# qitianwu/SGFormer

Hardware: AMD Instinct MI355X
Metric: SGFormer fwd+bwd nodes/sec on ogbn-products full-graph (higher is better)
Workload: dtype bf16

## Files before the change

include/sgf.h:

```cpp
#ifndef SGF_H_
#define SGF_H_

#include <stddef.h>
#include <stdint.h>

#ifdef __cplusplus
extern "C" {
#endif

#define SGF_VERSION 662

#define SGF_F32 0
#define SGF_BF16 1
#define SGF_F32_BF16X3 2

#define SGF_OK 0
#define SGF_E_INVALID (-1)
#define SGF_E_WORKSPACE (-2)
#define SGF_E_HIP (-3)
#define SGF_E_UNSUPPORTED (-4)

int sgf_version(void);
const char* sgf_last_error(void);
int sgf_reload_env(void);

size_t sgf_csr_workspace_bytes(int64_t nnz, int64_t n);
int sgf_csr_build(const int64_t* edge_index, int64_t nnz, int64_t n, int64_t* rowptr,
                  int32_t* colind, float* val, int32_t* deg, void* workspace,
                  size_t workspace_bytes, void* stream);

int sgf_csr_transpose(const int64_t* edge_index, int64_t nnz, int64_t n, const int32_t* deg,
                      const int64_t* rowptr, const int32_t* colind, int64_t* t_rowptr,
                      int32_t* t_colind, float* t_val, int32_t* is_symmetric, void* workspace,
                      size_t workspace_bytes, void* stream);

size_t sgf_subgraph_workspace_bytes(int64_t nnz, int64_t n);
int sgf_subgraph_plan(const int64_t* edge_index, int64_t nnz, int64_t n, const int64_t* subset,
                      int64_t m, int32_t* relabel, int64_t* total, void* workspace,
                      size_t workspace_bytes, void* stream);
int sgf_subgraph_emit(const int64_t* edge_index, int64_t nnz, int64_t n, const int32_t* relabel,
                      int32_t relabel_nodes, int64_t total, int64_t* out, int64_t* out_eid,
                      void* workspace, size_t workspace_bytes, void* stream);

size_t sgf_subgraph_csr_plan_workspace_bytes(int64_t m);
size_t sgf_subgraph_csr_emit_workspace_bytes(int64_t m, int64_t total);
int sgf_subgraph_csr_plan(const int64_t* rowptr, const int32_t* colind, int64_t n, const int64_t* subset, int64_t m,
                          int32_t* local_of, int64_t* rowptr_b, int32_t* deg_b, int64_t* total, void* workspace,
                          size_t workspace_bytes, void* stream);
int sgf_subgraph_csr_emit(const int64_t* rowptr, const int32_t* colind, int64_t n, const int64_t* subset, int64_t m,
                          int32_t* local_of, const int64_t* rowptr_b, const int32_t* deg_b, int64_t total, int32_t* colind_b,
                          float* val_b, int64_t* edge_index_b, void* workspace, size_t workspace_bytes, void* stream);

size_t sgf_graph_prologue_workspace_bytes(int64_t m, int64_t n);
int sgf_graph_prologue_plan(const int64_t* edge_index, int64_t m, int64_t n, int32_t to_undirected,
                            int32_t remove_self_loops, int32_t add_self_loops, int64_t* total,
                            void* workspace, size_t workspace_bytes, void* stream);
int sgf_graph_prologue_emit(int64_t m, int64_t n, int32_t to_undirected, int32_t add_self_loops,
                            int64_t total, int64_t* out, void* workspace, size_t workspace_bytes,
                            void* stream);

int sgf_spmm(const int64_t* rowptr, const int32_t* colind, const float* val, const void* x,
             int64_t ldx, int64_t n_cols, void* y, int64_t ldy, int64_t n_rows, int32_t d,
             int32_t dtype, void* stream);

int32_t sgf_spmm_segment_len(void);
int32_t sgf_spmm_arm(int32_t d, int32_t dtype, int64_t ldx, int64_t ldy, int64_t n_cols, int32_t aligned16,
                     int32_t stream);
size_t sgf_spmm_split_workspace_bytes(int64_t long_segments, int32_t d);
int sgf_spmm_split(const int64_t* rowptr, const int32_t* colind, const float* val, const void* x,
                   int64_t ldx, int64_t n_cols, void* y, int64_t ldy, int64_t n_rows, int32_t d, int32_t dtype,
                   int64_t long_len, int64_t long_segments, void* workspace, size_t workspace_bytes,
                   void* stream);

int sgf_spmm_stream(const int64_t* rowptr, const int32_t* colind, const float* val, const void* x,
                    int64_t ldx, int64_t n_cols, void* y, int64_t ldy, int64_t n_rows, int32_t d, int32_t dtype,
                    int64_t long_len, int64_t long_segments, void* workspace, size_t workspace_bytes,
                    void* stream);

size_t sgf_reorder_workspace_bytes(int64_t nnz, int64_t n);
int sgf_reorder(const int64_t* edge_index, int64_t nnz, int64_t n, int32_t iters1, int32_t iters2,
                int32_t* perm, int32_t* inv, int32_t* community, void* workspace, size_t workspace_bytes,
                void* stream);
size_t sgf_spmm_plan_workspace_bytes(int64_t nnz, int64_t n, int32_t rows_per_block);
int sgf_spmm_plan(const int64_t* rowptr, const int32_t* colind, const float* val, int64_t n, int64_t nnz,
                  int32_t rows_per_block, int32_t lds_rows, int64_t long_len, int32_t* ecode, float* eval,
                  int32_t* nlds, int32_t* sh_ptr, int32_t* sh_cols, int64_t* stats, void* workspace,
                  size_t workspace_bytes, void* stream);
int32_t sgf_spmm_lds_rows_len(int32_t dtype);
int32_t sgf_spmm_blocked_arm(int32_t d, int32_t dtype, int64_t ldx, int64_t ldy, int64_t n_rows, int32_t rows_per_block,
                             int32_t lds_rows, int32_t aligned16);
int sgf_spmm_blocked(const int64_t* rowptr, const int32_t* ecode, const float* eval, const int32_t* nlds,
                     const int32_t* sh_ptr, const int32_t* sh_cols, const void* x, int64_t ldx, void* y,
                     int64_t ldy, int64_t n_rows, int32_t d, int32_t dtype, int32_t rows_per_block,
                     int32_t lds_rows, int64_t long_len, int64_t long_segments, void* workspace,
                     size_t workspace_bytes, void* stream);

int sgf_spmm_tile_supported(int32_t d, int32_t dtype);
int sgf_spmm_tile_blocks(const int32_t* comm_sorted, int64_t n, int32_t max_rows, int32_t* blk_row,
                         int64_t blk_cap, int64_t* nb_out, void* stream);
size_t sgf_spmm_tile_plan_workspace_bytes(int64_t nnz, int64_t n, int64_t nb);
int sgf_spmm_tile_plan(const int64_t* rowptr, const int32_t* colind, const float* val, int64_t n, int64_t nnz,
                       const int32_t* blk_row, int64_t nb, int32_t cap, int32_t min_count, int64_t long_len,
                       int32_t* ecode, float* eval, int32_t* nlds, int32_t* sh_ptr, int32_t* sh_cols,
                       int64_t* tile_ptr, int64_t* rem_rowptr, int64_t* stats, void* workspace,
                       size_t workspace_bytes, void* stream);
int sgf_spmm_tile_fill(const int64_t* rowptr, const int32_t* ecode, const float* eval, const int32_t* nlds,
                       int64_t n, int64_t nnz, const int32_t* blk_row, int64_t nb, const int64_t* tile_ptr,
                       int64_t n_frag, const int64_t* rem_rowptr, void* tiles, int32_t* rem_col, float* rem_val,
                       void* stream);
int32_t sgf_spmm_tile_sparse_len(void);
size_t sgf_spmm_tile_pack_workspace_bytes(int64_t n_frag);
int sgf_spmm_tile_pack_layout(const int32_t* blk_row, int64_t nb, const int64_t* tile_ptr, const void* tiles,
                              int64_t n_frag, int32_t* grp, int64_t* pool_units, void* workspace,
                              size_t workspace_bytes, void* stream);
int sgf_spmm_tile_pack(const int32_t* blk_row, int64_t nb, const int64_t* tile_ptr, const void* tiles, int64_t n_frag,
                       const int32_t* grp, void* pool, int64_t pool_units, void* stream);
int sgf_spmm_tile(const int32_t* blk_row, int64_t nb, int32_t block_rows, const int32_t* sh_ptr, const int32_t* sh_cols,
                  const int64_t* tile_ptr, const int32_t* grp, const void* pool, const int64_t* rem_rowptr,
                  const int32_t* rem_col, const float* rem_val, const void* x, int64_t ldx, int64_t n_cols, void* y, int64_t ldy,
                  int64_t n_rows, int32_t d, int32_t dtype, int64_t long_len, int64_t long_segments,
                  void* workspace, size_t workspace_bytes, void* stream);

size_t sgf_neighbor_sample_workspace_bytes(int64_t m, int64_t edge_cap);
int sgf_neighbor_sample_mark(int32_t* local_of, const int32_t* ids, int64_t count, int32_t base, void* stream);
int sgf_neighbor_sample_hop(const int64_t* rowptr, const int32_t* colind, const int32_t* frontier, int64_t m,
                            int32_t frontier_local0, int32_t fanout, uint64_t seed, uint64_t batch, int32_t hop,
                            int32_t* local_of, int32_t n_known, int64_t edge_cap, int32_t* edge_src_local,
                            int32_t* edge_dst_local, int32_t* src_global, int32_t* new_nodes, int64_t* counts,
                            void* workspace, size_t workspace_bytes, void* stream);

size_t sgf_neighbor_sample_batch_workspace_bytes(int64_t batch_size, const int32_t* fanouts, int32_t hops, int64_t* node_cap,
                                                  int64_t* edge_cap);
int sgf_neighbor_sample_batch(const int64_t* rowptr, const int32_t* colind, const int32_t* seeds, int64_t batch_size,
                              const int32_t* fanouts, int32_t hops, uint64_t seed, uint64_t batch, int32_t* local_of,
                              int32_t* nodes, int64_t node_cap, int32_t* edge_src_local, int32_t* edge_dst_local,
                              int64_t edge_cap, int64_t* counts, void* workspace, size_t workspace_bytes, void* stream);

int32_t sgf_sampled_csr_supported(int32_t max_fanout);
size_t sgf_sampled_csr_build_workspace_bytes(int64_t node_cap, int64_t edge_cap);
int sgf_sampled_csr_build(const int32_t* edge_src_local, const int32_t* edge_dst_local, const int64_t* counts,
                          int64_t node_cap, int64_t edge_cap, int32_t max_fanout, int64_t* rowptr_b, int32_t* colind_b,
                          float* val_b, int32_t* deg_b, void* workspace, size_t workspace_bytes, void* stream);
size_t sgf_sampled_csr_transpose_workspace_bytes(int64_t n, int64_t nnz);
int sgf_sampled_csr_transpose(const int64_t* rowptr, const int32_t* colind, const float* val, int64_t n, int64_t nnz,
                              int64_t* t_rowptr, int32_t* t_colind, float* t_val, void* workspace, size_t workspace_bytes,
                              void* stream);

int sgf_gather_rows(const void* src, int64_t lds, int32_t src_dtype, int64_t n_src, const void* idx,
                    int32_t idx_is_int64, int64_t n_out, int32_t d, void* dst, int64_t ldd,
                    int32_t dst_dtype, void* stream);
int sgf_pad_rows(const void* src, int64_t lds, int32_t src_dtype, int64_t n_src, const void* idx, int32_t idx_is_int64,
                 int64_t n_out, int32_t d, int32_t d_pad, void* dst, int64_t ldd, int32_t dst_dtype, void* stream);

int64_t sgf_attn_stats_len(int32_t heads, int32_t d);
size_t sgf_attn_workspace_bytes(int64_t n, int32_t heads, int32_t d);
// ... 16 lines not shown
                        int64_t ldo, const float* den, int64_t n, int32_t heads, int32_t d,
                        int32_t dtype, float* bstats, void* workspace, size_t workspace_bytes,
                        void* stream);

int sgf_attn_bwd_apply(const void* q, int64_t ldq, const void* k, int64_t ldk, const void* v,
                       int64_t ldv, const void* g, int64_t ldg, const void* o, int64_t ldo,
                       const float* den, int64_t n, double n_total, int32_t heads,
                       int32_t v_heads, int32_t d, int32_t dtype, const float* stats,
                       float* bstats, void* dq, int64_t lddq, void* dk, int64_t lddk,
                       void* dv, int64_t lddv, void* stream);
int sgf_attn_bwd_reduce_heads(const void* q, int64_t ldq, const void* g, int64_t ldg, const void* o, int64_t ldo,
                              const float* den, int64_t n, int32_t heads, int32_t d, int32_t dtype, float* bstats,
                              void* workspace, size_t workspace_bytes, void* stream);
int sgf_attn_bwd_apply_heads(const void* q, int64_t ldq, const void* k, int64_t ldk, const void* v, int64_t ldv, const void* g,
                             int64_t ldg, const void* o, int64_t ldo, const float* den, int64_t n, double n_total,
                             int32_t heads, int32_t v_heads, int32_t d, int32_t dtype, const float* stats, float* bstats,
                             void* dq, int64_t lddq, void* dk, int64_t lddk, void* dv, int64_t lddv, void* stream);

int64_t sgf_attn_h_bstats_len(int32_t d);
int32_t sgf_attn_h_supported(int32_t d, int32_t dtype);
int sgf_attn_h_fwd(const void* h, int64_t ldh, int64_t n, int32_t d, int32_t dtype, const float* M,
                   const float* m, const float* w, const float* beta, void* out, int64_t ldo,
                   float* den, void* stream);
int sgf_attn_h_bwd_reduce(const void* h, int64_t ldh, const void* g, int64_t ldg, const void* o,
                          int64_t ldo, const float* den, int64_t n, int32_t d, int32_t dtype,
                          float* hstats, void* workspace, size_t workspace_bytes, void* stream);
int sgf_attn_h_bwd_apply(const void* h, int64_t ldh, const void* g, int64_t ldg, const void* o,
                         int64_t ldo, const float* den, int64_t n, int32_t d, int32_t dtype,
                         const float* M, const float* w, const float* D, const float* ds, void* dh,
                         int64_t lddh, void* workspace, size_t workspace_bytes, void* stream);
size_t sgf_attn_h_bwd_apply_workspace_bytes(int64_t n, int32_t d, int32_t dtype);
int32_t sgf_attn_h_bwd_split_supported(int32_t d, int32_t dtype);
int sgf_attn_h_bwd_pre(const void* g, int64_t ldg, const void* o, int64_t ldo, const float* den, int64_t n, int32_t d,
                       int32_t dtype, const float* M, const float* w, void* workspace, size_t workspace_bytes,
                       float* rowscal, void* stream);
int sgf_attn_h_bwd_reduce_scaled(const void* h, int64_t ldh, const void* g, int64_t ldg, const float* rowscal, int64_t n,
                                 int32_t d, int32_t dtype, float* hstats, void* workspace, size_t workspace_bytes,
                                 void* stream);
int sgf_attn_h_bwd_post(const void* h, int64_t ldh, int64_t n, int32_t d, int32_t dtype, const float* D, const float* ds,
                        const void* workspace, size_t workspace_bytes, const void* addend, int64_t ldadd, void* dh,
                        int64_t lddh, void* stream);

size_t sgf_attn_h_small_saved_bytes(int32_t d_in, int32_t d_out);
size_t sgf_attn_h_small_workspace_bytes(int32_t d_in, int32_t d_out);
int sgf_attn_h_small_fwd(const float* G, int64_t ldg, const float* s, float n_rows, float n_total, const float* wq,
                         const float* bq, const float* wk, const float* bk, const float* wv, const float* bv, int64_t ldw,
                         int32_t d_in, int32_t d_out, float* M, int64_t ldm, float* m, float* w, float* beta, void* saved,
                         size_t saved_bytes, void* stream);
int sgf_attn_h_small_bwd(const float* dM, int64_t lddm, const float* dw, const float* dm, const float* dbeta, float n_total,
                         int32_t d_in, int32_t d_out, const void* saved, size_t saved_bytes, float* dG2, int64_t lddg,
                         float* ds, float* gwq, float* gbq, float* gwk, float* gbk, float* gwv, float* gbv, int64_t ldgw,
                         void* workspace, size_t workspace_bytes, void* stream);

size_t sgf_gram_workspace_bytes(int64_t n, int32_t m, int32_t k);
int sgf_gram(const void* a, int64_t lda, int32_t m, const void* b, int64_t ldb, int32_t k,
             int64_t n, int32_t dtype, float* c, int64_t ldc, float* colsum_a, void* workspace,
             size_t workspace_bytes, void* stream);
int sgf_gram2(const void* a, int64_t lda, int32_t m, const void* b1, int64_t ldb1, const void* b2, int64_t ldb2, int32_t k,
              int64_t n, int32_t dtype, float* c1, int64_t ldc1, float* c2, int64_t ldc2, float* colsum_a, void* workspace,
              size_t workspace_bytes, void* stream);

int sgf_ln_fwd(const void* x, int64_t ldx, const void* res, int64_t ldr, float a, float b,
               const float* gamma, const float* beta, int32_t relu, float eps, int64_t n,
               int32_t d, int32_t dtype, void* y, int64_t ldy, float* mean, float* rstd,
               void* stream);

size_t sgf_ln_bwd_workspace_bytes(int64_t n, int32_t d);
int sgf_ln_bwd(const void* dy, int64_t lddy, const void* y, int64_t ldy, const void* x,
               int64_t ldx, const void* res, int64_t ldr, float a, float b, const float* gamma,
               int32_t relu, const float* mean, const float* rstd, int64_t n, int32_t d,
               int32_t dtype, void* dx, int64_t lddx, void* dres, int64_t lddres, float* dgamma,
               float* dbeta, void* workspace, size_t workspace_bytes, void* stream);

size_t sgf_colstats_workspace_bytes(int64_t n, int32_t d);
int sgf_colstats(const void* x, int64_t ldx, const float* shift, int64_t n, int32_t d,
                 int32_t dtype, float* stats, void* workspace, size_t workspace_bytes,
                 void* stream);
int sgf_bn_finalize(const float* sums, const float* shift, double n_total, float eps, float momentum, float* running_mean,
                    float* running_var, int32_t d, float* mean, float* rstd, void* stream);
int sgf_bn_apply(const void* x, int64_t ldx, const float* mean, const float* rstd,
                 const float* gamma, const float* beta, const void* res, int64_t ldr,
                 int32_t relu, int64_t n, int32_t d, int32_t dtype, void* y, int64_t ldy,
                 void* stream);
int sgf_bn_bwd_stats(const void* dy, int64_t lddy, const void* x, int64_t ldx, const float* mean,
                     const float* rstd, const float* gamma, const float* beta, int32_t relu,
                     int64_t n, int32_t d, int32_t dtype, float* stats, void* workspace,
                     size_t workspace_bytes, void* stream);
int sgf_bn_bwd_stats2(const void* dy, int64_t lddy, const void* dy2, int64_t lddy2, const void* x, int64_t ldx,
                      const float* mean, const float* rstd, const float* gamma, const float* beta, int32_t relu, int64_t n,
                      int32_t d, int32_t dtype, float* stats, void* workspace, size_t workspace_bytes, void* stream);
int32_t sgf_gram_ln_bwd_supported(int32_t m, int32_t k, int32_t dtype);
int sgf_gram_ln_bwd(const void* g, int64_t ldg, const void* xin, int64_t ldx, const float* mean, const float* rstd,
                    const float* gamma, const float* beta, int32_t relu, int32_t m, const void* b, int64_t ldb, int32_t k,
                    int64_t n, int32_t dtype, float* c, int64_t ldc, float* colsum, float* dgamma, float* dbeta, void* workspace,
                    size_t workspace_bytes, void* stream);
int32_t sgf_gram_bn_bwd_supported(int32_t m, int32_t k, int32_t dtype);
int sgf_gram_bn_bwd(const void* g1, int64_t ldg1, const void* g2, int64_t ldg2, const void* z, int64_t ldz, const float* mean,
                    const float* rstd, const float* gamma, const float* beta, int32_t relu, const float* stats, float inv_n,
                    int32_t training, int32_t m, const void* b, int64_t ldb, int32_t k, int64_t n, int32_t dtype, float* c,
                    int64_t ldc, float* colsum, void* workspace, size_t workspace_bytes, void* stream);
int32_t sgf_gram2_bn_bwd_supported(int32_t m, int32_t k, int64_t n, int32_t dtype);
int sgf_gram2_bn_bwd(const void* g, int64_t ldg, const void* z, int64_t ldz, const float* mean, const float* rstd,
                     const float* gamma, const float* beta, int32_t relu, const float* stats, float inv_n, int32_t training,
                     int32_t m, const void* b1, int64_t ldb1, const void* b2, int64_t ldb2, int32_t k, int64_t n, int32_t dtype,
                     void* dz, int64_t lddz, float* c1, int64_t ldc1, float* c2, int64_t ldc2, float* colsum, void* workspace,
                     size_t workspace_bytes, void* stream);
int sgf_bn_bwd_apply(const void* dy, int64_t lddy, const void* x, int64_t ldx, const float* mean,
                     const float* rstd, const float* gamma, const float* beta, int32_t relu,
                     const float* stats, float inv_n, int32_t training, int64_t n, int32_t d,
                     int32_t dtype, void* dx, int64_t lddx, void* stream);

int32_t sgf_combine_fc_supported(int32_t d, int32_t classes, int32_t dtype);
int sgf_combine_fc_fwd(const void* x1, int64_t ld1, float a, const void* x2, int64_t ld2, float b,
                       const float* w, const float* bias, int64_t n, int32_t d, int32_t classes,
                       int32_t dtype, float* logits, int64_t ldl, void* stream);
int sgf_combine_fc_bwd(const float* dlogits, int64_t lddl, const float* w, int64_t n, int32_t d,
                       int32_t classes, float a, float b, int32_t dtype, void* dx1, int64_t ld1, void* dx2,
                       int64_t ld2, void* stream);
int sgf_combine_fc_fwd_mapped(const void* x1, int64_t ld1, float a, const void* x2, int64_t ld2, float b, const float* w,
                              const float* bias, int64_t n, int32_t d, int32_t classes, int32_t dtype, float* logits,
                              int64_t ldl, const int32_t* row_map, void* stream);
int sgf_combine_fc_bwd_mapped(const float* dlogits, int64_t lddl, const float* w, int64_t n, int32_t d, int32_t classes,
                              float a, float b, int32_t dtype, void* dx1, int64_t ld1, void* dx2, int64_t ld2,
                              const int32_t* row_map, void* stream);
int sgf_combine_fc_bwd_g(const float* dlogits, int64_t lddl, const float* w, int64_t n, int32_t d, int32_t classes, float a,
                         float b, int32_t dtype, void* dx1, int64_t ld1, void* dx2, int64_t ld2, const int32_t* row_map,
                         void* g_out, int64_t ldg, void* stream);

int32_t sgf_gcn_epilogue_supported(int32_t d_in, int32_t d_out, int32_t dtype);
size_t sgf_gcn_epilogue_workspace_bytes(int64_t n, int32_t d_out);
int sgf_gcn_epilogue_stats(const void* a, int64_t lda, const void* w, int64_t ldw, const float* bias,
                           int64_t n, int32_t d_in, int32_t d_out, int32_t dtype, void* y, int64_t ldy,
                           const float* shift, float* stats, void* workspace, size_t workspace_bytes,
                           void* stream);
int sgf_gcn_epilogue_dx2(const void* dy, int64_t lddy, const void* w1, const void* w2, int64_t ldw, int64_t n, int32_t d,
                         int32_t dtype, void* dx1, int64_t lddx1, void* dx2, int64_t lddx2, int32_t pair, void* stream);

int32_t sgf_gcn_epilogue_dx2_acc_supported(int32_t d, int32_t dtype);
int sgf_gcn_epilogue_dx2_acc(const void* dz, int64_t lddz, const void* w, int64_t ldw, int64_t n, int32_t d, int32_t dtype,
                             void* dy, int64_t lddy, const void* gadd, int64_t ldg, const void* acc_in, int64_t ldai,
                             void* acc_out, int64_t ldao, void* stream);
int sgf_gcn_epilogue_dx(const void* dy, int64_t lddy, const void* w, int64_t ldw, int64_t n, int32_t d_in,
                        int32_t d_out, int32_t dtype, void* dx, int64_t lddx, void* stream);
int sgf_gcn_epilogue_apply(const void* y, int64_t ldy, const float* mean, const float* rstd, const float* gamma,
                           const float* beta, const void* res, int64_t ldr, int32_t relu, int64_t n, int32_t d,
                           int32_t dtype, void* out, int64_t ldo, void* stream);
int32_t sgf_gcn_bn_bwd_dx_supported(int32_t d, int32_t dtype);
size_t sgf_gcn_bn_bwd_dx_workspace_bytes(int64_t n, int32_t d);
int sgf_gcn_bn_bwd_dx(const void* gy, int64_t ldg, const void* z, int64_t ldz, const float* mean, const float* rstd,
                      const float* gamma, const float* beta, int32_t relu, const float* stats, float inv_n,
                      int32_t training, const void* w, int64_t ldw, int64_t n, int32_t d, int32_t dtype, void* dz,
                      int64_t lddz, void* dy, int64_t lddy, const void* acc_in, void* acc_out, size_t acc_bytes,
                      void* dx0, int64_t lddx0, int32_t add_gy, void* workspace, size_t workspace_bytes, void* stream);
int32_t sgf_gcn_epilogue_cat_supported(int32_t d, int32_t dtype);
int sgf_gcn_epilogue_cat(const void* a1, int64_t lda1, const void* a2, int64_t lda2, const void* w, int64_t ldw,
                         const float* bias, int64_t n, int32_t d, int32_t dtype, void* y, int64_t ldy, const float* shift,
                         float* stats, void* workspace, size_t workspace_bytes, void* stream);
size_t sgf_gcn_epilogue_partial_bytes(int64_t n, int32_t d_out);
size_t sgf_gcn_epilogue_dtype_partial_bytes(int64_t n, int32_t d_out, int32_t dtype);
int sgf_gcn_epilogue_partial(const void* a, int64_t lda, const void* w, int64_t ldw, const float* bias, int64_t n,
                             int32_t d_in, int32_t d_out, int32_t dtype, void* partial, size_t partial_bytes,
                             void* stream);
int sgf_gcn_epilogue_stats_add(const void* a, int64_t lda, const void* w, int64_t ldw, const void* partial,
                               size_t partial_bytes, int64_t n, int32_t d_in, int32_t d_out, int32_t dtype,
                               void* y, int64_t ldy, const float* shift, float* stats, void* workspace,
                               size_t workspace_bytes, void* stream);
// ... 74 lines not shown
```

sgformer_amd/_lib.py:

```python
from __future__ import annotations

import ctypes
import os
from ctypes import c_char_p, c_double, c_float, c_int32, c_int64, c_size_t, c_uint64, c_void_p

_HERE = os.path.dirname(os.path.abspath(__file__))
LIB_PATH = os.path.join(_HERE, "lib", "libsgf.so")

SGF_F32 = 0
SGF_BF16 = 1
SGF_F32_BF16X3 = 2
SGF_BCE_TARGET_F32 = 0
SGF_BCE_TARGET_I64 = 1
SGF_BCE_TARGET_CLASS = 2
SGF_METRIC_TARGET_F32 = 0
SGF_METRIC_TARGET_I64 = 1

_lib = None

_P = c_void_p
SIGNATURES = {
    "sgf_version": (c_int32, []),
    "sgf_last_error": (c_char_p, []),
    "sgf_reload_env": (c_int32, []),
    "sgf_csr_workspace_bytes": (c_size_t, [c_int64, c_int64]),
    "sgf_csr_build": (c_int32, [_P, c_int64, c_int64, _P, _P, _P, _P, _P, c_size_t, _P]),
    "sgf_csr_transpose": (c_int32, [_P, c_int64, c_int64, _P, _P, _P, _P, _P, _P, _P, _P, c_size_t, _P]),
    "sgf_subgraph_workspace_bytes": (c_size_t, [c_int64, c_int64]),
    "sgf_subgraph_plan": (c_int32, [_P, c_int64, c_int64, _P, c_int64, _P, _P, _P, c_size_t, _P]),
    "sgf_subgraph_emit": (c_int32, [_P, c_int64, c_int64, _P, c_int32, c_int64, _P, _P, _P, c_size_t, _P]),
    "sgf_subgraph_csr_plan_workspace_bytes": (c_size_t, [c_int64]),
    "sgf_subgraph_csr_emit_workspace_bytes": (c_size_t, [c_int64, c_int64]),
    "sgf_subgraph_csr_plan": (c_int32, [_P, _P, c_int64, _P, c_int64, _P, _P, _P, _P, _P, c_size_t, _P]),
    "sgf_subgraph_csr_emit": (c_int32, [_P, _P, c_int64, _P, c_int64, _P, _P, _P, c_int64, _P, _P, _P, _P, c_size_t, _P]),
    "sgf_graph_prologue_workspace_bytes": (c_size_t, [c_int64, c_int64]),
    "sgf_graph_prologue_plan": (c_int32, [_P, c_int64, c_int64, c_int32, c_int32, c_int32, _P, _P, c_size_t, _P]),
    "sgf_graph_prologue_emit": (c_int32, [c_int64, c_int64, c_int32, c_int32, c_int64, _P, _P, c_size_t, _P]),
    "sgf_spmm": (c_int32, [_P, _P, _P, _P, c_int64, c_int64, _P, c_int64, c_int64, c_int32, c_int32, _P]),
    "sgf_spmm_segment_len": (c_int32, []),
    "sgf_spmm_arm": (c_int32, [c_int32, c_int32, c_int64, c_int64, c_int64, c_int32, c_int32]),
    "sgf_spmm_split_workspace_bytes": (c_size_t, [c_int64, c_int32]),
    "sgf_spmm_split": (c_int32, [_P, _P, _P, _P, c_int64, c_int64, _P, c_int64, c_int64, c_int32, c_int32, c_int64,
                                 c_int64, _P, c_size_t, _P]),
    "sgf_spmm_stream": (c_int32, [_P, _P, _P, _P, c_int64, c_int64, _P, c_int64, c_int64, c_int32, c_int32, c_int64,
                                  c_int64, _P, c_size_t, _P]),
    "sgf_reorder_workspace_bytes": (c_size_t, [c_int64, c_int64]),
    "sgf_reorder": (c_int32, [_P, c_int64, c_int64, c_int32, c_int32, _P, _P, _P, _P, c_size_t, _P]),
    "sgf_spmm_plan_workspace_bytes": (c_size_t, [c_int64, c_int64, c_int32]),
    "sgf_spmm_plan": (c_int32, [_P, _P, _P, c_int64, c_int64, c_int32, c_int32, c_int64, _P, _P, _P, _P, _P, _P,
                                _P, c_size_t, _P]),
    "sgf_spmm_lds_rows_len": (c_int32, [c_int32]),
    "sgf_spmm_blocked_arm": (c_int32, [c_int32, c_int32, c_int64, c_int64, c_int64, c_int32, c_int32, c_int32]),
    "sgf_spmm_blocked": (c_int32, [_P, _P, _P, _P, _P, _P, _P, c_int64, _P, c_int64, c_int64, c_int32, c_int32,
                                   c_int32, c_int32, c_int64, c_int64, _P, c_size_t, _P]),
    "sgf_spmm_tile_supported": (c_int32, [c_int32, c_int32]),
    "sgf_spmm_tile_blocks": (c_int32, [_P, c_int64, c_int32, _P, c_int64, _P, _P]),
    "sgf_spmm_tile_plan_workspace_bytes": (c_size_t, [c_int64, c_int64, c_int64]),
    "sgf_spmm_tile_plan": (c_int32, [_P, _P, _P, c_int64, c_int64, _P, c_int64, c_int32, c_int32, c_int64, _P, _P, _P,
                                     _P, _P, _P, _P, _P, _P, c_size_t, _P]),
    "sgf_spmm_tile_fill": (c_int32, [_P, _P, _P, _P, c_int64, c_int64, _P, c_int64, _P, c_int64, _P, _P, _P, _P, _P]),
    "sgf_spmm_tile_sparse_len": (c_int32, []),
    "sgf_spmm_tile_pack_workspace_bytes": (c_size_t, [c_int64]),
    "sgf_spmm_tile_pack_layout": (c_int32, [_P, c_int64, _P, _P, c_int64, _P, _P, _P, c_size_t, _P]),
    "sgf_spmm_tile_pack": (c_int32, [_P, c_int64, _P, _P, c_int64, _P, _P, c_int64, _P]),
    "sgf_spmm_tile": (c_int32, [_P, c_int64, c_int32, _P, _P, _P, _P, _P, _P, _P, _P, _P, c_int64, c_int64, _P, c_int64,
                                c_int64, c_int32, c_int32, c_int64, c_int64, _P, c_size_t, _P]),
    "sgf_neighbor_sample_workspace_bytes": (c_size_t, [c_int64, c_int64]),
    "sgf_neighbor_sample_mark": (c_int32, [_P, _P, c_int64, c_int32, _P]),
    "sgf_neighbor_sample_batch_workspace_bytes": (c_size_t, [c_int64, _P, c_int32, _P, _P]),
    "sgf_neighbor_sample_batch": (c_int32, [_P, _P, _P, c_int64, _P, c_int32, c_uint64, c_uint64, _P, _P, c_int64, _P, _P,
                                            c_int64, _P, _P, c_size_t, _P]),
    "sgf_neighbor_sample_hop": (c_int32, [_P, _P, _P, c_int64, c_int32, c_int32, c_uint64, c_uint64, c_int32, _P, c_int32,
                                          c_int64, _P, _P, _P, _P, _P, _P, c_size_t, _P]),
    "sgf_sampled_csr_supported": (c_int32, [c_int32]),
    "sgf_sampled_csr_build_workspace_bytes": (c_size_t, [c_int64, c_int64]),
    "sgf_sampled_csr_build": (c_int32, [_P, _P, _P, c_int64, c_int64, c_int32, _P, _P, _P, _P, _P, c_size_t, _P]),
    "sgf_sampled_csr_transpose_workspace_bytes": (c_size_t, [c_int64, c_int64]),
    "sgf_sampled_csr_transpose": (c_int32, [_P, _P, _P, c_int64, c_int64, _P, _P, _P, _P, c_size_t, _P]),
    "sgf_gather_rows": (c_int32, [_P, c_int64, c_int32, c_int64, _P, c_int32, c_int64, c_int32, _P, c_int64,
                                  c_int32, _P]),
    "sgf_pad_rows": (c_int32, [_P, c_int64, c_int32, c_int64, _P, c_int32, c_int64, c_int32, c_int32, _P, c_int64,
                               c_int32, _P]),
    "sgf_attn_stats_len": (c_int64, [c_int32, c_int32]),
    "sgf_attn_bstats_len": (c_int64, [c_int32, c_int32]),
    "sgf_attn_workspace_bytes": (c_size_t, [c_int64, c_int32, c_int32]),
    "sgf_attn_max_blocks": (c_int32, []),
    "sgf_attn_tile_rows": (c_int32, [c_int32, c_int32, c_int32]),
    "sgf_attn_fwd_reduce": (c_int32, [_P, c_int64, _P, c_int64, _P, c_int64, c_int64, c_int32, c_int32,
                                      c_int32, c_int32, _P, _P, c_size_t, _P]),
    "sgf_attn_fwd_apply": (c_int32, [_P, c_int64, _P, c_int64, c_int64, c_double, c_int32, c_int32,
                                     c_int32, c_int32, _P, _P, c_int64, _P, _P, _P]),
    "sgf_attn_bwd_reduce": (c_int32, [_P, c_int64, _P, c_int64, _P, c_int64, _P, c_int64, c_int32,
                                      c_int32, c_int32, _P, _P, c_size_t, _P]),
    "sgf_attn_bwd_apply": (c_int32, [_P, c_int64, _P, c_int64, _P, c_int64, _P, c_int64, _P, c_int64,
                                     _P, c_int64, c_double, c_int32, c_int32, c_int32, c_int32, _P, _P,
                                     _P, c_int64, _P, c_int64, _P, c_int64, _P]),
    "sgf_attn_bwd_reduce_heads": (c_int32, [_P, c_int64, _P, c_int64, _P, c_int64, _P, c_int64, c_int32,
                                            c_int32, c_int32, _P, _P, c_size_t, _P]),
    "sgf_attn_bwd_apply_heads": (c_int32, [_P, c_int64, _P, c_int64, _P, c_int64, _P, c_int64, _P, c_int64,
                                           _P, c_int64, c_double, c_int32, c_int32, c_int32, c_int32, _P, _P,
                                           _P, c_int64, _P, c_int64, _P, c_int64, _P]),
    "sgf_attn_h_bstats_len": (c_int64, [c_int32]),
    "sgf_attn_h_fwd": (c_int32, [_P, c_int64, c_int64, c_int32, c_int32, _P, _P, _P, _P, _P, c_int64, _P, _P]),
    "sgf_attn_h_bwd_reduce": (c_int32, [_P, c_int64, _P, c_int64, _P, c_int64, _P, c_int64, c_int32, c_int32,
                                        _P, _P, c_size_t, _P]),
    "sgf_attn_h_bwd_apply": (c_int32, [_P, c_int64, _P, c_int64, _P, c_int64, _P, c_int64, c_int32, c_int32,
                                       _P, _P, _P, _P, _P, c_int64, _P, c_size_t, _P]),
    "sgf_attn_h_bwd_apply_workspace_bytes": (c_size_t, [c_int64, c_int32, c_int32]),
    "sgf_attn_h_bwd_split_supported": (c_int32, [c_int32, c_int32]),
    "sgf_attn_h_supported": (c_int32, [c_int32, c_int32]),
    "sgf_attn_h_bwd_pre": (c_int32, [_P, c_int64, _P, c_int64, _P, c_int64, c_int32, c_int32, _P, _P, _P, c_size_t, _P, _P]),
    "sgf_attn_h_bwd_reduce_scaled": (c_int32, [_P, c_int64, _P, c_int64, _P, c_int64, c_int32, c_int32, _P, _P, c_size_t,
                                               _P]),
    "sgf_attn_h_bwd_post": (c_int32, [_P, c_int64, c_int64, c_int32, c_int32, _P, _P, _P, c_size_t, _P, c_int64, _P,
                                      c_int64, _P]),
    "sgf_attn_h_small_saved_bytes": (c_size_t, [c_int32, c_int32]),
    "sgf_attn_h_small_workspace_bytes": (c_size_t, [c_int32, c_int32]),
    "sgf_attn_h_small_fwd": (c_int32, [_P, c_int64, _P, c_float, c_float, _P, _P, _P, _P, _P, _P, c_int64, c_int32, c_int32,
                                       _P, c_int64, _P, _P, _P, _P, c_size_t, _P]),
    "sgf_attn_h_small_bwd": (c_int32, [_P, c_int64, _P, _P, _P, c_float, c_int32, c_int32, _P, c_size_t, _P, c_int64, _P,
                                       _P, _P, _P, _P, _P, _P, c_int64, _P, c_size_t, _P]),
    "sgf_gram_workspace_bytes": (c_size_t, [c_int64, c_int32, c_int32]),
    "sgf_gram": (c_int32, [_P, c_int64, c_int32, _P, c_int64, c_int32, c_int64, c_int32, _P, c_int64, _P,
                           _P, c_size_t, _P]),
    "sgf_gram2": (c_int32, [_P, c_int64, c_int32, _P, c_int64, _P, c_int64, c_int32, c_int64, c_int32, _P, c_int64, _P,
                            c_int64, _P, _P, c_size_t, _P]),
    "sgf_ln_fwd": (c_int32, [_P, c_int64, _P, c_int64, c_float, c_float, _P, _P, c_int32, c_float,
                             c_int64, c_int32, c_int32, _P, c_int64, _P, _P, _P]),
    "sgf_ln_bwd_workspace_bytes": (c_size_t, [c_int64, c_int32]),
    "sgf_ln_bwd": (c_int32, [_P, c_int64, _P, c_int64, _P, c_int64, _P, c_int64, c_float, c_float, _P,
                             c_int32, _P, _P, c_int64, c_int32, c_int32, _P, c_int64, _P, c_int64, _P,
                             _P, _P, c_size_t, _P]),
    "sgf_colstats_workspace_bytes": (c_size_t, [c_int64, c_int32]),
    "sgf_colstats": (c_int32, [_P, c_int64, _P, c_int64, c_int32, c_int32, _P, _P, c_size_t, _P]),
    "sgf_bn_finalize": (c_int32, [_P, _P, c_double, c_float, c_float, _P, _P, c_int32, _P, _P, _P]),
    "sgf_bn_apply": (c_int32, [_P, c_int64, _P, _P, _P, _P, _P, c_int64, c_int32, c_int64, c_int32,
                               c_int32, _P, c_int64, _P]),
    "sgf_bn_bwd_stats": (c_int32, [_P, c_int64, _P, c_int64, _P, _P, _P, _P, c_int32, c_int64, c_int32,
                                   c_int32, _P, _P, c_size_t, _P]),
    "sgf_bn_bwd_stats2": (c_int32, [_P, c_int64, _P, c_int64, _P, c_int64, _P, _P, _P, _P, c_int32, c_int64, c_int32,
                                    c_int32, _P, _P, c_size_t, _P]),
    "sgf_gram_ln_bwd_supported": (c_int32, [c_int32, c_int32, c_int32]),
    "sgf_gram_ln_bwd": (c_int32, [_P, c_int64, _P, c_int64, _P, _P, _P, _P, c_int32, c_int32, _P, c_int64, c_int32, c_int64,
                                  c_int32, _P, c_int64, _P, _P, _P, _P, c_size_t, _P]),
    "sgf_gram_bn_bwd_supported": (c_int32, [c_int32, c_int32, c_int32]),
    "sgf_gram_bn_bwd": (c_int32, [_P, c_int64, _P, c_int64, _P, c_int64, _P, _P, _P, _P, c_int32, _P, c_float, c_int32,
                                  c_int32, _P, c_int64, c_int32, c_int64, c_int32, _P, c_int64, _P, _P, c_size_t, _P]),
    "sgf_gram2_bn_bwd_supported": (c_int32, [c_int32, c_int32, c_int64, c_int32]),
    "sgf_gram2_bn_bwd": (c_int32, [_P, c_int64, _P, c_int64, _P, _P, _P, _P, c_int32, _P, c_float, c_int32, c_int32, _P, c_int64,
                                   _P, c_int64, c_int32, c_int64, c_int32, _P, c_int64, _P, c_int64, _P, c_int64, _P, _P,
                                   c_size_t, _P]),
    "sgf_bn_bwd_apply": (c_int32, [_P, c_int64, _P, c_int64, _P, _P, _P, _P, c_int32, _P, c_float,
                                   c_int32, c_int64, c_int32, c_int32, _P, c_int64, _P]),
    "sgf_dropout": (c_int32, [_P, c_int64, _P, c_int64, c_float, c_uint64, c_int64, c_int32, c_int32, _P,
                              c_int64, _P]),
    "sgf_dropout_dev": (c_int32, [_P, c_int64, _P, c_int64, c_float, _P, c_int64, c_int32, c_int32, _P,
                                  c_int64, _P]),
    "sgf_nll_workspace_bytes": (c_size_t, [c_int64]),
    "sgf_nll_fwd": (c_int32, [_P, c_int64, c_int64, c_int32, c_int32, _P, _P, c_int64, _P, _P, c_size_t, _P]),
    "sgf_nll_bwd": (c_int32, [_P, c_int64, c_int64, c_int32, c_int32, _P, _P, c_int64, _P, c_float, _P,
                              c_int64, _P]),
    "sgf_bce_workspace_bytes": (c_size_t, [c_int64, c_int32]),
    "sgf_bce_fwd": (c_int32, [_P, c_int64, c_int64, c_int32, c_int32, _P, c_int64, c_int32, _P, c_int64, c_float, _P, _P,
                              c_size_t, _P]),
    "sgf_bce_bwd": (c_int32, [_P, c_int64, c_int64, c_int32, c_int32, _P, c_int64, c_int32, _P, c_int64, _P, c_float, _P,
                              c_int64, _P]),
    "sgf_rocauc_workspace_bytes": (c_size_t, [c_int64, c_int32]),
    "sgf_rocauc_counts": (c_int32, [_P, c_int64, c_int64, c_int32, c_int32, _P, c_int64, c_int32, _P, c_int64, _P, _P,
                                    c_size_t, _P]),
    "sgf_argmax_workspace_bytes": (c_size_t, [c_int64, c_int32]),
    "sgf_argmax_count": (c_int32, [_P, c_int64, c_int64, c_int32, c_int32, _P, c_int64, c_int32, _P, c_int64, _P, _P,
                                   c_size_t, _P]),
    "sgf_sum_n": (c_int32, [_P, _P, c_int32, c_int64, c_int32, c_int32, _P, c_int64, _P]),
    "sgf_colsum_workspace_bytes": (c_size_t, [c_int64, c_int32]),
    "sgf_colsum": (c_int32, [_P, c_int64, c_int64, c_int32, c_int32, _P, _P, c_size_t, _P]),
    "sgf_combine_fc_supported": (c_int32, [c_int32, c_int32, c_int32]),
    "sgf_combine_fc_fwd": (c_int32, [_P, c_int64, c_float, _P, c_int64, c_float, _P, _P, c_int64, c_int32, c_int32,
                                     c_int32, _P, c_int64, _P]),
    "sgf_combine_fc_bwd": (c_int32, [_P, c_int64, _P, c_int64, c_int32, c_int32, c_float, c_float, c_int32, _P,
                                     c_int64, _P, c_int64, _P]),
    "sgf_combine_fc_fwd_mapped": (c_int32, [_P, c_int64, c_float, _P, c_int64, c_float, _P, _P, c_int64, c_int32, c_int32,
                                     c_int32, _P, c_int64, _P, _P]),
    "sgf_combine_fc_bwd_g": (c_int32, [_P, c_int64, _P, c_int64, c_int32, c_int32, c_float, c_float, c_int32, _P, c_int64, _P,
                                       c_int64, _P, _P, c_int64, _P]),
    "sgf_combine_fc_bwd_mapped": (c_int32, [_P, c_int64, _P, c_int64, c_int32, c_int32, c_float, c_float, c_int32, _P,
                                     c_int64, _P, c_int64, _P, _P]),
    "sgf_gcn_epilogue_supported": (c_int32, [c_int32, c_int32, c_int32]),
    "sgf_gcn_epilogue_workspace_bytes": (c_size_t, [c_int64, c_int32]),
    "sgf_gcn_epilogue_stats": (c_int32, [_P, c_int64, _P, c_int64, _P, c_int64, c_int32, c_int32, c_int32, _P, c_int64,
                                         _P, _P, _P, c_size_t, _P]),
    "sgf_gcn_epilogue_dx": (c_int32, [_P, c_int64, _P, c_int64, c_int64, c_int32, c_int32, c_int32, _P, c_int64, _P]),
    "sgf_gcn_epilogue_dx2": (c_int32, [_P, c_int64, _P, _P, c_int64, c_int64, c_int32, c_int32, _P, c_int64, _P, c_int64,
                                       c_int32, _P]),
    "sgf_gcn_epilogue_dx2_acc_supported": (c_int32, [c_int32, c_int32]),
    "sgf_gcn_epilogue_dx2_acc": (c_int32, [_P, c_int64, _P, c_int64, c_int64, c_int32, c_int32, _P, c_int64, _P, c_int64, _P,
                                           c_int64, _P, c_int64, _P]),
    "sgf_gcn_epilogue_apply": (c_int32, [_P, c_int64, _P, _P, _P, _P, _P, c_int64, c_int32, c_int64, c_int32,
                               c_int32, _P, c_int64, _P]),
    "sgf_gcn_bn_bwd_dx_supported": (c_int32, [c_int32, c_int32]),
    "sgf_gcn_bn_bwd_dx_workspace_bytes": (c_size_t, [c_int64, c_int32]),
    "sgf_gcn_bn_bwd_dx": (c_int32, [_P, c_int64, _P, c_int64, _P, _P, _P, _P, c_int32, _P, c_float, c_int32, _P, c_int64,
                                    c_int64, c_int32, c_int32, _P, c_int64, _P, c_int64, _P, _P, c_size_t, _P, c_int64,
                                    c_int32, _P, c_size_t, _P]),
    "sgf_gcn_epilogue_cat_supported": (c_int32, [c_int32, c_int32]),
    "sgf_gcn_epilogue_cat": (c_int32, [_P, c_int64, _P, c_int64, _P, c_int64, _P, c_int64, c_int32, c_int32, _P, c_int64,
                                       _P, _P, _P, c_size_t, _P]),
    "sgf_gcn_epilogue_partial_bytes": (c_size_t, [c_int64, c_int32]),
    "sgf_gcn_epilogue_dtype_partial_bytes": (c_size_t, [c_int64, c_int32, c_int32]),
    "sgf_gcn_epilogue_partial": (c_int32, [_P, c_int64, _P, c_int64, _P, c_int64, c_int32, c_int32, c_int32, _P,
                                           c_size_t, _P]),
    "sgf_gcn_epilogue_stats_add": (c_int32, [_P, c_int64, _P, c_int64, _P, c_size_t, c_int64, c_int32, c_int32,
                                             c_int32, _P, c_int64, _P, _P, _P, c_size_t, _P]),
    "sgf_stem_pair_supported": (c_int32, [c_int32, c_int32, c_int32]),
    "sgf_stem_pair": (c_int32, [_P, c_int64, c_int64, c_int32, _P, c_int64, _P, _P, c_int64, _P, c_int32, c_int32, _P,
                                c_int64, _P, c_int64, _P, _P, _P, c_size_t, _P]),
    "sgf_gemm": (c_int32, [_P, c_int64, c_int64, c_int32, _P, c_int64, c_int64, c_int32, c_int64, c_int32, c_int64, c_float,
                           _P, _P, c_float, _P, c_int64, c_int32, _P, c_int64, c_int32, _P]),
    "sgf_comm_available": (c_int32, []),
    "sgf_comm_unique_id_bytes": (c_int32, []),
    "sgf_comm_unique_id": (c_int32, [_P]),
# ... 47 lines not shown
```

sgformer_amd/csrc/fused.hip:

```cpp
#include "common.h"

namespace sgf {
namespace {

constexpr int kThreads = 256;
constexpr int kMaxD = 1024;
constexpr int kMaxStatBlocks = 2048;

__device__ __forceinline__ float4 zero4() { return make_float4(0.f, 0.f, 0.f, 0.f); }
__device__ __forceinline__ float4 ld4f(const float* p) { return *reinterpret_cast<const float4*>(p); }

inline int lanes_per_row(int d) {
  int l = 16;
  while (l * 4 < d && l < 64) l <<= 1;
  return l;
}

template <typename T, int LPR, int NC>
__global__ __launch_bounds__(kThreads) void k_ln_fwd(
    const T* __restrict__ x, int64_t ldx, const T* __restrict__ res, int64_t ldr, float a, float b,
    const float* __restrict__ gamma, const float* __restrict__ beta, int relu, float eps, int64_t n,
    int d, T* __restrict__ y, int64_t ldy, float* __restrict__ mean, float* __restrict__ rstd) {
  constexpr int RPB = kThreads / LPR;
  const int sl = threadIdx.x % LPR;
// ... 466 lines not shown
          g.z = (xh.z * ga.z + be.z) > 0.f ? g.z : 0.f;
          g.w = (xh.w * ga.w + be.w) > 0.f ? g.w : 0.f;
        }
        if (training) {
          g.x -= s0.x * inv_n + xh.x * s1.x * inv_n;
          g.y -= s0.y * inv_n + xh.y * s1.y * inv_n;
          g.z -= s0.z * inv_n + xh.z * s1.z * inv_n;
          g.w -= s0.w * inv_n + xh.w * s1.w * inv_n;
        }
        store4<T>(dx + row * lddx + col,
                  make_float4(ga.x * rs.x * g.x, ga.y * rs.y * g.y, ga.z * rs.z * g.z, ga.w * rs.w * g.w));
      }
    }
  }
}

typedef __bf16 ew_bf16v2 __attribute__((ext_vector_type(2)));
typedef float ew_f32v2 __attribute__((ext_vector_type(2)));
__device__ __forceinline__ uint32_t ew_pack(float a, float b) {
  const ew_f32v2 v = {a, b};
  return __builtin_bit_cast(uint32_t, __builtin_convertvector(v, ew_bf16v2));
}
__device__ __forceinline__ void ew_unpack(const uint4& r, float (&v)[8]) {
  v[0] = __uint_as_float(r.x << 16); v[1] = __uint_as_float(r.x & 0xffff0000u);
  v[2] = __uint_as_float(r.y << 16); v[3] = __uint_as_float(r.y & 0xffff0000u);
  v[4] = __uint_as_float(r.z << 16); v[5] = __uint_as_float(r.z & 0xffff0000u);
  v[6] = __uint_as_float(r.w << 16); v[7] = __uint_as_float(r.w & 0xffff0000u);
}
__device__ __forceinline__ uint4 ew_pack8(const float (&o)[8]) {
  return make_uint4(ew_pack(o[0], o[1]), ew_pack(o[2], o[3]), ew_pack(o[4], o[5]), ew_pack(o[6], o[7]));
}
struct BnCoeffs8 {
  float mu[8], rs[8], ga[8], be[8];
};
__device__ __forceinline__ void bn_coeffs8(const BnParams& p, int col, BnCoeffs8& c) {
#pragma unroll
  for (int e = 0; e < 8; ++e) {
    c.mu[e] = p.mean[col + e];
    c.rs[e] = p.rstd[col + e];
    c.ga[e] = p.gamma ? p.gamma[col + e] : 1.f;
    c.be[e] = p.beta ? p.beta[col + e] : 0.f;
  }
}

template <bool kRes, int U>
__global__ __launch_bounds__(kThreads) void k_bn_apply_bf16x8(const uint16_t* __restrict__ x, int64_t ldx, BnParams p,
                                                              const uint16_t* __restrict__ res, int64_t ldr, int relu,
                                                              int64_t n, int d, uint16_t* __restrict__ y, int64_t ldy) {
  const int f8 = d / 8;
  const int rpp = kThreads / f8;
  const int sr = threadIdx.x / f8;
  if (sr >= rpp) return;
  const int col = (threadIdx.x % f8) * 8;
  BnCoeffs8 c;
  bn_coeffs8(p, col, c);
  const int64_t rpb = static_cast<int64_t>(rpp) * U;
  for (int64_t row0 = static_cast<int64_t>(blockIdx.x) * rpb + sr; row0 < n; row0 += static_cast<int64_t>(gridDim.x) * rpb) {
    uint4 xv[U], rv[U];
#pragma unroll
    for (int u = 0; u < U; ++u) {
      const int64_t row = row0 + u * rpp;
      if (row < n) {
        xv[u] = *reinterpret_cast<const uint4*>(x + row * ldx + col);
        if (kRes) rv[u] = *reinterpret_cast<const uint4*>(res + row * ldr + col);
      }
    }
#pragma unroll
    for (int u = 0; u < U; ++u) {
      const int64_t row = row0 + u * rpp;
      if (row < n) {
        float v[8], r[8], o[8];
        ew_unpack(xv[u], v);
        if (kRes) ew_unpack(rv[u], r);
#pragma unroll
        for (int e = 0; e < 8; ++e) {
          o[e] = fmaf((v[e] - c.mu[e]) * c.rs[e], c.ga[e], c.be[e]);
          if (relu) o[e] = fmaxf(o[e], 0.f);
          if (kRes) o[e] += r[e];
        }
        *reinterpret_cast<uint4*>(y + row * ldy + col) = ew_pack8(o);
      }
    }
  }
}

template <int U>
__global__ __launch_bounds__(kThreads) void k_bn_bwd_apply_bf16x8(
    const uint16_t* __restrict__ dy, int64_t lddy, const uint16_t* __restrict__ x, int64_t ldx, BnParams p, int relu,
    const float* __restrict__ stats, float inv_n, int training, int64_t n, int d, uint16_t* __restrict__ dx, int64_t lddx) {
  const int f8 = d / 8;
  const int rpp = kThreads / f8;
  const int sr = threadIdx.x / f8;
  if (sr >= rpp) return;
  const int col = (threadIdx.x % f8) * 8;
  BnCoeffs8 c;
  bn_coeffs8(p, col, c);
  float s0[8], s1[8];
#pragma unroll
  for (int e = 0; e < 8; ++e) {
    s0[e] = training ? stats[col + e] : 0.f;
    s1[e] = training ? stats[d + col + e] : 0.f;
  }
  const int64_t rpb = static_cast<int64_t>(rpp) * U;
  for (int64_t row0 = static_cast<int64_t>(blockIdx.x) * rpb + sr; row0 < n; row0 += static_cast<int64_t>(gridDim.x) * rpb) {
    uint4 xv[U], gv[U];
#pragma unroll
    for (int u = 0; u < U; ++u) {
      const int64_t row = row0 + u * rpp;
      if (row < n) {
        xv[u] = *reinterpret_cast<const uint4*>(x + row * ldx + col);
        gv[u] = *reinterpret_cast<const uint4*>(dy + row * lddy + col);
      }
    }
#pragma unroll
    for (int u = 0; u < U; ++u) {
      const int64_t row = row0 + u * rpp;
      if (row < n) {
        float v[8], g[8], o[8];
        ew_unpack(xv[u], v);
        ew_unpack(gv[u], g);
#pragma unroll
        for (int e = 0; e < 8; ++e) {
          const float xh = (v[e] - c.mu[e]) * c.rs[e];
          float ge = g[e];
          if (relu) ge = fmaf(xh, c.ga[e], c.be[e]) > 0.f ? ge : 0.f;
          if (training) ge -= s0[e] * inv_n + xh * s1[e] * inv_n;
          o[e] = c.ga[e] * c.rs[e] * ge;
        }
        *reinterpret_cast<uint4*>(dx + row * lddx + col) = ew_pack8(o);
      }
    }
  }
}

template <int LPR, int R>
__global__ __launch_bounds__(kThreads) void k_ln_bwd_bf16x8(
    const uint16_t* __restrict__ dy, int64_t lddy, const uint16_t* __restrict__ y, int64_t ldy, const uint16_t* __restrict__ x,
    int64_t ldx, const uint16_t* __restrict__ res, int64_t ldr, float a, float b, const float* __restrict__ gamma, int relu,
    const float* __restrict__ mean, const float* __restrict__ rstd, int64_t n, uint16_t* __restrict__ dxo, int64_t lddx,
    uint16_t* __restrict__ dro, int64_t lddr, float* __restrict__ part) {
  constexpr int RPS = kThreads / LPR;
  constexpr int RPB = RPS * R;
  constexpr int D = 8 * LPR;
  constexpr float inv_d = 1.0f / static_cast<float>(D);
  __shared__ float red[2 * RPS * D];
  const int sl = threadIdx.x % LPR;
  const int sr = threadIdx.x / LPR;
  const int col = sl * 8;
  const bool ln = gamma != nullptr;
  float gm[8], dg[8], db[8];
#pragma unroll
  for (int e = 0; e < 8; ++e) {
    gm[e] = ln ? gamma[col + e] : 1.f;
    dg[e] = db[e] = 0.f;
  }
  for (int64_t row0 = static_cast<int64_t>(blockIdx.x) * RPB; row0 < n; row0 += static_cast<int64_t>(gridDim.x) * RPB) {
    uint4 gv[R], yv[R], xv[R], rv[R];
    float mu[R], rs[R];
#pragma unroll
    for (int q = 0; q < R; ++q) {
      const int64_t row = row0 + q * RPS + sr;
      const int64_t rr = row < n ? row : n - 1;
      gv[q] = *reinterpret_cast<const uint4*>(dy + rr * lddy + col);
      if (relu) yv[q] = *reinterpret_cast<const uint4*>(y + rr * ldy + col);
      if (ln) {
        xv[q] = *reinterpret_cast<const uint4*>(x + rr * ldx + col);
// ... 713 lines not shown
}

extern "C" int sgf_colstats(const void* x, int64_t ldx, const float* shift, int64_t n, int32_t d,
                            int32_t dtype, float* stats, void* workspace, size_t workspace_bytes,
                            void* stream) {
  int rc = check_ew("sgf_colstats", n, d, dtype);
  if (rc != SGF_OK) return rc;
  hipStream_t st = static_cast<hipStream_t>(stream);
  SGF_REQUIRE(stats, SGF_E_INVALID, "sgf_colstats: null stats");
  if (n == 0) {
    SGF_CHECK_HIP(hipMemsetAsync(stats, 0, 2 * d * sizeof(float), st));
    return SGF_OK;
  }
  SGF_REQUIRE(x && ldx % 4 == 0, SGF_E_INVALID, "sgf_colstats: bad x / ldx");
  SGF_REQUIRE(workspace && workspace_bytes >= sgf_colstats_workspace_bytes(n, d), SGF_E_WORKSPACE,
              "sgf_colstats: workspace too small");
  if (dtype == SGF_F32)
    return colreduce(ColStatsF<float>{static_cast<const float*>(x), ldx, shift}, n, d, stats,
                     workspace, st);
  return colreduce(ColStatsF<uint16_t>{static_cast<const uint16_t*>(x), ldx, shift}, n, d, stats,
                   workspace, st);
}

__global__ __launch_bounds__(256) void k_bn_finalize(const float* __restrict__ sums, const float* __restrict__ shift,
                                                     float inv_n, float unbias, float eps, float momentum,
                                                     float* __restrict__ rmean, float* __restrict__ rvar, int d,
                                                     float* __restrict__ mean, float* __restrict__ rstd) {
  const int c = blockIdx.x * 256 + threadIdx.x;
  if (c >= d) return;
  const float m1 = sums[c] * inv_n;
  const float mu = (shift ? shift[c] : 0.f) + m1;
  float var = sums[d + c] * inv_n - m1 * m1;
  var = var > 0.f ? var : 0.f;
  mean[c] = mu;
  rstd[c] = 1.0f / sqrtf(var + eps);
  if (rmean) rmean[c] = rmean[c] * (1.0f - momentum) + momentum * mu;
  if (rvar) rvar[c] = rvar[c] * (1.0f - momentum) + momentum * (var * unbias);
}

extern "C" int sgf_bn_finalize(const float* sums, const float* shift, double n_total, float eps, float momentum,
                               float* running_mean, float* running_var, int32_t d, float* mean, float* rstd, void* stream) {
  SGF_REQUIRE(d >= 1 && n_total >= 0, SGF_E_INVALID, "sgf_bn_finalize: bad sizes");
  SGF_REQUIRE(sums && mean && rstd, SGF_E_INVALID, "sgf_bn_finalize: null pointer");
  const double nn = n_total > 1.0 ? n_total : 1.0;
  const float unbias = static_cast<float>(n_total / (n_total - 1.0 > 1.0 ? n_total - 1.0 : 1.0));
  hipLaunchKernelGGL(k_bn_finalize, dim3((d + 255) / 256), dim3(256), 0, static_cast<hipStream_t>(stream), sums, shift,
                     static_cast<float>(1.0 / nn), unbias, eps, momentum, running_mean, running_var, d, mean, rstd);
  SGF_LAUNCH_CHECK();
  return SGF_OK;
}

extern "C" int sgf_bn_apply(const void* x, int64_t ldx, const float* mean, const float* rstd,
                            const float* gamma, const float* beta, const void* res, int64_t ldr,
                            int32_t relu, int64_t n, int32_t d, int32_t dtype, void* y, int64_t ldy,
                            void* stream) {
  int rc = check_ew("sgf_bn_apply", n, d, dtype);
  if (rc != SGF_OK) return rc;
  if (n == 0) return SGF_OK;
  SGF_REQUIRE(x && y && mean && rstd, SGF_E_INVALID, "sgf_bn_apply: null pointer");
  SGF_REQUIRE(ldx % 4 == 0 && ldy % 4 == 0 && (!res || ldr % 4 == 0), SGF_E_INVALID,
              "sgf_bn_apply: leading dims must be multiples of 4");
  hipStream_t st = static_cast<hipStream_t>(stream);
  const BnParams p{mean, rstd, gamma, beta};
  if (dtype == SGF_BF16 && ew8_rows(d, {{x, ldx}, {res, ldr}, {y, ldy}})) {
    const dim3 g8(rowwalk8_grid(n, d));
#define SGF_BNA(RES_, U_)                                                                                             \
  hipLaunchKernelGGL((k_bn_apply_bf16x8<RES_, U_>), g8, dim3(kThreads), 0, st, static_cast<const uint16_t*>(x), ldx, p, \
                     static_cast<const uint16_t*>(res), ldr, relu, n, d, static_cast<uint16_t*>(y), ldy)
    if (res) SGF_BNA(true, kEw8Unroll);
    else SGF_BNA(false, kEw8Unroll);
#undef SGF_BNA
    SGF_LAUNCH_CHECK();
    return SGF_OK;
  }
  const dim3 grid(rowwalk_grid(n, d));
  if (dtype == SGF_F32)
    hipLaunchKernelGGL((k_bn_apply<float>), grid, dim3(kThreads), 0, st,
                       static_cast<const float*>(x), ldx, p, static_cast<const float*>(res), ldr,
                       relu, n, d, static_cast<float*>(y), ldy);
  else
    hipLaunchKernelGGL((k_bn_apply<uint16_t>), grid, dim3(kThreads), 0, st,
                       static_cast<const uint16_t*>(x), ldx, p, static_cast<const uint16_t*>(res),
                       ldr, relu, n, d, static_cast<uint16_t*>(y), ldy);
  SGF_LAUNCH_CHECK();
  return SGF_OK;
}

extern "C" int sgf_bn_bwd_stats2(const void* dy, int64_t lddy, const void* dy2, int64_t lddy2, const void* x, int64_t ldx,
                                 const float* mean, const float* rstd, const float* gamma, const float* beta,
                                 int32_t relu, int64_t n, int32_t d, int32_t dtype, float* stats, void* workspace,
                                 size_t workspace_bytes, void* stream) {
  int rc = check_ew("sgf_bn_bwd_stats2", n, d, dtype);
  if (rc != SGF_OK) return rc;
  hipStream_t st = static_cast<hipStream_t>(stream);
  SGF_REQUIRE(stats, SGF_E_INVALID, "sgf_bn_bwd_stats2: null stats");
  if (n == 0) {
    SGF_CHECK_HIP(hipMemsetAsync(stats, 0, 2 * d * sizeof(float), st));
    return SGF_OK;
  }
  SGF_REQUIRE(dy && x && mean && rstd && lddy % 4 == 0 && ldx % 4 == 0 && (!dy2 || lddy2 % 4 == 0), SGF_E_INVALID,
              "sgf_bn_bwd_stats2: bad pointer / ld");
  SGF_REQUIRE(workspace && workspace_bytes >= sgf_colstats_workspace_bytes(n, d), SGF_E_WORKSPACE,
              "sgf_bn_bwd_stats2: workspace too small");
  const BnParams p{mean, rstd, gamma, beta};
  if (dtype == SGF_BF16 && ew8_rows(d, {{dy, lddy}, {dy2, lddy2}, {x, ldx}})) {
    const int nblk = stat_blocks(n);
    float* part = static_cast<float*>(workspace);
#define SGF_BNS(TWO_, U_)                                                                                             \
  hipLaunchKernelGGL((k_bn_bwd_stats_bf16x8<TWO_, U_>), dim3(nblk), dim3(kThreads), 0, st, static_cast<const uint16_t*>(dy), \
                     lddy, static_cast<const uint16_t*>(dy2), lddy2, static_cast<const uint16_t*>(x), ldx, p, relu, n, d, part)
    if (dy2) SGF_BNS(true, kEw8Unroll);
    else SGF_BNS(false, kEw8Unroll);
#undef SGF_BNS
    SGF_LAUNCH_CHECK();
    hipLaunchKernelGGL(k_sum_partials, dim3((2 * d + 7) / 8), dim3(256), 0, st, part, nblk, 2 * d, stats, stats + d, d);
    SGF_LAUNCH_CHECK();
    return SGF_OK;
  }
  if (dtype == SGF_F32)
    return colreduce(BnBwdStatsF<float>{static_cast<const float*>(dy), lddy, static_cast<const float*>(x), ldx, p, relu,
                                        static_cast<const float*>(dy2), lddy2},
                     n, d, stats, workspace, st);
  return colreduce(BnBwdStatsF<uint16_t>{static_cast<const uint16_t*>(dy), lddy, static_cast<const uint16_t*>(x), ldx, p,
                                         relu, static_cast<const uint16_t*>(dy2), lddy2},
                   n, d, stats, workspace, st);
}

extern "C" int sgf_bn_bwd_stats(const void* dy, int64_t lddy, const void* x, int64_t ldx,
                                const float* mean, const float* rstd, const float* gamma,
                                const float* beta, int32_t relu, int64_t n, int32_t d,
                                int32_t dtype, float* stats, void* workspace,
                                size_t workspace_bytes, void* stream) {
  return sgf_bn_bwd_stats2(dy, lddy, nullptr, 0, x, ldx, mean, rstd, gamma, beta, relu, n, d, dtype, stats, workspace,
                           workspace_bytes, stream);
}

extern "C" int sgf_bn_bwd_apply(const void* dy, int64_t lddy, const void* x, int64_t ldx,
                                const float* mean, const float* rstd, const float* gamma,
                                const float* beta, int32_t relu, const float* stats, float inv_n,
                                int32_t training, int64_t n, int32_t d, int32_t dtype, void* dx,
                                int64_t lddx, void* stream) {
  int rc = check_ew("sgf_bn_bwd_apply", n, d, dtype);
  if (rc != SGF_OK) return rc;
  if (n == 0) return SGF_OK;
  SGF_REQUIRE(dy && x && dx && mean && rstd && (!training || stats), SGF_E_INVALID,
              "sgf_bn_bwd_apply: null pointer");
  SGF_REQUIRE(lddy % 4 == 0 && ldx % 4 == 0 && lddx % 4 == 0, SGF_E_INVALID,
              "sgf_bn_bwd_apply: leading dims must be multiples of 4");
  hipStream_t st = static_cast<hipStream_t>(stream);
  const BnParams p{mean, rstd, gamma, beta};
  if (dtype == SGF_BF16 && ew8_rows(d, {{dy, lddy}, {x, ldx}, {dx, lddx}})) {
#define SGF_BNB(U_)                                                                                                   \
  hipLaunchKernelGGL((k_bn_bwd_apply_bf16x8<U_>), dim3(rowwalk8_grid(n, d)), dim3(kThreads), 0, st,                     \
                     static_cast<const uint16_t*>(dy), lddy, static_cast<const uint16_t*>(x), ldx, p, relu, stats, inv_n, \
                     training, n, d, static_cast<uint16_t*>(dx), lddx)
    SGF_BNB(kEw8Unroll);
#undef SGF_BNB
    SGF_LAUNCH_CHECK();
    return SGF_OK;
  }
  const dim3 grid(rowwalk_grid(n, d));
  if (dtype == SGF_F32)
    hipLaunchKernelGGL((k_bn_bwd_apply<float>), grid, dim3(kThreads), 0, st,
                       static_cast<const float*>(dy), lddy, static_cast<const float*>(x), ldx, p,
                       relu, stats, inv_n, training, n, d, static_cast<float*>(dx), lddx);
  else
// ... 296 lines not shown
```

sgformer_amd/csrc/spmm.hip:

```cpp
#include "common.h"
#include "spmm_shared.h"

#include <climits>
#include <cstdlib>

namespace sgf {
namespace {

constexpr int kWavesPerBlock = 4;

__device__ __forceinline__ void fma4(float4& acc, float v, const float4& x) {
  acc.x = fmaf(v, x.x, acc.x);
  acc.y = fmaf(v, x.y, acc.y);
  acc.z = fmaf(v, x.z, acc.z);
  acc.w = fmaf(v, x.w, acc.w);
}

template <typename T, int UNROLL>
__global__ __launch_bounds__(kWavesPerBlock * 64) void k_spmm_wave(
    const int64_t* __restrict__ rowptr, const int32_t* __restrict__ colind,
    const float* __restrict__ val, const T* __restrict__ x, int64_t ldx, T* __restrict__ y,
    int64_t ldy, int64_t n_rows, int32_t d, LongQueue lq) {
  const int lane = threadIdx.x & 63;
  const int wid = __builtin_amdgcn_readfirstlane(static_cast<int>(threadIdx.x >> 6));
// ... 70 lines not shown
  int32_t c[N];
  float v[N];
  typename BufRow<T>::Raw raw[N];
#pragma unroll
  for (int u = 0; u < N; ++u) {
    c[u] = colind[e + u];
    v[u] = val[e + u];
  }
#pragma unroll
  for (int u = 0; u < N; ++u) raw[u] = BufRow<T>::load(rsrc, voff, static_cast<uint32_t>(c[u]) * pitch);
#pragma unroll
  for (int u = 0; u < N; ++u) fma4(acc, v[u], BufRow<T>::widen(raw[u]));
}

template <typename T, int UNROLL>
__global__ __launch_bounds__(kWavesPerBlock * 64) void k_spmm_row(
    const int64_t* __restrict__ rowptr, const int32_t* __restrict__ colind, const float* __restrict__ val,
    const T* __restrict__ x, uint32_t pitch, uint32_t x_bytes, T* __restrict__ y, int64_t ldy, int64_t n_rows,
    int32_t d, LongQueue lq) {
  const int lane = threadIdx.x & 63;
  const int wid = __builtin_amdgcn_readfirstlane(static_cast<int>(threadIdx.x >> 6));
  const int64_t blk = xcd_remap(blockIdx.x, gridDim.x);
  const int64_t row = blk * kWavesPerBlock + wid;
  if (row >= n_rows) return;
  const int64_t e0 = rowptr[row];
  const int64_t e1 = rowptr[row + 1];
  if (e1 - e0 > lq.long_len) {
    push_long_row(lq, row, e1 - e0, lane, 64);
    return;
  }
  const __amdgpu_buffer_rsrc_t rsrc = __builtin_amdgcn_make_buffer_rsrc(const_cast<T*>(x), 0, x_bytes, 0x00020000);
  const int fc = lane * 4;
  const bool active = fc < d;
  const int voff = active ? fc * static_cast<int>(sizeof(T)) : 0;
  float4 acc = make_float4(0.f, 0.f, 0.f, 0.f);
  const int32_t* __restrict__ ci = colind + e0;
  const float* __restrict__ va = val + e0;
  const int len = static_cast<int>(e1 - e0);
  int i = 0;
  if (UNROLL <= len) {
    int32_t c0[UNROLL], c1[UNROLL];
    float v0[UNROLL], v1[UNROLL];
    typename BufRow<T>::Raw raw[UNROLL];
#pragma unroll
    for (int u = 0; u < UNROLL; ++u) {
      c0[u] = ci[u];
      v0[u] = va[u];
    }
    for (;;) {
#pragma unroll
      for (int u = 0; u < UNROLL; ++u) raw[u] = BufRow<T>::load(rsrc, voff, static_cast<uint32_t>(c0[u]) * pitch);
      i += UNROLL;
      const bool more_a = i + UNROLL <= len;
      if (more_a) {
#pragma unroll
        for (int u = 0; u < UNROLL; ++u) {
          c1[u] = ci[i + u];
          v1[u] = va[i + u];
        }
      }
#pragma unroll
      for (int u = 0; u < UNROLL; ++u) fma4(acc, v0[u], BufRow<T>::widen(raw[u]));
      if (!more_a) break;
#pragma unroll
      for (int u = 0; u < UNROLL; ++u) raw[u] = BufRow<T>::load(rsrc, voff, static_cast<uint32_t>(c1[u]) * pitch);
      i += UNROLL;
      const bool more_b = i + UNROLL <= len;
      if (more_b) {
#pragma unroll
        for (int u = 0; u < UNROLL; ++u) {
          c0[u] = ci[i + u];
          v0[u] = va[i + u];
        }
      }
#pragma unroll
      for (int u = 0; u < UNROLL; ++u) fma4(acc, v1[u], BufRow<T>::widen(raw[u]));
      if (!more_b) break;
    }
  }
  if (i + 4 <= len) { gather_batch<T, 4>(rsrc, voff, pitch, ci, va, i, acc); i += 4; }
  if (i + 2 <= len) { gather_batch<T, 2>(rsrc, voff, pitch, ci, va, i, acc); i += 2; }
  if (i < len) gather_batch<T, 1>(rsrc, voff, pitch, ci, va, i, acc);
  if (active) store4<T>(y + row * ldy + fc, acc);
}

constexpr int kSegRows = 4;

template <typename T, int G>
__global__ __launch_bounds__(kWavesPerBlock * 64) void k_spmm_seg(
    const int64_t* __restrict__ rowptr, const int32_t* __restrict__ colind, const float* __restrict__ val,
    const T* __restrict__ x, uint32_t pitch, uint32_t x_bytes, T* __restrict__ y, int64_t ldy, int64_t n_rows,
    int32_t d, int32_t chunk_blocks, LongQueue lq) {
  using Raw = typename BufRow<T>::Raw;
  const int lane = threadIdx.x & 63;
  const int wid = __builtin_amdgcn_readfirstlane(static_cast<int>(threadIdx.x >> 6));
  const int64_t blk = xcd_remap(blockIdx.x, gridDim.x, chunk_blocks);
  const int64_t r_first = (blk * kWavesPerBlock + wid) * kSegRows;
  if (r_first >= n_rows) return;
  const int nr = n_rows - r_first < kSegRows ? static_cast<int>(n_rows - r_first) : kSegRows;
  const __amdgpu_buffer_rsrc_t rsrc = __builtin_amdgcn_make_buffer_rsrc(const_cast<T*>(x), 0, x_bytes, 0x00020000);
  const int fc = lane * 4;
  const bool active = fc < d;
  const int voff = active ? fc * static_cast<int>(sizeof(T)) : 0;
  T* __restrict__ yl = y + r_first * ldy + (active ? fc : 0);

  const int64_t e_first = rowptr[r_first];
  const int64_t end_abs = rowptr[r_first + 1 + (lane < nr ? lane : nr - 1)];
  const int64_t begin_abs = __shfl_up(end_abs, 1, 64);
  const int64_t len_i = end_abs - (lane == 0 ? e_first : begin_abs);
  const bool long_i = lane < nr && len_i > lq.long_len;
  auto lane64 = [&](int64_t v, int i) -> int64_t {
    const uint32_t lo = __builtin_amdgcn_readlane(static_cast<int>(v & 0xffffffff), i);
    const uint32_t hi = __builtin_amdgcn_readlane(static_cast<int>(v >> 32), i);
    return static_cast<int64_t>((static_cast<uint64_t>(hi) << 32) | lo);
  };
  const int64_t total64 = lane64(end_abs, nr - 1) - e_first;
  const int32_t* __restrict__ ci = colind + e_first;
  const float* __restrict__ va = val + e_first;

  if (__ballot(long_i) != 0 || total64 >= (static_cast<int64_t>(1) << 31)) {
    for (int r = 0; r < nr; ++r) {
      const int64_t re = lane64(end_abs, r);
      const int64_t rb = r == 0 ? e_first : lane64(end_abs, r - 1);
      if (re - rb > lq.long_len) {
        push_long_row(lq, r_first + r, re - rb, lane, 64);
        continue;
      }
      float4 acc = make_float4(0.f, 0.f, 0.f, 0.f);
      for (int64_t e = rb; e < re; ++e)
        fma4(acc, val[e], BufRow<T>::widen(BufRow<T>::load(rsrc, voff, static_cast<uint32_t>(colind[e]) * pitch)));
      if (active) store4<T>(yl + r * ldy, acc);
    }
    return;
  }

  const int rel_v = static_cast<int>(end_abs - e_first);
  const int total = static_cast<int>(total64);
  int row = 0;
  int row_end = __builtin_amdgcn_readlane(rel_v, 0);
  float4 acc = make_float4(0.f, 0.f, 0.f, 0.f);
  auto boundary = [&](int p) {
    while (p == row_end && row < nr) {
      if (active) store4<T>(yl + row * ldy, acc);
      acc = make_float4(0.f, 0.f, 0.f, 0.f);
      ++row;
      row_end = row < nr ? __builtin_amdgcn_readlane(rel_v, row < kSegRows ? row : kSegRows - 1) : 0x7fffffff;
    }
  };

  int pos = 0;
  int32_t c0[G], c1[G];
  float v0[G], v1[G];
  Raw raw[G];
  if (G <= total) {
#pragma unroll
    for (int u = 0; u < G; ++u) {
      c0[u] = ci[u];
      v0[u] = va[u];
    }
    for (;;) {
#pragma unroll
      for (int u = 0; u < G; ++u) raw[u] = BufRow<T>::load(rsrc, voff, static_cast<uint32_t>(c0[u]) * pitch);
      const bool more_a = pos + 2 * G <= total;
      if (more_a) {
#pragma unroll
        for (int u = 0; u < G; ++u) {
// ... 741 lines not shown
  c.blk2 = elem_size == 2 && d % 8 == 0 && d <= 256 && ldx % 8 == 0 && ldy % 8 == 0 && aligned16 &&
           c.x_bytes < (static_cast<uint64_t>(1) << 32) && c.threads <= 512 && g_blk2.get() != 0;
  return c;
}
bool blk_rows_ok(int32_t rows_per_block) {
  return rows_per_block >= kBlkRowsPerWave && rows_per_block <= 128 && rows_per_block % kBlkRowsPerWave == 0;
}
bool blk_lds_rows_ok(int32_t lds_rows, int32_t dtype) { return lds_rows >= 1 && lds_rows <= sgf_spmm_lds_rows_len(dtype); }

template <typename T>
int launch_blocked(const int64_t* rowptr, const int32_t* ecode, const float* eval, const int32_t* nlds,
                   const int32_t* sh_ptr, const int32_t* sh_cols, const T* x, int64_t ldx, T* y, int64_t ldy,
                   int64_t n_rows, int32_t d, int32_t rows_per_block, int32_t lds_rows, hipStream_t st,
                   const LongQueue& lq, float* partial) {
  const BlkChoice c = choose_blocked(d, sizeof(T), ldx, ldy, n_rows, rows_per_block, lds_rows,
                                     reinterpret_cast<uintptr_t>(x) % 16 == 0 && reinterpret_cast<uintptr_t>(y) % 16 == 0);
  const int threads = c.threads;
  const size_t lds_bytes = c.lds_bytes;
  const bool lean = c.lean;
  const int64_t nb = (n_rows + rows_per_block - 1) / rows_per_block;
  int chunk = 4096 / rows_per_block;
  if (chunk < 1) chunk = 1;
#ifdef SGF_PROBES
  const int dbg = g_blk_debug.get();
#else
  const int dbg = 0;
#endif
  constexpr int DGd = sizeof(T) == 4 ? 4 : 8, DGl = sizeof(T) == 4 ? 2 : 4;
  auto deep_fn = &k_spmm_blk<T, DGd, DGd, 4>;
  auto lean_fn = &k_spmm_blk<T, DGl, DGl, 8>;
  static thread_local size_t attr_set[4] = {0, 0, 0, 0};
  const int which = (sizeof(T) == 4 ? 0 : 2) + (lean ? 1 : 0);
  if (lds_bytes > attr_set[which]) {
    SGF_CHECK_HIP(hipFuncSetAttribute(lean ? reinterpret_cast<const void*>(lean_fn) : reinterpret_cast<const void*>(deep_fn),
                                      hipFuncAttributeMaxDynamicSharedMemorySize, static_cast<int>(lds_bytes)));
    attr_set[which] = lds_bytes;
  }
  if (c.blk2) {
    const size_t lds2 = lds_bytes;
    auto fn2 = &k_spmm_blk2<8, 4>;
    static thread_local size_t attr2 = 0;
    if (lds2 > attr2) {
      SGF_CHECK_HIP(hipFuncSetAttribute(reinterpret_cast<const void*>(fn2), hipFuncAttributeMaxDynamicSharedMemorySize,
                                        static_cast<int>(lds2)));
      attr2 = lds2;
    }
    hipLaunchKernelGGL(fn2, dim3(static_cast<unsigned>(nb)), dim3(threads), lds2, st, rowptr, ecode, eval, nlds, sh_ptr,
                       sh_cols, reinterpret_cast<const uint16_t*>(x), static_cast<uint32_t>(ldx * sizeof(T)),
                       static_cast<uint32_t>(c.x_bytes), reinterpret_cast<uint16_t*>(y), ldy, n_rows, d, rows_per_block,
                       lds_rows, chunk, lq, dbg);
  } else if (lean)
    hipLaunchKernelGGL(lean_fn, dim3(static_cast<unsigned>(nb)), dim3(threads), lds_bytes, st, rowptr, ecode, eval,
                       nlds, sh_ptr, sh_cols, x, ldx, y, ldy, n_rows, d, rows_per_block, lds_rows, chunk, lq, dbg);
  else
    hipLaunchKernelGGL(deep_fn, dim3(static_cast<unsigned>(nb)), dim3(threads), lds_bytes, st, rowptr, ecode, eval,
                       nlds, sh_ptr, sh_cols, x, ldx, y, ldy, n_rows, d, rows_per_block, lds_rows, chunk, lq, dbg);
  SGF_LAUNCH_CHECK();
  return spmm_long_rows(sizeof(T) == 2 ? SGF_BF16 : SGF_F32, rowptr, ecode, eval, x, ldx, d, lq, partial, y, ldy, st);
}

enum class Arm { SegBf16x2, Seg, Row, Wave, Sub };
struct Choice { Arm arm; int lanes_per_row; };
Choice choose_kernel(int32_t d, size_t elem_size, bool fits32, bool pair_ok, bool stream, int forced) {
  const bool pairs = fits32 && elem_size == 2 && pair_ok;
  const bool narrow_stream = d > 64 && d <= 128 && pairs && forced != kForceSub;
  if (d > 128 || narrow_stream) {
    if (pairs && (stream || forced == kForceSeg2 || (narrow_stream && forced == kForceNone))) return {Arm::SegBf16x2, 0};
    if (fits32 && forced == kForceSeg) return {Arm::Seg, 0};
    if (fits32 && forced != kForceWave) return {Arm::Row, 0};
    return {Arm::Wave, 0};
  }
  return {Arm::Sub, d > 64 ? 32 : d > 32 ? 16 : d > 16 ? 8 : d > 8 ? 4 : d > 4 ? 2 : 1};
}

Choice choose_for_operands(int32_t d, size_t elem_size, int64_t ldx, int64_t ldy, int64_t n_cols, bool aligned16,
                           bool stream, uint64_t* x_bytes_out = nullptr) {
  const uint64_t x_bytes = static_cast<uint64_t>(n_cols) * static_cast<uint64_t>(ldx) * elem_size;
  if (x_bytes_out) *x_bytes_out = x_bytes;
  const bool fits32 = d <= 256 && n_cols > 0 && x_bytes < (static_cast<uint64_t>(1) << 32);
  const bool pair_ok = d % 8 == 0 && ldx % 8 == 0 && ldy % 8 == 0 && aligned16;
  return choose_kernel(d, elem_size, fits32, pair_ok, stream, g_forced.get());
}

template <typename T>
int launch(const int64_t* rowptr, const int32_t* colind, const float* val, const T* x, int64_t ldx, int64_t n_cols,
           T* y, int64_t ldy, int64_t n_rows, int32_t d, hipStream_t st, const LongQueue& lq,
           float* partial, bool stream) {
  constexpr int UNROLL = 8;
  const dim3 block(kWavesPerBlock * 64);
  uint64_t x_bytes;
  const Choice c = choose_for_operands(d, sizeof(T), ldx, ldy, n_cols,
                                       reinterpret_cast<uintptr_t>(x) % 16 == 0 && reinterpret_cast<uintptr_t>(y) % 16 == 0,
                                       stream, &x_bytes);
  const int64_t nb = (n_rows + kWavesPerBlock - 1) / kWavesPerBlock;
  const int64_t nbs = (n_rows + kWavesPerBlock * kSegRows - 1) / (kWavesPerBlock * kSegRows);
  const int chunk_rows = g_chunk_rows.get() > 0 ? g_chunk_rows.get() : 4096;
  const int chunk = chunk_rows / (kWavesPerBlock * kSegRows) > 0 ? chunk_rows / (kWavesPerBlock * kSegRows) : 1;
#define SGF_SUB(LPR_)                                                                         \
  case LPR_: {                                                                                \
    constexpr int RPB = kWavesPerBlock * (64 / LPR_);                                         \
    const int64_t nbr = (n_rows + RPB - 1) / RPB;                                             \
    hipLaunchKernelGGL((k_spmm_sub<T, LPR_, UNROLL>), dim3(static_cast<unsigned>(nbr)), block, \
                       0, st, rowptr, colind, val, x, ldx, y, ldy, n_rows, d, lq);            \
  } break;
  switch (c.arm) {
    case Arm::SegBf16x2:
      hipLaunchKernelGGL((k_spmm_seg_bf16x2<16>), dim3(static_cast<unsigned>(nbs)), block, 0, st, rowptr, colind, val,
                         reinterpret_cast<const uint16_t*>(x), static_cast<uint32_t>(ldx * sizeof(T)),
                         static_cast<uint32_t>(x_bytes), reinterpret_cast<uint16_t*>(y), ldy, n_rows, d, chunk, lq);
      break;
    case Arm::Seg:
      hipLaunchKernelGGL((k_spmm_seg<T, (sizeof(T) == 4 ? 8 : 16)>), dim3(static_cast<unsigned>(nbs)), block, 0, st,
                         rowptr, colind, val, x, static_cast<uint32_t>(ldx * sizeof(T)),
                         static_cast<uint32_t>(x_bytes), y, ldy, n_rows, d, chunk, lq);
      break;
    case Arm::Row:
      hipLaunchKernelGGL((k_spmm_row<T, UNROLL>), dim3(static_cast<unsigned>(nb)), block, 0, st, rowptr, colind,
                         val, x, static_cast<uint32_t>(ldx * sizeof(T)), static_cast<uint32_t>(x_bytes), y, ldy,
                         n_rows, d, lq);
      break;
    case Arm::Wave:
      hipLaunchKernelGGL((k_spmm_wave<T, UNROLL>), dim3(static_cast<unsigned>(nb)), block, 0, st,
                         rowptr, colind, val, x, ldx, y, ldy, n_rows, d, lq);
      break;
    case Arm::Sub:
      switch (c.lanes_per_row) {
        SGF_SUB(32)
        SGF_SUB(16)
        SGF_SUB(8)
        SGF_SUB(4)
        SGF_SUB(2)
        SGF_SUB(1)
      }
      break;
  }
#undef SGF_SUB
  SGF_LAUNCH_CHECK();
  return spmm_long_rows(sizeof(T) == 2 ? SGF_BF16 : SGF_F32, rowptr, colind, val, x, ldx, d, lq, partial, y, ldy, st);
}

}

int spmm_long_rows(int dtype, const int64_t* rowptr, const int32_t* colind, const float* val, const void* x, int64_t ldx,
                   int32_t d, const LongQueue& lq, float* partial, void* y, int64_t ldy, hipStream_t st) {
  if (lq.cap <= 0) return SGF_OK;
  constexpr int UNROLL = 8;
  const dim3 block(kWavesPerBlock * 64);
  const int nb = lq.cap < 2048 ? lq.cap : 2048;
  if (dtype == SGF_BF16) {
    hipLaunchKernelGGL((k_spmm_long_seg<uint16_t, UNROLL>), dim3(nb), block, 0, st, rowptr, colind, val,
                       static_cast<const uint16_t*>(x), ldx, d, lq, partial);
    SGF_LAUNCH_CHECK();
    hipLaunchKernelGGL((k_spmm_long_fin<uint16_t>), dim3(nb), dim3(256), 0, st, lq, partial, d,
                       static_cast<uint16_t*>(y), ldy);
  } else {
    hipLaunchKernelGGL((k_spmm_long_seg<float, UNROLL>), dim3(nb), block, 0, st, rowptr, colind, val,
                       static_cast<const float*>(x), ldx, d, lq, partial);
    SGF_LAUNCH_CHECK();
    hipLaunchKernelGGL((k_spmm_long_fin<float>), dim3(nb), dim3(256), 0, st, lq, partial, d, static_cast<float*>(y), ldy);
  }
  SGF_LAUNCH_CHECK();
  return SGF_OK;
}

}

using namespace sgf;

namespace {
int check_spmm_operands(const char* fn, const void* x, int64_t ldx, const void* y, int64_t ldy, int32_t d, int32_t dtype) {
  SGF_REQUIRE(dtype == SGF_F32 || dtype == SGF_BF16, SGF_E_INVALID, "%s: unknown dtype %d", fn, dtype);
  SGF_REQUIRE(d % 4 == 0 && ldx % 4 == 0 && ldy % 4 == 0 && ldx >= d && ldy >= d, SGF_E_INVALID,
              "%s: d, ldx, ldy must be multiples of 4 with ld >= d (d=%d ldx=%lld ldy=%lld)", fn, d,
              static_cast<long long>(ldx), static_cast<long long>(ldy));
  const size_t esz = dtype == SGF_BF16 ? 2 : 4;
  SGF_REQUIRE(reinterpret_cast<uintptr_t>(x) % (4 * esz) == 0 && reinterpret_cast<uintptr_t>(y) % (4 * esz) == 0,
              SGF_E_INVALID, "%s: x / y must be aligned to 4 elements", fn);
  return SGF_OK;
}

int spmm_common(const int64_t* rowptr, const int32_t* colind, const float* val, const void* x, int64_t ldx,
                int64_t n_cols, void* y, int64_t ldy, int64_t n_rows, int32_t d, int32_t dtype, const LongQueue& lq,
                float* partial, hipStream_t st, const char* fn, bool stream = false) {
  SGF_REQUIRE(n_rows >= 0 && d >= 0 && n_cols >= 0, SGF_E_INVALID, "%s: negative size", fn);
  if (n_rows == 0 || d == 0) return SGF_OK;
  SGF_REQUIRE(rowptr && x && y, SGF_E_INVALID, "%s: null pointer", fn);
  SGF_REQUIRE(n_rows < (static_cast<int64_t>(1) << 31) * kWavesPerBlock, SGF_E_UNSUPPORTED,
              "%s: n_rows too large for one launch", fn);
  if (const int rc = check_spmm_operands(fn, x, ldx, y, ldy, d, dtype)) return rc;
  if (dtype == SGF_F32)
    return launch<float>(rowptr, colind, val, static_cast<const float*>(x), ldx, n_cols, static_cast<float*>(y), ldy,
                         n_rows, d, st, lq, partial, stream);
  return launch<uint16_t>(rowptr, colind, val, static_cast<const uint16_t*>(x), ldx, n_cols,
                          static_cast<uint16_t*>(y), ldy, n_rows, d, st, lq, partial, stream);
}
}

extern "C" int sgf_spmm(const int64_t* rowptr, const int32_t* colind, const float* val,
                        const void* x, int64_t ldx, int64_t n_cols, void* y, int64_t ldy, int64_t n_rows,
                        int32_t d, int32_t dtype, void* stream) {
  const LongQueue none{nullptr, nullptr, 0, INT64_MAX};
  return spmm_common(rowptr, colind, val, x, ldx, n_cols, y, ldy, n_rows, d, dtype, none, nullptr,
                     static_cast<hipStream_t>(stream), "sgf_spmm");
}

extern "C" int32_t sgf_spmm_segment_len(void) { return kSegLen; }

extern "C" int32_t sgf_spmm_arm(int32_t d, int32_t dtype, int64_t ldx, int64_t ldy, int64_t n_cols, int32_t aligned16,
                                int32_t stream) {
  if (dtype != SGF_F32 && dtype != SGF_BF16) return -1;
  const Choice c = choose_for_operands(d, dtype == SGF_BF16 ? 2 : 4, ldx, ldy, n_cols, aligned16 != 0, stream != 0);
  return static_cast<int32_t>(c.arm) | (c.arm == Arm::Sub ? c.lanes_per_row << 8 : 0);
}

extern "C" size_t sgf_spmm_split_workspace_bytes(int64_t long_segments, int32_t d) {
  if (long_segments < 0 || d < 0) return 0;
  return long_partial_off(long_segments) + static_cast<size_t>(long_segments) * static_cast<size_t>(d) * sizeof(float);
}

int sgf::spmm_long_queue(const char* fn, int64_t long_len, int64_t long_segments, int32_t d, void* workspace,
                         size_t workspace_bytes, hipStream_t st, LongQueue* lq, float** partial) {
  SGF_REQUIRE(long_len >= 1 && long_segments >= 0 && long_segments < (static_cast<int64_t>(1) << 31),
              SGF_E_INVALID, "%s: bad long_len / long_segments", fn);
  *lq = LongQueue{nullptr, nullptr, 0, INT64_MAX};
  *partial = nullptr;
  if (long_segments == 0) return SGF_OK;
  SGF_REQUIRE(workspace && workspace_bytes >= sgf_spmm_split_workspace_bytes(long_segments, d),
              SGF_E_WORKSPACE, "%s: workspace too small", fn);
  char* ws = static_cast<char*>(workspace);
  lq->count = reinterpret_cast<int32_t*>(ws + kLongCountOff);
  lq->entries = reinterpret_cast<LongEntry*>(ws + kLongEntriesOff);
  lq->cap = static_cast<int32_t>(long_segments);
  lq->long_len = long_len;
  *partial = reinterpret_cast<float*>(ws + long_partial_off(long_segments));
  SGF_CHECK_HIP(hipMemsetAsync(lq->count, 0, sizeof(int32_t), st));
  return SGF_OK;
}

static int spmm_split_impl(bool stream_hint, const char* fn, const int64_t* rowptr, const int32_t* colind, const float* val,
                              const void* x, int64_t ldx, int64_t n_cols, void* y, int64_t ldy, int64_t n_rows,
                              int32_t d, int32_t dtype, int64_t long_len, int64_t long_segments,
                              void* workspace, size_t workspace_bytes, void* stream) {
  hipStream_t st = static_cast<hipStream_t>(stream);
  LongQueue lq;
  float* partial;
  if (const int rc = spmm_long_queue(fn, long_len, long_segments, d, workspace, workspace_bytes, st, &lq, &partial)) return rc;
  return spmm_common(rowptr, colind, val, x, ldx, n_cols, y, ldy, n_rows, d, dtype, lq, partial, st, fn, stream_hint);
}

extern "C" int sgf_spmm_split(const int64_t* rowptr, const int32_t* colind, const float* val, const void* x,
                              int64_t ldx, int64_t n_cols, void* y, int64_t ldy, int64_t n_rows, int32_t d,
                              int32_t dtype, int64_t long_len, int64_t long_segments, void* workspace,
                              size_t workspace_bytes, void* stream) {
  return spmm_split_impl(false, "sgf_spmm_split", rowptr, colind, val, x, ldx, n_cols, y, ldy, n_rows, d, dtype,
                         long_len, long_segments, workspace, workspace_bytes, stream);
}

extern "C" int sgf_spmm_stream(const int64_t* rowptr, const int32_t* colind, const float* val, const void* x,
                               int64_t ldx, int64_t n_cols, void* y, int64_t ldy, int64_t n_rows, int32_t d,
                               int32_t dtype, int64_t long_len, int64_t long_segments, void* workspace,
                               size_t workspace_bytes, void* stream) {
  return spmm_split_impl(true, "sgf_spmm_stream", rowptr, colind, val, x, ldx, n_cols, y, ldy, n_rows, d, dtype,
                         long_len, long_segments, workspace, workspace_bytes, stream);
}

extern "C" int32_t sgf_spmm_lds_rows_len(int32_t dtype) {
  return dtype == SGF_BF16 ? 288 : 144;
}

extern "C" int32_t sgf_spmm_blocked_arm(int32_t d, int32_t dtype, int64_t ldx, int64_t ldy, int64_t n_rows,
                                        int32_t rows_per_block, int32_t lds_rows, int32_t aligned16) {
  if (dtype != SGF_F32 && dtype != SGF_BF16) return -1;
  if (!blk_rows_ok(rows_per_block) || !blk_lds_rows_ok(lds_rows, dtype)) return -1;
  const BlkChoice c = choose_blocked(d, dtype == SGF_BF16 ? 2 : 4, ldx, ldy, n_rows, rows_per_block, lds_rows, aligned16 != 0);
  return c.blk2 ? 0 : c.lean ? 1 : 2;
}

extern "C" int sgf_spmm_blocked(const int64_t* rowptr, const int32_t* ecode, const float* eval,
                                const int32_t* nlds, const int32_t* sh_ptr, const int32_t* sh_cols,
                                const void* x, int64_t ldx, void* y, int64_t ldy, int64_t n_rows, int32_t d,
                                int32_t dtype, int32_t rows_per_block, int32_t lds_rows, int64_t long_len,
                                int64_t long_segments, void* workspace, size_t workspace_bytes, void* stream) {
  const char* fn = "sgf_spmm_blocked";
  SGF_REQUIRE(n_rows >= 0 && d >= 0, SGF_E_INVALID, "%s: negative size", fn);
  if (n_rows == 0 || d == 0) return SGF_OK;
  SGF_REQUIRE(rowptr && ecode && eval && nlds && sh_ptr && sh_cols && x && y, SGF_E_INVALID, "%s: null pointer", fn);
  SGF_REQUIRE(d <= 256, SGF_E_UNSUPPORTED, "%s: d = %d > 256 (one wave per row)", fn, d);
  SGF_REQUIRE(blk_rows_ok(rows_per_block), SGF_E_INVALID, "%s: rows_per_block must be a multiple of %d in [%d, 128]", fn, kBlkRowsPerWave,
              kBlkRowsPerWave);
  SGF_REQUIRE(blk_lds_rows_ok(lds_rows, dtype), SGF_E_INVALID,
              "%s: lds_rows %d outside [1, %d]", fn, lds_rows, sgf_spmm_lds_rows_len(dtype));
  if (const int rc = check_spmm_operands(fn, x, ldx, y, ldy, d, dtype)) return rc;
  hipStream_t st = static_cast<hipStream_t>(stream);
  LongQueue lq;
  float* partial;
  if (const int rc = spmm_long_queue(fn, long_len, long_segments, d, workspace, workspace_bytes, st, &lq, &partial)) return rc;
  if (dtype == SGF_F32)
    return launch_blocked<float>(rowptr, ecode, eval, nlds, sh_ptr, sh_cols, static_cast<const float*>(x), ldx,
                                 static_cast<float*>(y), ldy, n_rows, d, rows_per_block, lds_rows, st, lq, partial);
  return launch_blocked<uint16_t>(rowptr, ecode, eval, nlds, sh_ptr, sh_cols, static_cast<const uint16_t*>(x), ldx,
                                  static_cast<uint16_t*>(y), ldy, n_rows, d, rows_per_block, lds_rows, st, lq, partial);
}
```

sgformer_amd/graph.py:

```python
from __future__ import annotations

import ctypes
from collections import OrderedDict
from typing import Optional

import torch

from . import _lib
from .kernels import (HipKernels, LONG_ROW, _SEGMENT, _code, _ld, _one_pass_cat, _pair_gram, _ptr, _rows,
                      _rows16, _stream, _workspace, _workspaces)

_F32 = torch.float32
_BF16 = torch.bfloat16


K = HipKernels()



SMALL_GRAPH_NNZ = 1 << 23


def long_row_segments(rowptr: torch.Tensor, nnz: Optional[int] = None, max_row_len: Optional[int] = None) -> int:
    if rowptr.numel() <= 1:
# ... 268 lines not shown
    def __init__(self, capacity: int = 4):
        self.capacity = capacity
        self._d: "OrderedDict[tuple, CSRGraph]" = OrderedDict()

    def get(self, edge_index: torch.Tensor, num_nodes: int, factory=None, tag=None):
        key = (edge_index.data_ptr(), edge_index._version, tuple(edge_index.shape),
               tuple(edge_index.stride()), str(edge_index.device), int(num_nodes), tag)
        g = self._d.get(key)
        if g is not None:
            self._d.move_to_end(key)
            return g
        g = (factory or CSRGraph)(edge_index, num_nodes)
        g.edge_index_ref = edge_index
        self._d[key] = g
        while len(self._d) > self.capacity:
            self._d.popitem(last=False)
        return g

    def clear(self):
        self._d.clear()


graph_cache = _GraphCache()


def _sharded_spmm(graph, x, shard, transposed: bool):
    rowptr, colind, val = graph.transposed() if transposed else (graph.rowptr, graph.colind, graph.val)
    long_segments = graph.t_long_segments if transposed else graph.long_segments
    n_local = graph.n_local
    plan = graph.halo(shard, transposed) if hasattr(graph, "halo") else None
    if plan is not None and plan.enabled:
        if plan.n_halo == 0:
            return _own_block_spmm(graph, plan, (rowptr, plan.colind, val, long_segments), x, n_local, transposed)
        if getattr(shard, "overlap", False):
            shard.overlapped_exchanges = getattr(shard, "overlapped_exchanges", 0) + 1
            own, (rp_h, ci_h, va_h, seg_h) = plan.split(rowptr, val, n_local)
            recv, work, keep = shard.halo_exchange_start(x, plan)
            y = _own_block_spmm(graph, plan, own, x, n_local, transposed)
            work.wait()
            y.add_(K.spmm(rp_h, ci_h, va_h, recv, n_local, long_segments=seg_h))
            del keep
            return y
        return K.spmm(rowptr, plan.colind, val, shard.halo_exchange(x, plan), n_local, long_segments=long_segments)
    d = x.shape[1]
    chunks = shard.gather_chunks(d)
    if chunks <= 1:
        return K.spmm(rowptr, colind, val, shard.all_gather_rows(x), n_local, long_segments=long_segments)
    w = d // chunks
    pending = [shard.all_gather_rows(x[:, c * w:(c + 1) * w].contiguous(), async_op=True) for c in range(chunks)]
    y = torch.empty((n_local, d), dtype=x.dtype, device=x.device)
    for c, (buf, work) in enumerate(pending):
        work.wait()
        K.spmm(rowptr, colind, val, buf, n_local, out=y[:, c * w:(c + 1) * w], long_segments=long_segments)
    return y


def _own_block_spmm(graph, plan, own, x, n_local: int, transposed: bool):
    rp, ci, va, segs = own
    if getattr(graph, "locality", False):
        import os
        if (hasattr(K, "tile_supported") and K.tile_supported(x.shape[1], x.dtype) and getattr(graph, "comm_local", None) is not None
                and os.environ.get("SGF_SPMM_TILED", "1") == "1" and n_local >= 256
                and x.shape[0] * max(x.stride(0), x.shape[1]) * 2 < 2 ** 32 - 2048):
            plans = plan.__dict__.setdefault("_own_tile_plans", {})
            tp = plans.get("plan")
            if tp is None:
                try:
                    _, _, max_rows = _tile_params()
                    blk_row = K.tile_blocks(graph.comm_local, n_local, max_rows, x.device)
                    tp = TilePlan(rp, ci, va, n_local, blk_row)
                    if tp.tile_fraction < REORDER_MIN_LDS_FRACTION:
                        tp = False
                except (ValueError, _lib.SgfError):
                    tp = False
                plans["plan"] = tp
            if tp:
                return K.spmm_tile(tp, x, n_local)
        return K.spmm(rp, ci, va, x, n_local, long_segments=segs, stream_hint=True)
    return K.spmm(rp, ci, va, x, n_local, long_segments=segs)


class _SpMM(torch.autograd.Function):
    @staticmethod
    def forward(ctx, x, graph, shard):
        K.check(x)
        ctx.graph, ctx.shard = graph, shard
        if shard is not None:
            return _sharded_spmm(graph, x, shard, False)
        return spmm_on(graph, x, False)

    @staticmethod
    def backward(ctx, gy):
        graph, shard = ctx.graph, ctx.shard
        if shard is not None:
            return _sharded_spmm(graph, gy.contiguous(), shard, True), None, None
        return spmm_on(graph, gy.contiguous(), True), None, None


def spmm_on(graph, x: torch.Tensor, transposed: bool, out=None) -> torch.Tensor:
    rp, ci, va = graph.transposed() if transposed else (graph.rowptr, graph.colind, graph.val)
    segs = graph.t_long_segments if transposed else graph.long_segments
    plan = graph.plan(x.dtype, transposed) if (getattr(graph, "blocked", False) and x.shape[1] <= 256) else None
    if plan is not None:
        return K.spmm_blocked(rp, plan, x, graph.n, out=out, long_segments=segs)
    if getattr(graph, "tiled", False):
        if (K.tile_supported(x.shape[1], x.dtype)
                and x.shape[0] * max(x.stride(0), x.shape[1]) * 2 < 2 ** 32 - 2048
                and (out is None or (out.stride(0) % 8 == 0 and out.data_ptr() % 16 == 0))):
            return K.spmm_tile(graph.tile_plan(transposed), x, graph.n, out=out)
        if not K.tile_supported(x.shape[1], x.dtype) and getattr(graph, "_tile_plans", None):
            graph._tile_plans.clear()
    if getattr(graph, "locality", False):
        return K.spmm(rp, ci, va, x, graph.n, out=out, long_segments=segs, stream_hint=True)
    return K.spmm(rp, ci, va, x, graph.n, out=out, long_segments=segs)


def spmm(graph, x: torch.Tensor, shard=None) -> torch.Tensor:
    return _SpMM.apply(x, graph, shard)
```

sgformer_amd/kernels.py:

```python
from __future__ import annotations

import ctypes
from typing import Optional

import torch

from . import _lib

_F32 = torch.float32
_BF16 = torch.bfloat16

LONG_ROW = 1024
_SEGMENT = 1024


def _ptr(t: Optional[torch.Tensor]):
    return None if t is None else ctypes.c_void_p(t.data_ptr())


def _stream(device) -> ctypes.c_void_p:
    return ctypes.c_void_p(torch.cuda.current_stream(device).cuda_stream)


def _code(t: torch.Tensor) -> int:
    if t.dtype == _F32:
        return _lib.SGF_F32
    if t.dtype == _BF16:
        return _lib.SGF_BF16
    raise TypeError(f"sgformer_amd kernels take float32 or bfloat16 storage, got {t.dtype}")


_X3_PRECISIONS = ("high", "medium")


def f32_matmul_code() -> int:
    return _lib.SGF_F32_BF16X3 if torch.get_float32_matmul_precision() in _X3_PRECISIONS else _lib.SGF_F32


_x3_cache: "dict[tuple, bool]" = {}


def _mm_code(t: torch.Tensor, query: Optional[str] = None, *shape) -> int:
    code = _code(t)
    if code != _lib.SGF_F32 or f32_matmul_code() != _lib.SGF_F32_BF16X3:
        return code
    if query is None:
        return _lib.SGF_F32_BF16X3
    key = (query,) + tuple(int(v) for v in shape)
    ok = _x3_cache.get(key)
    if ok is None:
        ok = _x3_cache[key] = bool(getattr(_lib.load(), query)(*key[1:], _lib.SGF_F32_BF16X3))
    return _lib.SGF_F32_BF16X3 if ok else _lib.SGF_F32


def _ld(t: Optional[torch.Tensor]) -> int:
    return 0 if t is None else t.stride(0)


def _rows(t: Optional[torch.Tensor]) -> Optional[torch.Tensor]:
    if t is None:
        return None
    if t.stride(-1) != 1 or t.stride(0) % 4 != 0 or t.data_ptr() % (4 * t.element_size()) != 0:
        t = t.contiguous()
        if t.shape[0] > 1 and t.stride(0) % 4 != 0:
            raise ValueError(f"feature dimension {t.shape[-1]} must be a multiple of 4")
    return t


_workspaces: "dict[tuple, torch.Tensor]" = {}


_capture_scope = None


def begin_capture_scope() -> dict:
    global _capture_scope
    _capture_scope = {}
    return _capture_scope


def end_capture_scope():
    global _capture_scope
    _capture_scope = None


class SeedBank:

    def __init__(self, device, capacity: int = 64):
        self.seeds = torch.zeros(int(capacity), dtype=torch.int64, device=device)
        self.used = 0

    def take(self) -> int:
        if self.used >= self.seeds.numel():
            raise RuntimeError(f"sgformer_amd: more than {self.seeds.numel()} dropout calls in one captured step")
        self.used += 1
        return self.used - 1
# ... 126 lines not shown
                t = 0 if bad else int(t)
                colind_b = torch.empty(t, dtype=torch.int32, device=dev)
                val_b = torch.empty(t, dtype=_F32, device=dev)
                ei_b = torch.empty((2, t), dtype=torch.int64, device=dev) if want_edges else None
                ws2 = _workspace(dev, "subgraph_csr_emit", lib.sgf_subgraph_csr_emit_workspace_bytes(m, t))
            except BaseException:
                local_of.fill_(-1)
                raise
            _lib.call("sgf_subgraph_csr_emit", _ptr(rowptr), _ptr(colind), n, _ptr(subset), m, _ptr(local_of), _ptr(rowptr_b),
                      _ptr(deg_b), t, _ptr(colind_b), _ptr(val_b), _ptr(ei_b), _ptr(ws2), ws2.numel(), _stream(dev))
        if bad:
            return None
        return rowptr_b, colind_b, val_b, deg_b[:m], ei_b, int(longest)

    @staticmethod
    def sampled_csr_supported(max_fanout: int) -> bool:
        return bool(_lib.load().sgf_sampled_csr_supported(int(max_fanout)))

    @staticmethod
    def sampled_csr_build(e_src: torch.Tensor, e_dst: torch.Tensor, counts: torch.Tensor, node_cap: int, edge_cap: int,
                          max_fanout: int):
        dev = e_src.device
        rowptr_b = torch.empty(node_cap + 1, dtype=torch.int64, device=dev)
        colind_b = torch.empty(max(edge_cap, 1), dtype=torch.int32, device=dev)
        val_b = torch.empty(max(edge_cap, 1), dtype=_F32, device=dev)
        deg_b = torch.empty(node_cap + 1, dtype=torch.int32, device=dev)
        ws = _workspace(dev, "sampled_csr_build", _lib.load().sgf_sampled_csr_build_workspace_bytes(node_cap, edge_cap))
        with torch.cuda.device(dev):
            _lib.call("sgf_sampled_csr_build", _ptr(e_src), _ptr(e_dst), _ptr(counts), node_cap, edge_cap, int(max_fanout),
                      _ptr(rowptr_b), _ptr(colind_b), _ptr(val_b), _ptr(deg_b), _ptr(ws), ws.numel(), _stream(dev))
        return rowptr_b, colind_b, val_b, deg_b

    @staticmethod
    def sampled_csr_transpose(rowptr, colind, val, n: int):
        dev, nnz = rowptr.device, int(colind.numel())
        t_rowptr = torch.empty(n + 1, dtype=torch.int64, device=dev)
        t_colind = torch.empty(nnz, dtype=torch.int32, device=dev)
        t_val = torch.empty(nnz, dtype=_F32, device=dev)
        ws = _workspace(dev, "sampled_csr_transpose", _lib.load().sgf_sampled_csr_transpose_workspace_bytes(n, nnz))
        with torch.cuda.device(dev):
            _lib.call("sgf_sampled_csr_transpose", _ptr(rowptr), _ptr(colind), _ptr(val), n, nnz, _ptr(t_rowptr), _ptr(t_colind),
                      _ptr(t_val), _ptr(ws), ws.numel(), _stream(dev))
        return t_rowptr, t_colind, t_val

    @staticmethod
    def graph_prologue(ei: torch.Tensor, n: int, undirected: bool, remove_loops: bool, add_loops: bool):
        dev, m = ei.device, int(ei.shape[1])
        lib = _lib.load()
        total = torch.zeros(1, dtype=torch.int64, device=dev)
        ws = torch.empty(max(lib.sgf_graph_prologue_workspace_bytes(m, n), 256), dtype=torch.uint8, device=dev)
        with torch.cuda.device(dev):
            _lib.call("sgf_graph_prologue_plan", _ptr(ei), m, n, int(undirected), int(remove_loops), int(add_loops),
                      _ptr(total), _ptr(ws), ws.numel(), _stream(dev))
            k = int(total.item())
            out = torch.empty((2, k), dtype=torch.int64, device=dev)
            _lib.call("sgf_graph_prologue_emit", m, n, int(undirected), int(add_loops), k, _ptr(out), _ptr(ws),
                      ws.numel(), _stream(dev))
        return out

    @staticmethod
    def spmm(rowptr, colind, val, x: torch.Tensor, n_rows: int, out: Optional[torch.Tensor] = None,
             long_segments: int = 0, stream_hint: bool = False) -> torch.Tensor:
        x = _rows(x)
        d = x.shape[1]
        y = torch.empty((n_rows, d), dtype=x.dtype, device=x.device) if out is None else out
        if out is not None and (out.shape != (n_rows, d) or out.dtype != x.dtype or out.stride(1) != 1
                                or out.stride(0) % 4 != 0 or out.data_ptr() % (4 * out.element_size()) != 0):
            raise ValueError("spmm: `out` must be [n_rows, d], same dtype, row-contiguous and 4-element aligned")
        if n_rows == 0 or d == 0:
            return y
        with torch.cuda.device(x.device):
            if long_segments > 0 or stream_hint:
                ws = (_workspace(x.device, "spmm_long", _lib.load().sgf_spmm_split_workspace_bytes(long_segments, d))
                      if long_segments > 0 else None)
                _lib.call("sgf_spmm_stream" if stream_hint else "sgf_spmm_split", _ptr(rowptr), _ptr(colind), _ptr(val), _ptr(x), x.stride(0), x.shape[0],
                          _ptr(y), y.stride(0), n_rows, d, _code(x), LONG_ROW, long_segments, _ptr(ws),
                          0 if ws is None else ws.numel(), _stream(x.device))
            else:
                _lib.call("sgf_spmm", _ptr(rowptr), _ptr(colind), _ptr(val), _ptr(x), x.stride(0), x.shape[0],
                          _ptr(y), y.stride(0), n_rows, d, _code(x), _stream(x.device))
        return y

    @staticmethod
    def reorder(ei: torch.Tensor, n: int, iters1: int, iters2: int):
        dev, nnz = ei.device, int(ei.shape[1])
        perm = torch.empty(n, dtype=torch.int32, device=dev)
        inv = torch.empty(n, dtype=torch.int32, device=dev)
        comm = torch.empty(n, dtype=torch.int32, device=dev)
        nbytes = _lib.load().sgf_reorder_workspace_bytes(nnz, n)
        ws = torch.empty(max(nbytes, 256), dtype=torch.uint8, device=dev)
        with torch.cuda.device(dev):
            _lib.call("sgf_reorder", _ptr(ei), nnz, n, int(iters1), int(iters2), _ptr(perm), _ptr(inv),
                      _ptr(comm), _ptr(ws), ws.numel(), _stream(dev))
        return perm, inv, comm

    @staticmethod
    def spmm_plan(rowptr, colind, val, n: int, rows_per_block: int, lds_rows: int, long_len: int):
        dev, nnz = rowptr.device, int(colind.numel())
        nb = (n + rows_per_block - 1) // rows_per_block
        ecode = torch.empty(nnz, dtype=torch.int32, device=dev)
        ev = torch.empty(nnz, dtype=_F32, device=dev)
        nlds = torch.empty(max(n, 1), dtype=torch.int32, device=dev)
        sh_ptr = torch.empty(nb + 1, dtype=torch.int32, device=dev)
        sh_cols = torch.empty(max(nb * lds_rows, 1), dtype=torch.int32, device=dev)
        stats = torch.zeros(4, dtype=torch.int64, device=dev)
        nbytes = _lib.load().sgf_spmm_plan_workspace_bytes(nnz, n, rows_per_block)
        ws = torch.empty(max(nbytes, 256), dtype=torch.uint8, device=dev)
        with torch.cuda.device(dev):
            _lib.call("sgf_spmm_plan", _ptr(rowptr), _ptr(colind), _ptr(val), n, nnz, int(rows_per_block),
                      int(lds_rows), int(long_len), _ptr(ecode), _ptr(ev), _ptr(nlds), _ptr(sh_ptr),
                      _ptr(sh_cols), _ptr(stats), _ptr(ws), ws.numel(), _stream(dev))
        st = [int(v) for v in stats.tolist()]
        return ecode, ev, nlds, sh_ptr, sh_cols[: max(st[1], 1)].clone(), st

    @staticmethod
    def spmm_blocked(rowptr, plan, x: torch.Tensor, n_rows: int, out: Optional[torch.Tensor] = None,
                     long_segments: int = 0) -> torch.Tensor:
        x = _rows(x)
        d = x.shape[1]
        y = torch.empty((n_rows, d), dtype=x.dtype, device=x.device) if out is None else out
        if n_rows == 0 or d == 0:
            return y
        with torch.cuda.device(x.device):
            ws = None
            if long_segments > 0:
                ws = _workspace(x.device, "spmm_long", _lib.load().sgf_spmm_split_workspace_bytes(long_segments, d))
            _lib.call("sgf_spmm_blocked", _ptr(rowptr), _ptr(plan.ecode), _ptr(plan.eval), _ptr(plan.nlds),
                      _ptr(plan.sh_ptr), _ptr(plan.sh_cols), _ptr(x), x.stride(0), _ptr(y), y.stride(0), n_rows, d,
                      _code(x), plan.rows_per_block, plan.lds_rows, LONG_ROW, long_segments, _ptr(ws),
                      0 if ws is None else ws.numel(), _stream(x.device))
        return y

    @staticmethod
    def tile_supported(d: int, dtype) -> bool:
        return bool(_lib.load().sgf_spmm_tile_supported(int(d), _lib.SGF_BF16 if dtype == _BF16 else _lib.SGF_F32))

    @staticmethod
    def tile_blocks(comm_sorted: Optional[torch.Tensor], n: int, max_rows: int, device) -> torch.Tensor:
        cap = 4 * n // int(max_rows) + 4
        blk = torch.empty(cap + 1, dtype=torch.int32, device=device)
        nb = ctypes.c_int64(0)
        with torch.cuda.device(device):
            _lib.call("sgf_spmm_tile_blocks", _ptr(comm_sorted), n, int(max_rows), _ptr(blk), cap, ctypes.byref(nb),
                      _stream(device))
        return blk[: nb.value + 1].clone()

    @staticmethod
    def tile_plan(rowptr, colind, val, n: int, blk_row: torch.Tensor, cap: int, min_count: int, long_len: int):
        dev, nnz, nb = rowptr.device, int(colind.numel()), int(blk_row.numel()) - 1
        ecode = torch.empty(max(nnz, 1), dtype=torch.int32, device=dev)
        ev = torch.empty(max(nnz, 1), dtype=_F32, device=dev)
        nlds = torch.empty(max(n, 1), dtype=torch.int32, device=dev)
        sh_ptr = torch.empty(nb + 1, dtype=torch.int32, device=dev)
        sh_cols = torch.empty(max(nb * cap, 1), dtype=torch.int32, device=dev)
        tile_ptr = torch.empty(nb + 1, dtype=torch.int64, device=dev)
        rem_rowptr = torch.empty(n + 1, dtype=torch.int64, device=dev)
        stats = torch.zeros(8, dtype=torch.int64, device=dev)
        nbytes = _lib.load().sgf_spmm_tile_plan_workspace_bytes(nnz, n, nb)
        ws = torch.empty(max(nbytes, 256), dtype=torch.uint8, device=dev)
        with torch.cuda.device(dev):
            _lib.call("sgf_spmm_tile_plan", _ptr(rowptr), _ptr(colind), _ptr(val), n, nnz, _ptr(blk_row), nb, int(cap),
                      int(min_count), int(long_len), _ptr(ecode), _ptr(ev), _ptr(nlds), _ptr(sh_ptr), _ptr(sh_cols),
                      _ptr(tile_ptr), _ptr(rem_rowptr), _ptr(stats), _ptr(ws), ws.numel(), _stream(dev))
            st = [int(v) for v in stats.tolist()]
            del ws
            if st[7]:
# ... 254 lines not shown
        dev = a.device
        if out is None:
            out = torch.empty((m, k), dtype=_F32, device=dev)
        cs = torch.empty(m, dtype=_F32, device=dev) if want_colsum else None
        ws = _workspace(dev, "attn", _lib.load().sgf_gram_workspace_bytes(n, m, k))
        with torch.cuda.device(dev):
            _lib.call("sgf_gram", _ptr(a), _ld(a), m, _ptr(b), _ld(b), k, n, _mm_code(a), _ptr(out),
                      out.stride(0), _ptr(cs), _ptr(ws), ws.numel(), _stream(dev))
        return out, cs

    @staticmethod
    def gram2(a, b1, b2, out1, out2, want_colsum=True):
        n, m = a.shape
        k = b1.shape[1]
        dev = a.device
        cs = torch.empty(m, dtype=_F32, device=dev) if want_colsum else None
        ws = _workspace(dev, "attn", _lib.load().sgf_gram_workspace_bytes(n, m, k))
        with torch.cuda.device(dev):
            _lib.call("sgf_gram2", _ptr(a), _ld(a), m, _ptr(b1), _ld(b1), _ptr(b2), _ld(b2), k, n, _mm_code(a), _ptr(out1),
                      out1.stride(0), _ptr(out2), out2.stride(0), _ptr(cs), _ptr(ws), ws.numel(), _stream(dev))
        return cs

    @staticmethod
    def ln_fwd(x, res, a: float, b: float, gamma, beta, relu: bool, eps: float):
        n, d = x.shape
        dev = x.device
        y = torch.empty((n, d), dtype=x.dtype, device=dev)
        mean = torch.empty(n, dtype=_F32, device=dev) if gamma is not None else None
        rstd = torch.empty(n, dtype=_F32, device=dev) if gamma is not None else None
        with torch.cuda.device(dev):
            _lib.call("sgf_ln_fwd", _ptr(x), _ld(x), _ptr(res), _ld(res), float(a), float(b),
                      _ptr(gamma), _ptr(beta), int(relu), float(eps), n, d, _code(x), _ptr(y),
                      y.stride(0), _ptr(mean), _ptr(rstd), _stream(dev))
        return y, mean, rstd

    @staticmethod
    def ln_bwd(gy, y, x, res, a: float, b: float, gamma, relu: bool, mean, rstd):
        n, d = x.shape
        dev = x.device
        dx = torch.empty_like(x)
        shared = res is not None and float(a) == float(b)
        dres = torch.empty_like(res) if (res is not None and not shared) else None
        dgamma = torch.empty(d, dtype=_F32, device=dev) if gamma is not None else None
        dbeta = torch.empty(d, dtype=_F32, device=dev) if gamma is not None else None
        ws = _workspace(dev, "ln", _lib.load().sgf_ln_bwd_workspace_bytes(n, d))
        with torch.cuda.device(dev):
            _lib.call("sgf_ln_bwd", _ptr(gy), _ld(gy), _ptr(y), _ld(y), _ptr(x), _ld(x), _ptr(res),
                      _ld(res), float(a), float(b), _ptr(gamma), int(relu), _ptr(mean), _ptr(rstd), n,
                      d, _code(x), _ptr(dx), _ld(dx), _ptr(dres), _ld(dres), _ptr(dgamma), _ptr(dbeta),
                      _ptr(ws), ws.numel(), _stream(dev))
        return dx, (dx if shared else dres), dgamma, dbeta

    @staticmethod
    def colstats(x, shift) -> torch.Tensor:
        n, d = x.shape
        dev = x.device
        stats = torch.empty(2 * d, dtype=_F32, device=dev)
        ws = _workspace(dev, "col", _lib.load().sgf_colstats_workspace_bytes(n, d))
        with torch.cuda.device(dev):
            _lib.call("sgf_colstats", _ptr(x), _ld(x), _ptr(shift), n, d, _code(x), _ptr(stats),
                      _ptr(ws), ws.numel(), _stream(dev))
        return stats

    @staticmethod
    def bn_finalize(sums, shift, n_total: float, eps: float, momentum: float, running_mean, running_var):
        d = sums.numel() // 2
        mean = torch.empty(d, dtype=_F32, device=sums.device)
        rstd = torch.empty(d, dtype=_F32, device=sums.device)
        with torch.cuda.device(sums.device):
            _lib.call("sgf_bn_finalize", _ptr(sums), _ptr(shift), float(n_total), float(eps), float(momentum),
                      _ptr(running_mean), _ptr(running_var), d, _ptr(mean), _ptr(rstd), _stream(sums.device))
        return mean, rstd

    @staticmethod
    def bn_apply(x, mean, rstd, gamma, beta, res, relu: bool) -> torch.Tensor:
        n, d = x.shape
        dev = x.device
        y = torch.empty((n, d), dtype=x.dtype, device=dev)
        with torch.cuda.device(dev):
            _lib.call("sgf_bn_apply", _ptr(x), _ld(x), _ptr(mean), _ptr(rstd), _ptr(gamma), _ptr(beta),
                      _ptr(res), _ld(res), int(relu), n, d, _code(x), _ptr(y), y.stride(0),
                      _stream(dev))
        return y

    @staticmethod
    def bn_bwd_stats(gy, x, mean, rstd, gamma, beta, relu: bool) -> torch.Tensor:
        n, d = x.shape
        dev = x.device
        stats = torch.empty(2 * d, dtype=_F32, device=dev)
        ws = _workspace(dev, "col", _lib.load().sgf_colstats_workspace_bytes(n, d))
        with torch.cuda.device(dev):
            _lib.call("sgf_bn_bwd_stats", _ptr(gy), _ld(gy), _ptr(x), _ld(x), _ptr(mean), _ptr(rstd),
                      _ptr(gamma), _ptr(beta), int(relu), n, d, _code(x), _ptr(stats), _ptr(ws),
                      ws.numel(), _stream(dev))
        return stats

    @staticmethod
    def bn_bwd_stats2(gy, gy2, x, mean, rstd, gamma, beta, relu: bool) -> torch.Tensor:
        n, d = x.shape
        dev = x.device
        stats = torch.empty(2 * d, dtype=_F32, device=dev)
        ws = _workspace(dev, "col", _lib.load().sgf_colstats_workspace_bytes(n, d))
        with torch.cuda.device(dev):
            _lib.call("sgf_bn_bwd_stats2", _ptr(gy), _ld(gy), _ptr(gy2), _ld(gy2), _ptr(x), _ld(x), _ptr(mean), _ptr(rstd),
                      _ptr(gamma), _ptr(beta), int(relu), n, d, _code(x), _ptr(stats), _ptr(ws), ws.numel(), _stream(dev))
        return stats

    @staticmethod
    def gram_ln_bwd_supported(m: int, k: int, dtype) -> bool:
        return dtype == _BF16 and bool(_lib.load().sgf_gram_ln_bwd_supported(int(m), int(k), _lib.SGF_BF16))

    @staticmethod
    def gram_ln_bwd(g, xin, mean, rstd, gamma, beta, relu: bool, b):
        n, m = xin.shape
        k = b.shape[1]
        dev = xin.device
        out = torch.empty((m, k), dtype=_F32, device=dev)
        cs = torch.empty(m, dtype=_F32, device=dev)
        dg = torch.empty(m, dtype=_F32, device=dev)
        db = torch.empty(m, dtype=_F32, device=dev)
        ws = _workspace(dev, "attn", _lib.load().sgf_gram_workspace_bytes(n, m, k))
        with torch.cuda.device(dev):
            _lib.call("sgf_gram_ln_bwd", _ptr(g), _ld(g), _ptr(xin), _ld(xin), _ptr(mean), _ptr(rstd), _ptr(gamma), _ptr(beta),
                      int(relu), m, _ptr(b), _ld(b), k, n, _code(xin), _ptr(out), out.stride(0), _ptr(cs), _ptr(dg), _ptr(db),
                      _ptr(ws), ws.numel(), _stream(dev))
        return out, cs, dg, db

    @staticmethod
    def gram_bn_bwd_supported(m: int, k: int, dtype) -> bool:
        return dtype == _BF16 and bool(_lib.load().sgf_gram_bn_bwd_supported(int(m), int(k), _lib.SGF_BF16))

    @staticmethod
    def gram_bn_bwd(gy, gy2, z, mean, rstd, gamma, beta, relu: bool, stats, inv_n: float, training: bool, b):
        n, m = z.shape
        k = b.shape[1]
        dev = z.device
        out = torch.empty((m, k), dtype=_F32, device=dev)
        cs = torch.empty(m, dtype=_F32, device=dev)
        ws = _workspace(dev, "attn", _lib.load().sgf_gram_workspace_bytes(n, m, k))
        with torch.cuda.device(dev):
            _lib.call("sgf_gram_bn_bwd", _ptr(gy), _ld(gy), _ptr(gy2), _ld(gy2), _ptr(z), _ld(z), _ptr(mean), _ptr(rstd),
                      _ptr(gamma), _ptr(beta), int(relu), _ptr(stats), float(inv_n), int(training), m, _ptr(b), _ld(b), k, n,
                      _code(z), _ptr(out), out.stride(0), _ptr(cs), _ptr(ws), ws.numel(), _stream(dev))
        return out, cs

    @staticmethod
    def gram2_bn_bwd_supported(g, z, b1, b2) -> bool:
        n, m = z.shape
        ok = all(t.dtype == _BF16 and t.dim() == 2 and t.stride(1) == 1 and t.stride(0) % 8 == 0 and t.data_ptr() % 16 == 0
                 for t in (g, z, b1, b2))
        return (ok and b1.shape == b2.shape and g.shape == z.shape
                and bool(_lib.load().sgf_gram2_bn_bwd_supported(int(m), int(b1.shape[1]), int(n), _lib.SGF_BF16)))

    @staticmethod
    def gram2_bn_bwd(g, z, mean, rstd, gamma, beta, relu: bool, stats, inv_n: float, training: bool, b1, b2, out1, out2):
        n, m = z.shape
        k = b1.shape[1]
        dev = z.device
        dz = torch.empty((n, m), dtype=z.dtype, device=dev)
        cs = torch.empty(m, dtype=_F32, device=dev)
        ws = _workspace(dev, "attn", _lib.load().sgf_gram_workspace_bytes(n, m, k))
        with torch.cuda.device(dev):
            _lib.call("sgf_gram2_bn_bwd", _ptr(g), _ld(g), _ptr(z), _ld(z), _ptr(mean), _ptr(rstd), _ptr(gamma), _ptr(beta),
                      int(relu), _ptr(stats), float(inv_n), int(training), m, _ptr(b1), _ld(b1), _ptr(b2), _ld(b2), k, n,
                      _code(z), _ptr(dz), dz.stride(0), _ptr(out1), out1.stride(0), _ptr(out2), out2.stride(0), _ptr(cs),
                      _ptr(ws), ws.numel(), _stream(dev))
# ... 419 lines not shown
```

sgformer_amd/linear.py:

```python
from __future__ import annotations

import ctypes
from collections import OrderedDict
from typing import Optional

import torch

from . import _lib
from .kernels import (HipKernels, LONG_ROW, _SEGMENT, _code, _ld, _one_pass_cat, _pair_gram, _ptr, _rows,
                      _rows16, _stream, _workspace, _workspaces)

_F32 = torch.float32
_BF16 = torch.bfloat16

from .graph import K


_BN_SAMPLE_ROWS = 1024


def batch_stats(x: torch.Tensor, shard=None):
    K.check(x)
    x = _rows(x.detach())
    n, d = x.shape
# ... 64 lines not shown
        return (dw, db, None, *dxs)


def _linear_param_grads(g, xs, widths, need_w, need_b, wdtype, bdtype):
    dw = db = None
    if need_w or need_b:
        m = g.shape[1]
        gp = _rows(g if m % 4 == 0 else torch.nn.functional.pad(g, (0, 4 - m % 4)))
        dw = torch.empty((gp.shape[1], sum(widths)), dtype=_F32, device=g.device)
        off = 0
        if (len(xs) == 2 and widths[0] == widths[1] and widths[0] % 4 == 0 and hasattr(K, "gram2") and gp.dtype == _BF16
                and xs[0].dtype == _BF16 and xs[1].dtype == _BF16 and _pair_gram()):
            k = widths[0]
            db = K.gram2(gp, _rows(xs[0]), _rows(xs[1]), dw[:, :k], dw[:, k:], want_colsum=need_b)
            xs, widths = [], []
        for i, (x, k) in enumerate(zip(xs, widths)):
            if k % 4 == 0 and off % 4 == 0:
                _, cs = K.gram(gp, _rows(x), out=dw[:, off:off + k], want_colsum=(i == 0 and need_b))
            elif k % 4 == 0:
                blk, cs = K.gram(gp, _rows(x), want_colsum=(i == 0 and need_b))
                dw[:, off:off + k] = blk
            else:
                xp = _rows(torch.nn.functional.pad(x, (0, 4 - k % 4)))
                blk, cs = K.gram(gp, xp, want_colsum=(i == 0 and need_b))
                dw[:, off:off + k] = blk[:, :k]
            if i == 0:
                db = cs
            off += k
        dw = dw[:m].to(wdtype) if need_w else None
        db = db[:m].to(bdtype) if need_b else None
    return dw, db


class _StemPair(torch.autograd.Function):

    @staticmethod
    def forward(ctx, x, w0, b0, w1, b1, stats_req):
        K.check(x)
        dt = x.dtype
        w0c, w1c = w0.to(dt), w1.to(dt)
        f32 = [None if b is None else b.detach().float().contiguous() for b in (b0, b1)]
        d = w0.shape[0]
        shift = None
        if stats_req is not None:
            shard = stats_req.get("shard")
            n = x.shape[0]
            ns = min(n, _BN_SAMPLE_ROWS)
            _, _, st_s = K.stem_pair(x[:ns], w0c, f32[0], None, None, None, want_stats0=True)
            samp = torch.cat([st_s[:d], torch.full((1,), float(ns), dtype=_F32, device=x.device)])
            n_tot = float(n)
            if shard is not None:
                shard.all_reduce(samp)
                n_tot = float(shard.n_global)
            shift = (samp[:d] / samp[d].clamp_min(1.0)).contiguous()
        y0, y1, st = K.stem_pair(x, w0c, f32[0], w1c, f32[1], shift, want_stats0=stats_req is not None)
        if stats_req is not None:
            if shard is not None:
                shard.all_reduce(st)
            m1 = st[:d] / max(n_tot, 1.0)
            stats_req["out"] = (shift + m1, (st[d:] / max(n_tot, 1.0) - m1 * m1).clamp_min_(0.0), n_tot)
        ctx.save_for_backward(x, w0c, w1c)
        ctx.meta = (w0.dtype, None if b0 is None else b0.dtype, w1.dtype, None if b1 is None else b1.dtype)
        return y0, y1

    @staticmethod
    def backward(ctx, g0, g1):
        x, w0c, w1c = ctx.saved_tensors
        wd0, bd0, wd1, bd1 = ctx.meta
        k = [x.shape[1]]
        dw0, db0 = _linear_param_grads(g0.contiguous(), [x], k, ctx.needs_input_grad[1],
                                       ctx.needs_input_grad[2] and bd0 is not None, wd0, bd0)
        dw1, db1 = _linear_param_grads(g1.contiguous(), [x], k, ctx.needs_input_grad[3],
                                       ctx.needs_input_grad[4] and bd1 is not None, wd1, bd1)
        dx = None
        if ctx.needs_input_grad[0]:
            dx = K.gemm(g0.contiguous(), w0c)
            K.gemm(g1.contiguous(), w1c, out=dx, beta=1.0, addend=dx)
        return dx, dw0, db0, dw1, db1, None


class _StemPairBN(torch.autograd.Function):

    @staticmethod
    def forward(ctx, x, w0, b0, w1, b1, gamma, beta, bn_hook, shard, ln_gamma=None, ln_beta=None, ln_cfg=None):
        K.check(x)
        dt = x.dtype
        w0c, w1c = w0.to(dt), w1.to(dt)
        f32 = [None if b is None else b.detach().float().contiguous() for b in (b0, b1)]
        d = w0.shape[0]
        n = x.shape[0]
        want = bn_hook(None)
        shift = None
        if want:
            ns = min(n, _BN_SAMPLE_ROWS)
            _, _, st_s = K.stem_pair(x[:ns], w0c, f32[0], None, None, None, want_stats0=True)
            n_tot = float(n)
            if shard is None:
                shift = st_s[:d] * (1.0 / float(max(ns, 1)))
            else:
                samp = torch.cat([st_s[:d], torch.full((1,), float(ns), dtype=_F32, device=x.device)])
                shard.all_reduce(samp)
                n_tot = float(shard.n_global)
                shift = (samp[:d] / samp[d].clamp_min(1.0)).contiguous()
        y0, y1, st = K.stem_pair(x, w0c, f32[0], w1c, f32[1], shift, want_stats0=want)
        if want:
            if shard is not None:
                shard.all_reduce(st)
            if hasattr(K, "bn_finalize"):
                mean, rstd, n_tot, training = bn_hook(("raw", st, shift, n_tot))
            else:
                m1 = st[:d] / max(n_tot, 1.0)
                mean, rstd, n_tot, training = bn_hook((shift + m1, (st[d:] / max(n_tot, 1.0) - m1 * m1).clamp_min_(0.0), n_tot))
        else:
            mean, rstd, n_tot, training = bn_hook(False)
        g32 = gamma.detach().float().contiguous() if gamma is not None else None
        be32 = beta.detach().float().contiguous() if beta is not None else None
        mean = mean.detach().float().contiguous()
        rstd = rstd.detach().float().contiguous()
        x0 = K.bn_apply(y0, mean, rstd, g32, be32, None, True)
        out1, ln_saved = y1, (None, None, None, None, None)
        if ln_cfg is not None:
            eps, ln_relu, affine = ln_cfg
            lg32 = ln_gamma.detach().float().contiguous() if affine else None
            lb32 = ln_beta.detach().float().contiguous() if affine else None
            out1, lmean, lrstd = K.ln_fwd(_rows(y1), None, 1.0, 0.0, lg32, lb32, bool(ln_relu), float(eps))
            ln_saved = (y1, lmean, lrstd, lg32, lb32)
        ctx.save_for_backward(x, w0c, w1c, y0, g32, be32, mean, rstd, *ln_saved)
        ctx.meta = (w0.dtype, None if b0 is None else b0.dtype, w1.dtype, None if b1 is None else b1.dtype,
                    None if gamma is None else gamma.dtype, bool(training), float(n_tot), shard,
                    None if ln_cfg is None else (bool(ln_cfg[1]), None if ln_gamma is None else ln_gamma.dtype))
        return x0, x0.view_as(x0), out1

    @staticmethod
    def backward(ctx, ga, gb, g1):
        x, w0c, w1c, y0, g32, be32, mean, rstd, y1, lmean, lrstd, lg32, lb32 = ctx.saved_tensors
        wd0, bd0, wd1, bd1, gdt, training, n_tot, shard, ln_meta = ctx.meta
        d = y0.shape[1]
        if ga is None:
            ga, gb = gb, None
        if ga is None:
            ga = torch.zeros_like(y0)
        ga = _rows(ga.contiguous())
        gb = None if gb is None else _rows(gb.contiguous())
        stats = K.bn_bwd_stats2(ga, gb, y0, mean, rstd, g32, be32, True)
        if shard is not None:
            shard.all_reduce(stats)
        inv_n = 1.0 / max(n_tot, 1.0)
        dw0, db0 = K.gram_bn_bwd(ga, gb, y0, mean, rstd, g32, be32, True, stats, inv_n, training, _rows(x))
        dw0 = dw0.to(wd0) if ctx.needs_input_grad[1] else None
        db0 = db0.to(bd0) if (ctx.needs_input_grad[2] and bd0 is not None) else None
        dlg = dlb = None
        if ln_meta is not None:
            ln_relu, lgdt = ln_meta
            dw1, db1, dlg, dlb = K.gram_ln_bwd(_rows(g1.contiguous()), y1, lmean, lrstd, lg32, lb32, ln_relu, _rows(x))
            dw1 = dw1.to(wd1) if ctx.needs_input_grad[3] else None
            db1 = db1.to(bd1) if (ctx.needs_input_grad[4] and bd1 is not None) else None
            dlg, dlb = (dlg.to(lgdt), dlb.to(lgdt)) if lg32 is not None else (None, None)
        else:
            dw1, db1 = _linear_param_grads(g1.contiguous(), [x], [x.shape[1]], ctx.needs_input_grad[3],
                                           ctx.needs_input_grad[4] and bd1 is not None, wd1, bd1)
        dgamma = stats[d:].to(gdt) if g32 is not None else None
        dbeta = stats[:d].to(gdt) if be32 is not None else None
        if shard is not None and g32 is not None:
            dgamma, dbeta = shard.unsum(dgamma), shard.unsum(dbeta)
        dx = None
        if ctx.needs_input_grad[0]:
            g = ga if gb is None else ga + gb
            dz = K.bn_bwd_apply(g, y0, mean, rstd, g32, be32, True, stats, inv_n, training)
            gl = g1
            if ln_meta is not None:
                gl = K.ln_bwd(_rows(g1.contiguous()), None, y1, None, 1.0, 0.0, lg32, False, lmean, lrstd)[0] \
                    if not ln_meta[0] else None
                if gl is None:
                    raise NotImplementedError("features that require a gradient behind the fused LayerNorm stem: set "
                                              "SGF_STEM_LN_FUSED=0")
            dx = K.gemm(dz, w0c)
            K.gemm(gl.contiguous(), w1c, out=dx, beta=1.0, addend=dx)
        return dx, dw0, db0, dw1, db1, dgamma, dbeta, None, None, dlg, dlb, None


def stem_pair_bn_supported(x, w0, w1) -> bool:
    return (stem_pair_supported(x, w0, w1) and hasattr(K, "gram_bn_bwd_supported")
            and K.gram_bn_bwd_supported(w0.shape[0], x.shape[1], x.dtype))


def stem_pair_bn(x, w0, b0, w1, b1, gamma, beta, bn_hook, shard=None, ln=None):
    if ln is None:
        return _StemPairBN.apply(x, w0, b0, w1, b1, gamma, beta, bn_hook, shard)
    lg, lb, eps, relu = ln
    return _StemPairBN.apply(x, w0, b0, w1, b1, gamma, beta, bn_hook, shard, lg, lb, (eps, relu, lg is not None))


def stem_ln_supported(x, w1) -> bool:
    import os
    return (hasattr(K, "gram_ln_bwd_supported") and K.gram_ln_bwd_supported(w1.shape[0], x.shape[1], x.dtype)
            and not x.requires_grad and os.environ.get("SGF_STEM_LN_FUSED", "1") != "0")


def stem_pair_supported(x, w0, w1) -> bool:
    return (x.dim() == 2 and x.shape[0] > 0 and w0.shape == w1.shape and x.stride(-1) == 1
            and (x.stride(0) * x.element_size()) % 8 == 0 and x.data_ptr() % 8 == 0
            and K.stem_pair_supported(x.shape[1], w0.shape[0], x.dtype))


def stem_pair(x, w0, b0, w1, b1, want_stats0=False, shard=None):
    req = {"shard": shard, "out": None} if want_stats0 else None
    y0, y1 = _StemPair.apply(x, w0, b0, w1, b1, req)
    return (y0, y1), (req["out"] if req is not None else None)


def _streaming_linear_ok(x: torch.Tensor, wc: torch.Tensor, dx: bool = False) -> bool:
    return (x.dim() == 2 and x.shape[0] > 0 and wc.stride(-1) == 1 and (wc.stride(0) * wc.element_size()) % 16 == 0
            and wc.data_ptr() % 16 == 0 and x.shape[1] == (wc.shape[0] if dx else wc.shape[1])
            and K.gcn_epilogue_supported(wc.shape[1], wc.shape[0], x.dtype))


def _streaming_linear(xr, wc, b32, shift=None, want_stats=False, rows=None):
    xs = xr if rows is None else [x[:rows] for x in xr]
    if len(xs) == 1:
        return K.gcn_epilogue_stats(xs[0], wc, b32, shift, want_stats=want_stats)
    return K.gcn_epilogue_cat(xs[0], xs[1], wc, b32, shift, want_stats=want_stats)


def _linear_with_stats(xr, wc, b32, stats_req):
    shard = stats_req.get("shard")
    n, d = xr[0].shape[0], wc.shape[0]
    ns = min(n, _BN_SAMPLE_ROWS)
    _, st_s = _streaming_linear(xr, wc, b32, None, want_stats=True, rows=ns)
    n_tot = float(n)
    if shard is None:
        shift = st_s[:d] * (1.0 / float(max(ns, 1)))
    else:
        samp = torch.cat([st_s[:d], torch.full((1,), float(ns), dtype=_F32, device=xr[0].device)])
        shard.all_reduce(samp)
        n_tot = float(shard.n_global)
        shift = (samp[:d] / samp[d].clamp_min(1.0)).contiguous()
    y, st = _streaming_linear(xr, wc, b32, shift, want_stats=True)
    if shard is not None:
        shard.all_reduce(st)
    if stats_req.get("raw"):
        stats_req["out"] = ("raw", st, shift, n_tot)
        return y
    m1 = st[:d] / max(n_tot, 1.0)
    stats_req["out"] = (shift + m1, (st[d:] / max(n_tot, 1.0) - m1 * m1).clamp_min_(0.0), n_tot)
    return y


class GradChain:

    def __init__(self):
        self.acc = None
        self.parts = []


def _fused_bwd() -> bool:
    import os
    return os.environ.get("SGF_GCN_BWD_FUSED", "0") == "1"


def _acc_in_place(d: int, dtype) -> bool:
    import os
    return (hasattr(K, "gcn_epilogue_dx2_acc_supported") and K.gcn_epilogue_dx2_acc_supported(d, dtype)
            and os.environ.get("SGF_GCN_DX_ACC", "1") != "0")


def gcn_layer_fused_ok(x0: torch.Tensor, w: torch.Tensor) -> bool:
    import os
    d = x0.shape[1] if x0.dim() == 2 else 0
    return (x0.dim() == 2 and x0.shape[0] > 0 and x0.dtype == _BF16 and tuple(w.shape) == (d, 2 * d)
            and hasattr(K, "gcn_bn_bwd_dx_supported") and K.gcn_bn_bwd_dx_supported(d, x0.dtype)
            and os.environ.get("SGF_GCN_FUSED", "1") != "0")


class _LinearBNActRes(torch.autograd.Function):

    @staticmethod
    def forward(ctx, y, x0, w, b, gamma, beta, bn_hook, relu: bool, use_res: bool, shard, chain, first: bool):
        K.check(y, x0)
        dt = x0.dtype
        wc = w.detach().to(dt).contiguous()
        b32 = None if b is None else b.detach().float().contiguous()
        yr, xr = _rows16(y), _rows16(x0)
        want = bn_hook(None)
        if want:
            req = {"shard": shard, "out": None, "raw": hasattr(K, "bn_finalize")}
            z = _linear_with_stats([yr, xr], wc, b32, req)
            mean, rstd, n_tot, training = bn_hook(req["out"])
        else:
            z, _ = _streaming_linear([yr, xr], wc, b32)
            mean, rstd, n_tot, training = bn_hook(False)
        g32 = gamma.detach().float().contiguous() if gamma is not None else None
        be32 = beta.detach().float().contiguous() if beta is not None else None
        mean = mean.detach().float().contiguous()
        rstd = rstd.detach().float().contiguous()
        out = K.bn_apply(z, mean, rstd, g32, be32, xr if use_res else None, relu)
        ctx.save_for_backward(yr, xr, z, wc, g32, be32, mean, rstd)
        ctx.meta = (bool(relu), bool(use_res), bool(training), float(n_tot), shard, chain, bool(first), w.dtype,
                    None if b is None else b.dtype, None if gamma is None else gamma.dtype)
        return out

    @staticmethod
    def backward(ctx, gout):
        yr, xr, z, wc, g32, be32, mean, rstd = ctx.saved_tensors
        relu, use_res, training, n_tot, shard, chain, first, wdt, bdt, gdt = ctx.meta
        d = z.shape[1]
        gout = _rows16(gout.contiguous())
        stats = K.bn_bwd_stats(gout, z, mean, rstd, g32, be32, relu)
        if shard is not None:
            shard.all_reduce(stats)
        inv_n = 1.0 / max(n_tot, 1.0)
        if _fused_bwd():
            dz, dy, acc = K.gcn_bn_bwd_dx(gout, z, mean, rstd, g32, be32, relu, stats, inv_n, training, wc, chain.acc,
                                          last=first, add_gy=use_res)
            chain.acc = None if first else acc
            dx0 = acc if first else None
        else:
            fused_dw = None
            if (ctx.needs_input_grad[2] and hasattr(K, "gram2_bn_bwd_supported") and _pair_gram()
                    and K.gram2_bn_bwd_supported(gout, z, yr, xr)):
                dwf = torch.empty((d, 2 * d), dtype=_F32, device=z.device)
                dz, dbf = K.gram2_bn_bwd(gout, z, mean, rstd, g32, be32, relu, stats, inv_n, training, yr, xr, dwf[:, :d], dwf[:, d:])
                fused_dw = (dwf.to(wdt), dbf.to(bdt) if (ctx.needs_input_grad[3] and bdt is not None) else None)
            else:
                dz = K.bn_bwd_apply(gout, z, mean, rstd, g32, be32, relu, stats, inv_n, training)
            if _acc_in_place(d, dz.dtype) and not chain.parts:
                dy, chain.acc = K.gcn_epilogue_dx2_acc(dz, wc, _rows16(gout) if use_res else None, chain.acc)
                dx0 = None
                if first:
                    dx0, chain.acc = chain.acc, None
            else:
                dy, dxi = K.gcn_epilogue_dx2(dz, wc[:, :d], wc[:, d:], True)
                chain.parts.append(dxi)
                if use_res:
                    chain.parts.append(gout)
                dx0 = None
                if first:
                    parts, chain.parts = chain.parts, []
                    if chain.acc is not None:
                        parts.append(chain.acc)
                        chain.acc = None
                    dx0 = parts[0] if len(parts) == 1 else (K.sum_n(parts) if len(parts) <= 8 else sum(parts[1:], parts[0]))
        if not _fused_bwd() and fused_dw is not None:
            dw, db = fused_dw
        else:
            dw, db = _linear_param_grads(dz, [yr, xr], [d, d], ctx.needs_input_grad[2],
                                         ctx.needs_input_grad[3] and bdt is not None, wdt, bdt)
        dgamma = stats[d:].to(gdt) if g32 is not None else None
        dbeta = stats[:d].to(gdt) if be32 is not None else None
        if shard is not None and g32 is not None:
            dgamma, dbeta = shard.unsum(dgamma), shard.unsum(dbeta)
        return dy, dx0, dw, db, dgamma, dbeta, None, None, None, None, None, None


def linear_bn_act_res(y, x0, w, b, gamma, beta, bn_hook, relu, use_res, shard, chain, first):
    return _LinearBNActRes.apply(y, x0, w, b, gamma, beta, bn_hook, relu, use_res, shard, chain, first)


def linear(x, w, b):
    return _Linear.apply(w, b, None, x)


def linear_bn_stats(xs, w, b, shard=None):
    req = {"shard": shard, "out": None}
    xs = xs if isinstance(xs, (tuple, list)) else (xs,)
    y = _Linear.apply(w, b, req, *xs)
    return y, req["out"]


def linear_cat(xs, w, b):
    return _Linear.apply(w, b, None, *xs)


def out_linear_cat(xs, w, b):
    m = w.shape[0]
    if (xs[0].dtype == _F32 and xs[0].is_cuda and m % 4 != 0
            and all(K.gcn_epilogue_supported(x.shape[1], (m + 3) // 4 * 4, _F32) for x in xs)):
        pad = (m + 3) // 4 * 4 - m
        wp = torch.nn.functional.pad(w, (0, 0, 0, pad))
        bp = None if b is None else torch.nn.functional.pad(b, (0, pad))
        return _Linear.apply(wp, bp, None, *xs)[:, :m]
    return _Linear.apply(w, b, None, *xs)


def out_linear(x, w, b):
    m = w.shape[0]
    if (x.dtype == _F32 and x.is_cuda and x.dim() == 2 and m % 4 != 0
            and K.gcn_epilogue_supported(w.shape[1], (m + 3) // 4 * 4, _F32)):
        pad = (m + 3) // 4 * 4 - m
        wp = torch.nn.functional.pad(w, (0, 0, 0, pad))
        bp = None if b is None else torch.nn.functional.pad(b, (0, pad))
        return _Linear.apply(wp, bp, None, x)[:, :m]
    if x.dtype == _BF16 and x.dim() == 2 and m % 8 != 0 and not K.gcn_epilogue_supported(w.shape[1], m, _BF16):
        pad = (m + 7) // 8 * 8 - m
        wp = torch.nn.functional.pad(w, (0, 0, 0, pad))
        bp = None if b is None else torch.nn.functional.pad(b, (0, pad))
        return _Linear.apply(wp, bp, None, x)[:, :m]
    return _Linear.apply(w, b, None, x)
```

sgformer_amd/ours.py:

```python
from __future__ import annotations

import torch
import torch.nn as nn
import torch.nn.functional as F

from . import ops

__all__ = ["GraphConvLayer", "GraphConv", "TransConvLayer", "TransConv", "SGFormer",
           "full_attention_conv"]

_NO_SHARD = None

DEFAULT_COMPUTE_DTYPE = None

import os as _os
OVERLAP_BRANCHES = _os.environ.get("SGF_OVERLAP", "1") == "1"
OVERLAP_MIN_NODES = 65536
_side_streams = {}


def _side_stream(device):
    s = _side_streams.get(device.index)
    if s is None:
        s = _side_streams[device.index] = torch.cuda.Stream(device=device)
    return s


class _Holder:
    _x_cache = None


import weakref as _weakref
_entry_cache = _weakref.WeakKeyDictionary()


def _stem_w(lin: nn.Linear, x):
    f = lin.weight.shape[1]
    pad = x.shape[1] - f
    if pad != 0 and x.shape[1] not in ((f + 3) // 4 * 4, (f + 7) // 8 * 8):
        raise RuntimeError(f"input has {x.shape[1]} features, the layer expects {f}")
    return lin.weight if pad == 0 else F.pad(lin.weight, (0, pad))


def _entry_width(f: int, cdt) -> int:
    q = 8 if cdt == torch.bfloat16 else 4
    return (f + q - 1) // q * q


def _lin(x, lin: nn.Linear):
    return ops.linear(x, _stem_w(lin, x), lin.bias)


def _drop(x, p, training, res=None):
    if training and p is not None and p > 0.0:
        if x.dim() == 2 and x.shape[1] % 4 == 0:
            return ops.dropout_res(x, res, float(p))
        x = F.dropout(x, p=p, training=True)
        return x if res is None else x + res
    if p is None:
        raise TypeError("dropout probability is None (pass --trans_dropout / --gnn_dropout)")
    return x if res is None else x + res


def full_attention_conv(qs, ks, vs, output_attn=False, shard=None):
    n, h, d = qs.shape
    qk = torch.cat([qs.reshape(n, h * d), ks.reshape(n, h * d)], dim=1)
    if vs.shape[1] == h:
        qkv = torch.cat([qk, vs.reshape(n, h * d)], dim=1)
        out = ops.attention(qkv, None, h, d, shard, per_head=h > 1)
    else:
        out = ops.attention(qk, vs.reshape(n, d), h, d, shard, per_head=h > 1)
    out = out.reshape(n, h, d)
    if output_attn:
        return out, _attention_matrix(qs, ks)
    return out


def _attention_matrix(qs, ks):
    n = qs.shape[0]
    qn = qs / torch.norm(qs, p=2)
    kn = ks / torch.norm(ks, p=2)
    attention = torch.einsum("nhm,lhm->nlh", qn, kn).mean(dim=-1)
    normalizer = (torch.einsum("nhm,hm->nh", qn, kn.sum(dim=0)) + n).mean(dim=-1, keepdim=True)
    return attention / normalizer


def _uses_batch_stats(module: nn.Module, bn: nn.BatchNorm1d) -> bool:
    return module.training or not bn.track_running_stats or bn.running_mean is None


class GraphConvLayer(nn.Module):

    def __init__(self, in_channels, out_channels, use_weight=True, use_init=False):
        super().__init__()
        self.use_init = use_init
        self.use_weight = use_weight
        in_channels_ = 2 * in_channels if use_init else in_channels
        self.W = nn.Linear(in_channels_, out_channels)
        self._shard = _NO_SHARD

    def reset_parameters(self):
        self.W.reset_parameters()

    def propagate(self, x, edge_index):
        shard = self._shard
        if isinstance(edge_index, ops.CSRGraph):
            graph = edge_index
        elif shard is not None and not shard.local_graph:
            graph = shard.graph_for(edge_index)
        else:
            graph = ops.graph_cache.get(edge_index, x.shape[0])
        return ops.spmm(graph, x, None if (shard is not None and shard.local_graph) else shard)

    def forward(self, x, edge_index, x0, bn_stats=False):
        shard = self._shard
        y = self.propagate(x, edge_index)
        if self.use_init:
            if bn_stats:
                return ops.linear_bn_stats((y, x0), self.W.weight, self.W.bias, shard)
            y = ops.linear_cat((y, x0), self.W.weight, self.W.bias)
        elif self.use_weight:
            if bn_stats:
                return ops.linear_bn_stats(y, self.W.weight, self.W.bias, shard)
            y = _lin(y, self.W)
        return (y, None) if bn_stats else y


class GraphConv(nn.Module):

    def __init__(self, in_channels, hidden_channels, num_layers=2, dropout=0.5, use_bn=True,
                 use_residual=True, use_weight=True, use_init=False, use_act=True):
        super().__init__()
        self.convs = nn.ModuleList()
        self.fcs = nn.ModuleList()
        self.fcs.append(nn.Linear(in_channels, hidden_channels))
        self.bns = nn.ModuleList()
        self.bns.append(nn.BatchNorm1d(hidden_channels))
        for _ in range(num_layers):
            self.convs.append(GraphConvLayer(hidden_channels, hidden_channels, use_weight, use_init))
            self.bns.append(nn.BatchNorm1d(hidden_channels))
        self.dropout = dropout
        self.activation = F.relu
        self.use_bn = use_bn
        self.use_residual = use_residual
        self.use_act = use_act
        self._shard = _NO_SHARD

    def reset_parameters(self):
        for conv in self.convs:
            conv.reset_parameters()
        for bn in self.bns:
            bn.reset_parameters()
        for fc in self.fcs:
            fc.reset_parameters()

    def _bn_act_res(self, bn: nn.BatchNorm1d, x, res, relu, stats=None):
        shard = self._shard
        use_batch = _uses_batch_stats(self, bn)
        if use_batch:
            mean, var, n_tot = stats if stats is not None else ops.batch_stats(x, shard)
            if n_tot <= 1 and self.training:
                raise ValueError("Expected more than 1 value per channel when training")
            if self.training and bn.track_running_stats and bn.running_mean is not None:
                with torch.no_grad():
                    bn.num_batches_tracked += 1
                    m = bn.momentum if bn.momentum is not None else 1.0 / float(bn.num_batches_tracked)
                    bn.running_mean.mul_(1.0 - m).add_(mean.to(bn.running_mean.dtype), alpha=m)
                    unbiased = var * (n_tot / max(n_tot - 1.0, 1.0))
                    bn.running_var.mul_(1.0 - m).add_(unbiased.to(bn.running_var.dtype), alpha=m)
        else:
            mean, var, n_tot = bn.running_mean.float(), bn.running_var.float(), float(x.shape[0])
        rstd = torch.rsqrt(var + bn.eps)
        return ops.bn_act_res(x, res, bn.weight, bn.bias, mean, rstd, relu, use_batch, n_tot, shard)

    def _bn_hook(self, bn: nn.BatchNorm1d):
        def hook(stats):
            use_batch = _uses_batch_stats(self, bn)
            if stats is None:
                return use_batch
            if use_batch and stats[0] == "raw":
                _, sums, shift, n_tot = stats
                if n_tot <= 1 and self.training:
                    raise ValueError("Expected more than 1 value per channel when training")
                track = self.training and bn.track_running_stats and bn.running_mean is not None
                if track and bn.momentum is not None and bn.running_mean.dtype == torch.float32:
                    with torch.no_grad():
                        bn.num_batches_tracked += 1
                        mean, rstd = ops.K.bn_finalize(sums, shift, n_tot, bn.eps, float(bn.momentum), bn.running_mean,
                                                       bn.running_var)
                    return mean, rstd, n_tot, True
                if not track:
                    mean, rstd = ops.K.bn_finalize(sums, shift, n_tot, bn.eps, 0.0, None, None)
                    return mean, rstd, n_tot, True
                d = sums.numel() // 2
                m1 = sums[:d] / max(n_tot, 1.0)
                stats = ((shift + m1) if shift is not None else m1, (sums[d:] / max(n_tot, 1.0) - m1 * m1).clamp_min_(0.0),
                         n_tot)
            if use_batch:
                mean, var, n_tot = stats
                if n_tot <= 1 and self.training:
                    raise ValueError("Expected more than 1 value per channel when training")
                if self.training and bn.track_running_stats and bn.running_mean is not None:
                    with torch.no_grad():
                        bn.num_batches_tracked += 1
                        m = bn.momentum if bn.momentum is not None else 1.0 / float(bn.num_batches_tracked)
                        bn.running_mean.mul_(1.0 - m).add_(mean.to(bn.running_mean.dtype), alpha=m)
                        unbiased = var * (n_tot / max(n_tot - 1.0, 1.0))
                        bn.running_var.mul_(1.0 - m).add_(unbiased.to(bn.running_var.dtype), alpha=m)
            else:
                mean, var, n_tot = bn.running_mean.float(), bn.running_var.float(), 0.0
            return mean, torch.rsqrt(var + bn.eps), n_tot, use_batch
        return hook

    def fused_stem_ok(self, x) -> bool:
        import os
        d = self.fcs[0].out_features
        drop_on = self.training and self.dropout is not None and self.dropout > 0.0
        return (self.use_bn and not drop_on and len(self.convs) > 0 and all(c.use_init for c in self.convs)
                and x.dim() == 2 and x.dtype == torch.bfloat16
                and all(tuple(c.W.weight.shape) == (d, 2 * d) for c in self.convs)
                and hasattr(ops.K, "gcn_bn_bwd_dx_supported") and ops.K.gcn_bn_bwd_dx_supported(d, x.dtype)
                and os.environ.get("SGF_GCN_FUSED", "1") != "0" and os.environ.get("SGF_STEM_FUSED", "1") != "0")

    def _fused_layers(self, x0):
        drop_on = self.training and self.dropout is not None and self.dropout > 0.0
        return (self.use_bn and not drop_on and len(self.convs) > 0 and all(c.use_init for c in self.convs)
                and all(ops.gcn_layer_fused_ok(x0, c.W.weight) for c in self.convs))

    def _stage(self, bn, x, res, relu, stats=None):
        drop_on = self.training and self.dropout is not None and self.dropout > 0.0
        fuse_res = res is not None and not drop_on
        if self.use_bn:
            x = self._bn_act_res(bn, x, res if fuse_res else None, relu, stats)
        else:
            if relu:
                x = torch.relu(x)
            if fuse_res:
                x = x + res
        return _drop(x, self.dropout, self.training, res if (res is not None and not fuse_res) else None)

    def forward(self, x, edge_index, stem=None):
        ops._require_cuda(x, None if isinstance(edge_index, ops.CSRGraph) else edge_index)
        x_first = None
        if stem is not None and len(stem) == 3:
            _, x, x_first = stem
        else:
            if stem is not None:
                x, stats0 = stem
            else:
                x, stats0 = _lin(x, self.fcs[0]), None
            x = self._stage(self.bns[0], x, None, True, stats0)
        if self._fused_layers(x):
            x0, chain = x, ops.GradChain()
            if x_first is not None:
                x = x_first
            for i, conv in enumerate(self.convs):
                bn = self.bns[i + 1]
                y = conv.propagate(x, edge_index)
                x = ops.linear_bn_act_res(y, x0, conv.W.weight, conv.W.bias, bn.weight, bn.bias, self._bn_hook(bn),
                                          self.use_act, self.use_residual, self._shard, chain, i == 0)
            return x
        uses_init = [c.use_init for c in self.convs]
        k = 1 + sum(uses_init) + (len(self.convs) if self.use_residual else 0)
        hub = list(ops.fan_out(x, k)) if k <= 8 else [x] * k
        x = hub.pop()
        for i, conv in enumerate(self.convs):
            want = self.use_bn and _uses_batch_stats(self, self.bns[i + 1])
            x0 = hub.pop() if uses_init[i] else None
            if want:
                x, stats = conv(x, edge_index, x0, bn_stats=True)
            else:
                x, stats = conv(x, edge_index, x0), None
            x = self._stage(self.bns[i + 1], x, hub.pop() if self.use_residual else None, self.use_act, stats)
        return x


class TransConvLayer(nn.Module):

    def __init__(self, in_channels, out_channels, num_heads, use_weight=True):
        super().__init__()
        self.Wk = nn.Linear(in_channels, out_channels * num_heads)
        self.Wq = nn.Linear(in_channels, out_channels * num_heads)
        if use_weight:
            self.Wv = nn.Linear(in_channels, out_channels * num_heads)
        self.out_channels = out_channels
        self.num_heads = num_heads
        self.use_weight = use_weight
        self._shard = _NO_SHARD

    def reset_parameters(self):
        self.Wk.reset_parameters()
        self.Wq.reset_parameters()
        if self.use_weight:
            self.Wv.reset_parameters()

    def _project(self, query_input, source_input):
        ws = [self.Wq.weight, self.Wk.weight] + ([self.Wv.weight] if self.use_weight else [])
        bs = [self.Wq.bias, self.Wk.bias] + ([self.Wv.bias] if self.use_weight else [])
        if query_input is source_input:
            return ops.linear(query_input, torch.cat(ws, 0), torch.cat(bs, 0))
        q = ops.linear(query_input, ws[0], bs[0])
        kv = ops.linear(source_input, torch.cat(ws[1:], 0), torch.cat(bs[1:], 0))
        return torch.cat([q, kv], 1)

    def forward(self, query_input, source_input, output_attn=False, grad_tap=None):
        ops._require_cuda(query_input, source_input)
        h, d = self.num_heads, self.out_channels
        if (h == 1 and query_input is source_input and not output_attn and query_input.shape[1] == d
                and d % 4 == 0 and d <= 256):
            wv, bv = (self.Wv.weight, self.Wv.bias) if self.use_weight else (None, None)
            return ops.attention_from_input(query_input, self.Wq.weight, self.Wq.bias, self.Wk.weight,
                                            self.Wk.bias, wv, bv, self._shard, tap=grad_tap)
        qkv = self._project(query_input, source_input)
        v_ext = None
        if not self.use_weight:
            if source_input.shape[1] != d:
                raise RuntimeError(f"use_weight=False needs in_channels == out_channels ({d})")
            v_ext = source_input
        final_output = ops.attention(qkv, v_ext, h, d, self._shard)
        if output_attn:
            n = qkv.shape[0]
            qs = qkv[:, :h * d].reshape(n, h, d)
            ks = qkv[:, h * d:2 * h * d].reshape(n, h, d)
            return final_output, _attention_matrix(qs, ks)
        return final_output


class TransConv(nn.Module):

    def __init__(self, in_channels, hidden_channels, num_layers=2, num_heads=1, dropout=0.5,
                 use_bn=True, use_residual=True, use_weight=True, use_act=True, alpha=None,
                 layer_cls=None):
        super().__init__()
        layer_cls = layer_cls or TransConvLayer
        self.convs = nn.ModuleList()
        self.fcs = nn.ModuleList()
        self.fcs.append(nn.Linear(in_channels, hidden_channels))
        self.bns = nn.ModuleList()
        self.bns.append(nn.LayerNorm(hidden_channels))
        for _ in range(num_layers):
            self.convs.append(layer_cls(hidden_channels, hidden_channels, num_heads=num_heads,
                                        use_weight=use_weight))
            self.bns.append(nn.LayerNorm(hidden_channels))
# ... 93 lines not shown
            self.fc = nn.Linear(2 * hidden_channels, out_channels)
        else:
            raise ValueError(f'Invalid aggregate type:{aggregate}')
        self.params1 = list(self.trans_conv.parameters())
        self.params2 = list(self.graph_conv.parameters()) if self.graph_conv is not None else []
        self.params2.extend(list(self.fc.parameters()))

    def _forward_on_gpu_from_host(self, x, edge_index):
        if not torch.cuda.is_available():
            ops._require_cuda(x)
        if torch.is_grad_enabled():
            raise RuntimeError("sgformer_amd: CPU tensors with autograd enabled — there is no CPU fallback "
                               "and training runs on MI355X only; move the model and inputs to the GPU")
        dev = torch.device("cuda", torch.cuda.current_device())
        state = {k: v.to(dev) for k, v in list(self.named_parameters()) + list(self.named_buffers())}
        out = torch.func.functional_call(self, state, (x.to(dev), edge_index.to(dev)))
        for k, v in self.named_buffers():
            v.copy_(state[k])
        return out.to(x.device)

    def forward(self, x, edge_index):
        if not x.is_cuda and ops.K.name == "hip" and not next(self.parameters()).is_cuda:
            return self._forward_on_gpu_from_host(x, edge_index)
        ops._require_cuda(x, edge_index)
        out_dtype = x.dtype if getattr(self, 'logits_dtype', None) is None else self.logits_dtype
        cdt = self.compute_dtype if self.compute_dtype is not None else x.dtype
        if getattr(edge_index, "_sgf_csr", None) is not None:
            from . import graphed
            out = graphed.maybe_step(self, x, edge_index, cdt, out_dtype)
            if out is not None:
                return out
        view = None
        if self.use_graph and self.graph_conv._shard is None and ops.K.name == "hip":
            view = ops.graph_cache.get(edge_index, x.shape[0]).view()
            edge_index = view.graph
        repart = None
        shard = self.graph_conv._shard if self.use_graph else None
        if shard is not None and not shard.local_edges and not shard.local_graph:
            repart = shard.repartition_for(edge_index)
            if repart is not None:
                x, edge_index = repart.to_new(x), repart.edge_index
        perm = view.perm if view is not None else None
        f = x.shape[1]
        fp = _entry_width(f, cdt)
        pad = fp != f and not x.requires_grad and hasattr(ops.K, "pad_rows")
        if x.requires_grad:
            if perm is not None:
                x = ops.permute_rows(x, view.perm, view.inv, cdt)
            elif x.dtype != cdt:
                x = x.to(cdt)
        elif perm is not None or pad or x.dtype != cdt:
            holder = view if view is not None else _entry_cache.setdefault(self, _Holder())
            key = (x.data_ptr(), x._version, tuple(x.shape), x.dtype, cdt, bool(pad), perm is not None)
            hit = getattr(holder, "_x_cache", None)
            if hit is None or hit[0] != key:
                if pad:
                    xe = ops.K.pad_rows(x, perm, fp, cdt)
                elif perm is not None:
                    xe = ops.permute_rows(x, view.perm, view.inv, cdt)
                else:
                    xe = x.to(cdt)
                hit = (key, xe, x)
                holder._x_cache = hit
            x = hit[1]
        return self._core(x, edge_index, view, repart, out_dtype)

    def _entry_copy_uncached(self, x, cdt):
        f = x.shape[1]
        fp = _entry_width(f, cdt)
        if fp != f and hasattr(ops.K, "pad_rows"):
            return ops.K.pad_rows(x, None, fp, cdt)
        return x if x.dtype == cdt else x.to(cdt)

    def _core(self, x, edge_index, view, repart, out_dtype):
        stem_t = stem_g = None
        gc, tc = (self.graph_conv if self.use_graph else None), self.trans_conv
        both = gc is not None and hasattr(tc, "fcs") and hasattr(gc, "fcs") and hasattr(gc, "bns")
        wg, wt = (_stem_w(gc.fcs[0], x), _stem_w(tc.fcs[0], x)) if both else (None, None)
        if both and gc.fused_stem_ok(x) and ops.stem_pair_bn_supported(x, wg, wt):
            bn0 = gc.bns[0]
            ln = None
            if getattr(tc, "use_bn", False) and hasattr(tc, "bns") and ops.stem_ln_supported(x, wt):
                ln = (tc.bns[0].weight, tc.bns[0].bias, tc.bns[0].eps, True)
            x0a, x0b, yt = ops.stem_pair_bn(x, wg, gc.fcs[0].bias, wt, tc.fcs[0].bias,
                                            bn0.weight, bn0.bias, gc._bn_hook(bn0), gc._shard, ln)
            stem_t, stem_g = (("ln", yt) if ln is not None else yt), ("bn", x0a, x0b)
        elif both and ops.stem_pair_supported(x, wg, wt):
            want = gc.use_bn and _uses_batch_stats(gc, gc.bns[0])
            (yg, yt), st = ops.stem_pair(x, wg, gc.fcs[0].bias, wt, tc.fcs[0].bias,
                                         want_stats0=want, shard=gc._shard)
            stem_t, stem_g = yt, (yg, st)
        if (self.use_graph and self.overlap_branches and ops.K.name == "hip" and self.graph_conv._shard is None
                and x.shape[0] >= OVERLAP_MIN_NODES and not torch.cuda.is_current_stream_capturing() and not ops._fused_bwd()):
            cur = torch.cuda.current_stream(x.device)
            side = _side_stream(x.device)
            side.wait_stream(cur)
            with torch.cuda.stream(side):
                x1 = self.trans_conv(x) if stem_t is None else self.trans_conv(x, stem=stem_t)
            x.record_stream(side)
            for t in (stem_t if isinstance(stem_t, (tuple, list)) else (stem_t,)):
                if torch.is_tensor(t):
                    t.record_stream(side)
            x2 = self.graph_conv(x, edge_index) if stem_g is None else self.graph_conv(x, edge_index, stem=stem_g)
            cur.wait_stream(side)
            x1.record_stream(cur)
        else:
            x1 = self.trans_conv(x) if stem_t is None else self.trans_conv(x, stem=stem_t)
            if self.use_graph:
                x2 = self.graph_conv(x, edge_index) if stem_g is None else self.graph_conv(x, edge_index, stem=stem_g)
            else:
                x2 = None
        if self.use_graph and self.aggregate == 'add' and ops.combine_fc_supported(x1, self.fc.out_features):
            gw = float(self.graph_weight)
            if (view is not None and view.perm is not None and repart is None
                    and ops.combine_fc_mapped_supported(x1, self.fc.out_features)):
                out = ops.combine_fc(x2, x1, self.fc.weight, self.fc.bias, gw, 1.0 - gw, view.perm).to(out_dtype)
                view = None
            else:
                out = ops.combine_fc(x2, x1, self.fc.weight, self.fc.bias, gw, 1.0 - gw).to(out_dtype)
        else:
            if self.use_graph and self.aggregate != 'add':
                out = ops.out_linear_cat((x1, x2), self.fc.weight, self.fc.bias).to(out_dtype)
            else:
                if self.use_graph:
                    gw = float(self.graph_weight)
                    x = ops.axpby(x2, x1, gw, 1.0 - gw)
                else:
                    x = x1
                out = ops.out_linear(x, self.fc.weight, self.fc.bias).to(out_dtype)
        if view is not None and view.perm is not None:
            out = ops.permute_rows(out, view.inv, view.perm)
        if repart is not None:
            out = repart.to_old(out)
        return out

    def get_attentions(self, x):
        return self.trans_conv.get_attentions(x)

    def reset_parameters(self):
        self.trans_conv.reset_parameters()
        if self.use_graph:
            self.graph_conv.reset_parameters()
```

Measured before the change: 29.16 million.

## Gather SpMM rows from sparsity-packed ReLU output written by BN apply

The BN-apply kernel now also writes a compressed copy of each bf16 row of width 256: a per-row nonzero bitmask followed by the packed nonzero values in a fixed-size slot, and it counts rows whose nonzeros do not fit. A new SpMM kernel gathers neighbor rows from these packed slots, rebuilding values with popcount prefix sums, DPP and byte permutes. Rows that overflow fall back to the dense source. The goal is to cut SpMM gather bandwidth after ReLU, where many entries are zero, at the cost of an extra write in BN apply, more ALU work per gathered element, and a dependent second load per neighbor. It is enabled only for the first layer by default (slot 384).

```diff
diff --git a/include/sgf.h b/include/sgf.h
--- a/include/sgf.h
+++ b/include/sgf.h
@@ -8,7 +8,7 @@
 extern "C" {
 #endif
 
-#define SGF_VERSION 662
+#define SGF_VERSION 663
 
 #define SGF_F32 0
 #define SGF_BF16 1
@@ -71,6 +71,14 @@
                    int64_t ldx, int64_t n_cols, void* y, int64_t ldy, int64_t n_rows, int32_t d, int32_t dtype,
                    int64_t long_len, int64_t long_segments, void* workspace, size_t workspace_bytes,
                    void* stream);
+
+size_t sgf_spmm_packed_bytes(int64_t n, int32_t slot_bytes);
+int32_t sgf_spmm_packed_supported(int32_t d, int32_t dtype, int64_t ldx, int64_t ldy, int64_t n_cols, int32_t aligned16,
+                                  int32_t slot_bytes);
+int sgf_spmm_packed(const int64_t* rowptr, const int32_t* colind, const float* val, const void* x, int64_t ldx,
+                    int64_t n_cols, const void* packed, int32_t slot_bytes, const int32_t* overflow, void* y, int64_t ldy,
+                    int64_t n_rows, int32_t d, int32_t dtype, int64_t long_len, int64_t long_segments, void* workspace,
+                    size_t workspace_bytes, void* stream);
 
 int sgf_spmm_stream(const int64_t* rowptr, const int32_t* colind, const float* val, const void* x,
                     int64_t ldx, int64_t n_cols, void* y, int64_t ldy, int64_t n_rows, int32_t d, int32_t dtype,
@@ -253,6 +261,9 @@
                  const float* gamma, const float* beta, const void* res, int64_t ldr,
                  int32_t relu, int64_t n, int32_t d, int32_t dtype, void* y, int64_t ldy,
                  void* stream);
+int sgf_bn_apply_packed(const void* x, int64_t ldx, const float* mean, const float* rstd, const float* gamma,
+                        const float* beta, const void* res, int64_t ldr, int32_t relu, int64_t n, int32_t d, int32_t dtype,
+                        void* y, int64_t ldy, void* packed, int32_t slot_bytes, int32_t* overflow, void* stream);
 int sgf_bn_bwd_stats(const void* dy, int64_t lddy, const void* x, int64_t ldx, const float* mean,
                      const float* rstd, const float* gamma, const float* beta, int32_t relu,
                      int64_t n, int32_t d, int32_t dtype, float* stats, void* workspace,
diff --git a/sgformer_amd/_lib.py b/sgformer_amd/_lib.py
--- a/sgformer_amd/_lib.py
+++ b/sgformer_amd/_lib.py
@@ -42,6 +42,10 @@
     "sgf_spmm_split_workspace_bytes": (c_size_t, [c_int64, c_int32]),
     "sgf_spmm_split": (c_int32, [_P, _P, _P, _P, c_int64, c_int64, _P, c_int64, c_int64, c_int32, c_int32, c_int64,
                                  c_int64, _P, c_size_t, _P]),
+    "sgf_spmm_packed_bytes": (c_size_t, [c_int64, c_int32]),
+    "sgf_spmm_packed_supported": (c_int32, [c_int32, c_int32, c_int64, c_int64, c_int64, c_int32, c_int32]),
+    "sgf_spmm_packed": (c_int32, [_P, _P, _P, _P, c_int64, c_int64, _P, c_int32, _P, _P, c_int64, c_int64, c_int32, c_int32,
+                                  c_int64, c_int64, _P, c_size_t, _P]),
     "sgf_spmm_stream": (c_int32, [_P, _P, _P, _P, c_int64, c_int64, _P, c_int64, c_int64, c_int32, c_int32, c_int64,
                                   c_int64, _P, c_size_t, _P]),
     "sgf_reorder_workspace_bytes": (c_size_t, [c_int64, c_int64]),
@@ -136,6 +140,8 @@
     "sgf_bn_finalize": (c_int32, [_P, _P, c_double, c_float, c_float, _P, _P, c_int32, _P, _P, _P]),
     "sgf_bn_apply": (c_int32, [_P, c_int64, _P, _P, _P, _P, _P, c_int64, c_int32, c_int64, c_int32,
                                c_int32, _P, c_int64, _P]),
+    "sgf_bn_apply_packed": (c_int32, [_P, c_int64, _P, _P, _P, _P, _P, c_int64, c_int32, c_int64, c_int32, c_int32, _P,
+                                      c_int64, _P, c_int32, _P, _P]),
     "sgf_bn_bwd_stats": (c_int32, [_P, c_int64, _P, c_int64, _P, _P, _P, _P, c_int32, c_int64, c_int32,
                                    c_int32, _P, _P, c_size_t, _P]),
     "sgf_bn_bwd_stats2": (c_int32, [_P, c_int64, _P, c_int64, _P, c_int64, _P, _P, _P, _P, c_int32, c_int64, c_int32,
diff --git a/sgformer_amd/csrc/fused.hip b/sgformer_amd/csrc/fused.hip
--- a/sgformer_amd/csrc/fused.hip
+++ b/sgformer_amd/csrc/fused.hip
@@ -572,6 +572,95 @@
       }
     }
   }
+}
+
+typedef uint16_t __attribute__((may_alias)) ew_u16a;
+typedef uint4 __attribute__((may_alias)) ew_uint4a;
+
+template <bool kRes, int U, int S>
+__global__ __launch_bounds__(kThreads) void k_bn_apply_bf16x8_packed(const uint16_t* __restrict__ x, int64_t ldx, BnParams p,
+                                                                     const uint16_t* __restrict__ res, int64_t ldr, int relu,
+                                                                     int64_t n, uint16_t* __restrict__ y, int64_t ldy,
+                                                                     uint4* __restrict__ packed, int32_t* __restrict__ overflow) {
+  constexpr int kCap = (S - 32) / 2;
+  constexpr int kQ = S / 16;
+  constexpr int rpp = kThreads / 32;
+  __shared__ __align__(16) unsigned char stage[rpp][S];
+  const int q = threadIdx.x & 31;
+  const int sr = threadIdx.x >> 5;
+  const int col = q * 8;
+  BnCoeffs8 c;
+  bn_coeffs8(p, col, c);
+  unsigned char* const slot = stage[sr];
+  int over = 0;
+  const int64_t rpb = static_cast<int64_t>(rpp) * U;
+  for (int64_t row0 = static_cast<int64_t>(blockIdx.x) * rpb + sr; row0 < n; row0 += static_cast<int64_t>(gridDim.x) * rpb) {
+    uint4 xv[U], rv[U];
+#pragma unroll
+    for (int u = 0; u < U; ++u) {
+      const int64_t row = row0 + u * rpp;
+      if (row < n) {
+        xv[u] = *reinterpret_cast<const uint4*>(x + row * ldx + col);
+        if (kRes) rv[u] = *reinterpret_cast<const uint4*>(res + row * ldr + col);
+      }
+    }
+#pragma unroll
+    for (int u = 0; u < U; ++u) {
+      const int64_t row = row0 + u * rpp;
+      const bool live = row < n;
+      uint4 ov = make_uint4(0u, 0u, 0u, 0u);
+      if (live) {
+        float v[8], r[8], o[8];
+        ew_unpack(xv[u], v);
+        if (kRes) ew_unpack(rv[u], r);
+#pragma unroll
+        for (int e = 0; e < 8; ++e) {
+          o[e] = fmaf((v[e] - c.mu[e]) * c.rs[e], c.ga[e], c.be[e]);
+          if (relu) o[e] = fmaxf(o[e], 0.f);
+          if (kRes) o[e] += r[e];
+        }
+        ov = ew_pack8(o);
+        *reinterpret_cast<uint4*>(y + row * ldy + col) = ov;
+      }
+      const uint32_t w[4] = {ov.x, ov.y, ov.z, ov.w};
+      uint32_t m8 = 0;
+#pragma unroll
+      for (int e = 0; e < 8; ++e)
+        if (((w[e >> 1] >> (16 * (e & 1))) & 0xffffu) != 0) m8 |= 1u << e;
+      const int cnt = __popc(m8);
+      int incl = cnt;
+#pragma unroll
+      for (int off = 1; off < 32; off <<= 1) {
+        const int t = __shfl_up(incl, off, 32);
+        if (q >= off) incl += t;
+      }
+      const int total = __shfl(incl, 31, 32);
+      if (live && q == 0 && total > kCap) ++over;
+      if (q < kQ) reinterpret_cast<ew_uint4a*>(slot)[q] = make_uint4(0u, 0u, 0u, 0u);
+      __builtin_amdgcn_fence(__ATOMIC_RELEASE, "wavefront");
+      __builtin_amdgcn_wave_barrier();
+      __builtin_amdgcn_fence(__ATOMIC_ACQUIRE, "wavefront");
+      slot[q] = static_cast<unsigned char>(m8);
+      int pos = incl - cnt;
+#pragma unroll
+      for (int e = 0; e < 8; ++e) {
+        if (m8 & (1u << e)) {
+          if (pos < kCap) *reinterpret_cast<ew_u16a*>(slot + 32 + 2 * pos) = static_cast<uint16_t>(w[e >> 1] >> (16 * (e & 1)));
+          ++pos;
+        }
+      }
+      __builtin_amdgcn_fence(__ATOMIC_RELEASE, "wavefront");
+      __builtin_amdgcn_wave_barrier();
+      __builtin_amdgcn_fence(__ATOMIC_ACQUIRE, "wavefront");
+      if (live && q < kQ) packed[row * kQ + q] = reinterpret_cast<const ew_uint4a*>(slot)[q];
+      __builtin_amdgcn_fence(__ATOMIC_RELEASE, "wavefront");
+      __builtin_amdgcn_wave_barrier();
+      __builtin_amdgcn_fence(__ATOMIC_ACQUIRE, "wavefront");
+    }
+  }
+#pragma unroll
+  for (int off = 32; off > 0; off >>= 1) over += __shfl_xor(over, off, 64);
+  if ((threadIdx.x & 63) == 0 && over > 0) atomicAdd(overflow, over);
 }
 
 template <int U>
@@ -1451,6 +1540,41 @@
     hipLaunchKernelGGL((k_bn_apply<uint16_t>), grid, dim3(kThreads), 0, st,
                        static_cast<const uint16_t*>(x), ldx, p, static_cast<const uint16_t*>(res),
                        ldr, relu, n, d, static_cast<uint16_t*>(y), ldy);
+  SGF_LAUNCH_CHECK();
+  return SGF_OK;
+}
+
+extern "C" int sgf_bn_apply_packed(const void* x, int64_t ldx, const float* mean, const float* rstd, const float* gamma,
+                                   const float* beta, const void* res, int64_t ldr, int32_t relu, int64_t n, int32_t d,
+                                   int32_t dtype, void* y, int64_t ldy, void* packed, int32_t slot_bytes, int32_t* overflow,
+                                   void* stream) {
+  const char* fn = "sgf_bn_apply_packed";
+  SGF_REQUIRE(x && y && mean && rstd && packed && overflow, SGF_E_INVALID, "%s: null pointer", fn);
+  int rc = check_ew(fn, n, d, dtype);
+  if (rc != SGF_OK) return rc;
+  SGF_REQUIRE(dtype == SGF_BF16 && d == 256, SGF_E_UNSUPPORTED, "%s: packed rows are bf16 rows of 256 columns", fn);
+  SGF_REQUIRE(slot_bytes == 384 || slot_bytes == 448, SGF_E_UNSUPPORTED, "%s: slot_bytes must be 384 or 448", fn);
+  SGF_REQUIRE(ldx % 8 == 0 && ldy % 8 == 0 && (!res || ldr % 8 == 0) && reinterpret_cast<uintptr_t>(x) % 16 == 0 &&
+                  reinterpret_cast<uintptr_t>(y) % 16 == 0 && (!res || reinterpret_cast<uintptr_t>(res) % 16 == 0) &&
+                  reinterpret_cast<uintptr_t>(packed) % 128 == 0,
+              SGF_E_INVALID, "%s: rows must be 16-byte aligned, the packed buffer 128-byte aligned", fn);
+  hipStream_t st = static_cast<hipStream_t>(stream);
+  SGF_CHECK_HIP(hipMemsetAsync(overflow, 0, sizeof(int32_t), st));
+  if (n == 0) return SGF_OK;
+  const BnParams p{mean, rstd, gamma, beta};
+  const dim3 g8(rowwalk8_grid(n, d));
+#define SGF_BNP(RES_, S_)                                                                                                 \
+  hipLaunchKernelGGL((k_bn_apply_bf16x8_packed<RES_, kEw8Unroll, S_>), g8, dim3(kThreads), 0, st,                         \
+                     static_cast<const uint16_t*>(x), ldx, p, static_cast<const uint16_t*>(res), ldr, relu, n,            \
+                     static_cast<uint16_t*>(y), ldy, static_cast<uint4*>(packed), overflow)
+  if (res) {
+    if (slot_bytes == 384) SGF_BNP(true, 384);
+    else SGF_BNP(true, 448);
+  } else {
+    if (slot_bytes == 384) SGF_BNP(false, 384);
+    else SGF_BNP(false, 448);
+  }
+#undef SGF_BNP
   SGF_LAUNCH_CHECK();
   return SGF_OK;
 }
diff --git a/sgformer_amd/csrc/spmm.hip b/sgformer_amd/csrc/spmm.hip
--- a/sgformer_amd/csrc/spmm.hip
+++ b/sgformer_amd/csrc/spmm.hip
@@ -176,6 +176,191 @@
   if (i + 2 <= len) { gather_batch<T, 2>(rsrc, voff, pitch, ci, va, i, acc); i += 2; }
   if (i < len) gather_batch<T, 1>(rsrc, voff, pitch, ci, va, i, acc);
   if (active) store4<T>(y + row * ldy + fc, acc);
+}
+
+typedef uint32_t u32x3 __attribute__((ext_vector_type(3)));
+constexpr int kPackedMaskBytes = 32;
+constexpr int kPackedTail = 128;
+
+struct DenseRowLoader {
+  static constexpr bool kAhead = false;
+  __amdgpu_buffer_rsrc_t rsrc;
+  int voff;
+  uint32_t pitch;
+  template <int N> struct Batch { u32x2 raw[N]; };
+  template <int N> __device__ __forceinline__ void request(Batch<N>& b, const int32_t (&c)[N]) const {
+#pragma unroll
+    for (int u = 0; u < N; ++u) b.raw[u] = BufRow<uint16_t>::load(rsrc, voff, static_cast<uint32_t>(c[u]) * pitch);
+  }
+  template <int N> __device__ __forceinline__ void follow(Batch<N>&) const {}
+  template <int N> __device__ __forceinline__ void apply(const Batch<N>& b, const float (&v)[N], float4& acc) const {
+#pragma unroll
+    for (int u = 0; u < N; ++u) fma4(acc, v[u], BufRow<uint16_t>::widen(b.raw[u]));
+  }
+};
+
+template <int S>
+struct PackedRowLoader {
+  static constexpr bool kAhead = true;
+  __amdgpu_buffer_rsrc_t rsrc;
+  int mask_voff;
+  int shift;
+  uint32_t below;
+  const uint4* lut;
+  template <int N> struct Batch {
+    uint32_t slot[N], mw[N], pre[N];
+    u32x3 raw[N];
+  };
+  template <int N> __device__ __forceinline__ void request(Batch<N>& b, const int32_t (&c)[N]) const {
+#pragma unroll
+    for (int u = 0; u < N; ++u) {
+      b.slot[u] = static_cast<uint32_t>(c[u]) * static_cast<uint32_t>(S);
+      b.mw[u] = __builtin_amdgcn_raw_buffer_load_b32(rsrc, mask_voff, static_cast<int>(b.slot[u]), 0);
+    }
+  }
+  template <int N> __device__ __forceinline__ void follow(Batch<N>& b) const {
+#pragma unroll
+    for (int u = 0; u < N; ++u) {
+      const int t = __popc(b.mw[u]);
+      int s = t + __builtin_amdgcn_update_dpp(0, t, 0x118, 0xf, 0xf, true);
+      s += __builtin_amdgcn_update_dpp(0, s, 0x142, 0xa, 0xf, false);
+      s += __builtin_amdgcn_update_dpp(0, s, 0x143, 0xc, 0xf, false);
+      b.pre[u] = static_cast<uint32_t>(s - t) + __popc(b.mw[u] & below);
+      const uint32_t off = ((b.pre[u] & ~1u) << 1) + (b.slot[u] + kPackedMaskBytes);
+      b.raw[u] = __builtin_amdgcn_raw_buffer_load_b96(rsrc, static_cast<int>(off), 0, 0);
+    }
+  }
+  template <int N> __device__ __forceinline__ void apply(const Batch<N>& b, const float (&v)[N], float4& acc) const {
+#pragma unroll
+    for (int u = 0; u < N; ++u) {
+      const uint4 sel = lut[(b.mw[u] >> shift) & 15u];
+      const uint32_t sh = b.pre[u] << 4;
+      const uint32_t lo = __builtin_amdgcn_alignbit(b.raw[u].y, b.raw[u].x, sh);
+      const uint32_t hi = __builtin_amdgcn_alignbit(b.raw[u].z, b.raw[u].y, sh);
+      float4 f;
+      f.x = __uint_as_float(__builtin_amdgcn_perm(hi, lo, sel.x));
+      f.y = __uint_as_float(__builtin_amdgcn_perm(hi, lo, sel.y));
+      f.z = __uint_as_float(__builtin_amdgcn_perm(hi, lo, sel.z));
+      f.w = __uint_as_float(__builtin_amdgcn_perm(hi, lo, sel.w));
+      fma4(acc, v[u], f);
+    }
+  }
+};
+
+template <int N, typename L>
+__device__ __forceinline__ void gather_batch_with(const L& ld, const int32_t* __restrict__ colind,
+                                                  const float* __restrict__ val, int e, float4& acc) {
+  int32_t c[N];
+  float v[N];
+  typename L::template Batch<N> b;
+#pragma unroll
+  for (int u = 0; u < N; ++u) {
+    c[u] = colind[e + u];
+    v[u] = val[e + u];
+  }
+  ld.request(b, c);
+  ld.follow(b);
+  ld.apply(b, v, acc);
+}
+
+template <int UNROLL, typename L>
+__device__ __forceinline__ float4 walk_row(const L& ld, const int32_t* __restrict__ ci, const float* __restrict__ va, int len) {
+  float4 acc = make_float4(0.f, 0.f, 0.f, 0.f);
+  int i = 0;
+  if (UNROLL <= len) {
+    int32_t c0[UNROLL], c1[UNROLL];
+    float v0[UNROLL], v1[UNROLL];
+    typename L::template Batch<UNROLL> ba, bb;
+#pragma unroll
+    for (int u = 0; u < UNROLL; ++u) {
+      c0[u] = ci[u];
+      v0[u] = va[u];
+    }
+    ld.request(ba, c0);
+    for (;;) {
+      i += UNROLL;
+      const bool more_a = i + UNROLL <= len;
+      if (more_a) {
+#pragma unroll
+        for (int u = 0; u < UNROLL; ++u) {
+          c1[u] = ci[i + u];
+          v1[u] = va[i + u];
+        }
+      }
+      ld.follow(ba);
+      if (L::kAhead && more_a) ld.request(bb, c1);
+      ld.apply(ba, v0, acc);
+      if (!more_a) break;
+      if (!L::kAhead) ld.request(bb, c1);
+      i += UNROLL;
+      const bool more_b = i + UNROLL <= len;
+      if (more_b) {
+#pragma unroll
+        for (int u = 0; u < UNROLL; ++u) {
+          c0[u] = ci[i + u];
+          v0[u] = va[i + u];
+        }
+      }
+      ld.follow(bb);
+      if (L::kAhead && more_b) ld.request(ba, c0);
+      ld.apply(bb, v1, acc);
+      if (!more_b) break;
+      if (!L::kAhead) ld.request(ba, c0);
+    }
+  }
+  if (i + 4 <= len) { gather_batch_with<4>(ld, ci, va, i, acc); i += 4; }
+  if (i + 2 <= len) { gather_batch_with<2>(ld, ci, va, i, acc); i += 2; }
+  if (i < len) gather_batch_with<1>(ld, ci, va, i, acc);
+  return acc;
+}
+
+template <int S, int UNROLL>
+__global__ __launch_bounds__(kWavesPerBlock * 64) void k_spmm_row_packed(
+    const int64_t* __restrict__ rowptr, const int32_t* __restrict__ colind, const float* __restrict__ val,
+    const uint16_t* __restrict__ x, uint32_t pitch, uint32_t x_bytes, const void* __restrict__ packed, uint32_t packed_bytes,
+    const int32_t* __restrict__ overflow, uint16_t* __restrict__ y, int64_t ldy, int64_t n_rows, LongQueue lq) {
+  __shared__ uint4 lut[16];
+  if (threadIdx.x < 16) {
+    uint32_t s[4];
+#pragma unroll
+    for (int k = 0; k < 4; ++k) {
+      const uint32_t i = __popc(threadIdx.x & ((1u << k) - 1u));
+      s[k] = (threadIdx.x >> k) & 1u ? ((2u * i + 1u) << 24) | ((2u * i) << 16) | 0x0c0cu : 0x0c0c0c0cu;
+    }
+    lut[threadIdx.x] = make_uint4(s[0], s[1], s[2], s[3]);
+  }
+  __syncthreads();
+  const int lane = threadIdx.x & 63;
+  const int wid = __builtin_amdgcn_readfirstlane(static_cast<int>(threadIdx.x >> 6));
+  const int64_t blk = xcd_remap(blockIdx.x, gridDim.x);
+  const int64_t row = blk * kWavesPerBlock + wid;
+  if (row >= n_rows) return;
+  const int64_t e0 = rowptr[row];
+  const int64_t e1 = rowptr[row + 1];
+  if (e1 - e0 > lq.long_len) {
+    push_long_row(lq, row, e1 - e0, lane, 64);
+    return;
+  }
+  const int32_t* __restrict__ ci = colind + e0;
+  const float* __restrict__ va = val + e0;
+  const int len = static_cast<int>(e1 - e0);
+  float4 acc;
+  if (*overflow == 0) {
+    PackedRowLoader<S> ld;
+    ld.rsrc = __builtin_amdgcn_make_buffer_rsrc(const_cast<void*>(packed), 0, packed_bytes, 0x00020000);
+    ld.mask_voff = (lane >> 3) * 4;
+    ld.shift = (lane & 7) * 4;
+    ld.below = (1u << ld.shift) - 1u;
+    ld.lut = lut;
+    acc = walk_row<UNROLL>(ld, ci, va, len);
+  } else {
+    DenseRowLoader ld;
+    ld.rsrc = __builtin_amdgcn_make_buffer_rsrc(const_cast<uint16_t*>(x), 0, x_bytes, 0x00020000);
+    ld.voff = lane * 8;
+    ld.pitch = pitch;
+    acc = walk_row<UNROLL>(ld, ci, va, len);
+  }
+  store4<uint16_t>(y + row * ldy + lane * 4, acc);
 }
 
 constexpr int kSegRows = 4;
@@ -1083,10 +1268,22 @@
   return choose_kernel(d, elem_size, fits32, pair_ok, stream, g_forced.get());
 }
 
+EnvInt g_packed{"SGF_SPMM_PACKED", 1};
+struct PackedOperand {
+  const void* slots;
+  int32_t slot_bytes;
+  const int32_t* overflow;
+};
+bool packed_rule(const Choice& c, int32_t d, size_t elem_size, int64_t n_cols, int32_t slot_bytes) {
+  return g_packed.get() != 0 && c.arm == Arm::Row && elem_size == 2 && d == 256 &&
+         (slot_bytes == 384 || slot_bytes == 448) &&
+         static_cast<uint64_t>(n_cols) * static_cast<uint64_t>(slot_bytes) + kPackedTail < (static_cast<uint64_t>(1) << 32);
+}
+
 template <typename T>
 int launch(const int64_t* rowptr, const int32_t* colind, const float* val, const T* x, int64_t ldx, int64_t n_cols,
            T* y, int64_t ldy, int64_t n_rows, int32_t d, hipStream_t st, const LongQueue& lq,
-           float* partial, bool stream) {
+           float* partial, bool stream, const PackedOperand* pk = nullptr) {
   constexpr int UNROLL = 8;
   const dim3 block(kWavesPerBlock * 64);
   uint64_t x_bytes;
@@ -1116,6 +1313,18 @@
                          static_cast<uint32_t>(x_bytes), y, ldy, n_rows, d, chunk, lq);
       break;
     case Arm::Row:
+      if (pk && packed_rule(c, d, sizeof(T), n_cols, pk->slot_bytes)) {
+        const uint32_t pk_bytes = static_cast<uint32_t>(n_cols * pk->slot_bytes + 16);
+#define SGF_ROWP(S_)                                                                                                  \
+  hipLaunchKernelGGL((k_spmm_row_packed<S_, UNROLL>), dim3(static_cast<unsigned>(nb)), block, 0, st, rowptr, colind, \
+                     val, reinterpret_cast<const uint16_t*>(x), static_cast<uint32_t>(ldx * sizeof(T)),               \
+                     static_cast<uint32_t>(x_bytes), pk->slots, pk_bytes, pk->overflow, reinterpret_cast<uint16_t*>(y), \
+                     ldy, n_rows, lq)
+        if (pk->slot_bytes == 384) SGF_ROWP(384);
+        else SGF_ROWP(448);
+#undef SGF_ROWP
+        break;
+      }
       hipLaunchKernelGGL((k_spmm_row<T, UNROLL>), dim3(static_cast<unsigned>(nb)), block, 0, st, rowptr, colind,
                          val, x, static_cast<uint32_t>(ldx * sizeof(T)), static_cast<uint32_t>(x_bytes), y, ldy,
                          n_rows, d, lq);
@@ -1182,7 +1391,7 @@
 
 int spmm_common(const int64_t* rowptr, const int32_t* colind, const float* val, const void* x, int64_t ldx,
                 int64_t n_cols, void* y, int64_t ldy, int64_t n_rows, int32_t d, int32_t dtype, const LongQueue& lq,
-                float* partial, hipStream_t st, const char* fn, bool stream = false) {
+                float* partial, hipStream_t st, const char* fn, bool stream = false, const PackedOperand* pk = nullptr) {
   SGF_REQUIRE(n_rows >= 0 && d >= 0 && n_cols >= 0, SGF_E_INVALID, "%s: negative size", fn);
   if (n_rows == 0 || d == 0) return SGF_OK;
   SGF_REQUIRE(rowptr && x && y, SGF_E_INVALID, "%s: null pointer", fn);
@@ -1193,7 +1402,7 @@
     return launch<float>(rowptr, colind, val, static_cast<const float*>(x), ldx, n_cols, static_cast<float*>(y), ldy,
                          n_rows, d, st, lq, partial, stream);
   return launch<uint16_t>(rowptr, colind, val, static_cast<const uint16_t*>(x), ldx, n_cols,
-                          static_cast<uint16_t*>(y), ldy, n_rows, d, st, lq, partial, stream);
+                          static_cast<uint16_t*>(y), ldy, n_rows, d, st, lq, partial, stream, pk);
 }
 }
 
@@ -1255,6 +1464,35 @@
                               size_t workspace_bytes, void* stream) {
   return spmm_split_impl(false, "sgf_spmm_split", rowptr, colind, val, x, ldx, n_cols, y, ldy, n_rows, d, dtype,
                          long_len, long_segments, workspace, workspace_bytes, stream);
+}
+
+extern "C" size_t sgf_spmm_packed_bytes(int64_t n, int32_t slot_bytes) {
+  if (n < 0 || slot_bytes <= 0) return 0;
+  return static_cast<size_t>(n) * static_cast<size_t>(slot_bytes) + kPackedTail;
+}
+
+extern "C" int32_t sgf_spmm_packed_supported(int32_t d, int32_t dtype, int64_t ldx, int64_t ldy, int64_t n_cols,
+                                             int32_t aligned16, int32_t slot_bytes) {
+  if (dtype != SGF_F32 && dtype != SGF_BF16) return 0;
+  const size_t esz = dtype == SGF_BF16 ? 2 : 4;
+  const Choice c = choose_for_operands(d, esz, ldx, ldy, n_cols, aligned16 != 0, false);
+  return packed_rule(c, d, esz, n_cols, slot_bytes) ? 1 : 0;
+}
+
+extern "C" int sgf_spmm_packed(const int64_t* rowptr, const int32_t* colind, const float* val, const void* x, int64_t ldx,
+                               int64_t n_cols, const void* packed, int32_t slot_bytes, const int32_t* overflow, void* y,
+                               int64_t ldy, int64_t n_rows, int32_t d, int32_t dtype, int64_t long_len, int64_t long_segments,
+                               void* workspace, size_t workspace_bytes, void* stream) {
+  const char* fn = "sgf_spmm_packed";
+  SGF_REQUIRE(packed && overflow, SGF_E_INVALID, "%s: null pointer", fn);
+  SGF_REQUIRE(slot_bytes == 384 || slot_bytes == 448, SGF_E_UNSUPPORTED, "%s: slot_bytes must be 384 or 448", fn);
+  SGF_REQUIRE(reinterpret_cast<uintptr_t>(packed) % 128 == 0, SGF_E_INVALID, "%s: the packed buffer must be 128-byte aligned", fn);
+  hipStream_t st = static_cast<hipStream_t>(stream);
+  LongQueue lq;
+  float* partial;
+  if (const int rc = spmm_long_queue(fn, long_len, long_segments, d, workspace, workspace_bytes, st, &lq, &partial)) return rc;
+  const PackedOperand pk{packed, slot_bytes, overflow};
+  return spmm_common(rowptr, colind, val, x, ldx, n_cols, y, ldy, n_rows, d, dtype, lq, partial, st, fn, false, &pk);
 }
 
 extern "C" int sgf_spmm_stream(const int64_t* rowptr, const int32_t* colind, const float* val, const void* x,
diff --git a/sgformer_amd/graph.py b/sgformer_amd/graph.py
--- a/sgformer_amd/graph.py
+++ b/sgformer_amd/graph.py
@@ -374,22 +374,32 @@
 
 class _SpMM(torch.autograd.Function):
     @staticmethod
-    def forward(ctx, x, graph, shard):
+    def forward(ctx, x, graph, shard, packed=None):
         K.check(x)
         ctx.graph, ctx.shard = graph, shard
         if shard is not None:
             return _sharded_spmm(graph, x, shard, False)
-        return spmm_on(graph, x, False)
+        return spmm_on(graph, x, False, packed=packed)
 
     @staticmethod
     def backward(ctx, gy):
         graph, shard = ctx.graph, ctx.shard
         if shard is not None:
-            return _sharded_spmm(graph, gy.contiguous(), shard, True), None, None
-        return spmm_on(graph, gy.contiguous(), True), None, None
-
-
-def spmm_on(graph, x: torch.Tensor, transposed: bool, out=None) -> torch.Tensor:
+            return _sharded_spmm(graph, gy.contiguous(), shard, True), None, None, None
+        return spmm_on(graph, gy.contiguous(), True), None, None, None
+
+
+def _row_kernel_graph(graph) -> bool:
+    return not (getattr(graph, "blocked", False) or getattr(graph, "tiled", False) or getattr(graph, "locality", False))
+
+
+def spmm_packed_slot(graph, x_shape, dtype, slot_bytes: int) -> int:
+    if not slot_bytes or not hasattr(K, "spmm_packed_supported") or not _row_kernel_graph(graph):
+        return 0
+    return slot_bytes if K.spmm_packed_supported(x_shape, dtype, slot_bytes) else 0
+
+
+def spmm_on(graph, x: torch.Tensor, transposed: bool, out=None, packed=None) -> torch.Tensor:
     rp, ci, va = graph.transposed() if transposed else (graph.rowptr, graph.colind, graph.val)
     segs = graph.t_long_segments if transposed else graph.long_segments
     plan = graph.plan(x.dtype, transposed) if (getattr(graph, "blocked", False) and x.shape[1] <= 256) else None
@@ -404,8 +414,12 @@
             graph._tile_plans.clear()
     if getattr(graph, "locality", False):
         return K.spmm(rp, ci, va, x, graph.n, out=out, long_segments=segs, stream_hint=True)
+    if packed is not None and not transposed and out is None:
+        return K.spmm_packed(rp, ci, va, x, packed, graph.n, long_segments=segs)
     return K.spmm(rp, ci, va, x, graph.n, out=out, long_segments=segs)
 
 
-def spmm(graph, x: torch.Tensor, shard=None) -> torch.Tensor:
-    return _SpMM.apply(x, graph, shard)
+def spmm(graph, x: torch.Tensor, shard=None, packed=None) -> torch.Tensor:
+    if packed is None:
+        return _SpMM.apply(x, graph, shard)
+    return _SpMM.apply(x, graph, shard, packed)
diff --git a/sgformer_amd/kernels.py b/sgformer_amd/kernels.py
--- a/sgformer_amd/kernels.py
+++ b/sgformer_amd/kernels.py
@@ -12,6 +12,15 @@
 
 LONG_ROW = 1024
 _SEGMENT = 1024
+
+counters = {"spmm_packed": 0}
+
+
+class PackedRows:
+    __slots__ = ("slots", "slot_bytes", "n", "overflow")
+
+    def __init__(self, slots, slot_bytes, n, overflow):
+        self.slots, self.slot_bytes, self.n, self.overflow = slots, slot_bytes, n, overflow
 
 
 def _ptr(t: Optional[torch.Tensor]):
@@ -304,6 +313,31 @@
         return y
 
     @staticmethod
+    def spmm_packed_supported(x_shape, dtype, slot_bytes: int) -> bool:
+        n, d = int(x_shape[0]), int(x_shape[1])
+        if dtype != torch.bfloat16 or n == 0:
+            return False
+        return bool(_lib.load().sgf_spmm_packed_supported(d, _lib.SGF_BF16, d, d, n, 1, int(slot_bytes)))
+
+    @staticmethod
+    def spmm_packed(rowptr, colind, val, x: torch.Tensor, packed: "PackedRows", n_rows: int, long_segments: int = 0) -> torch.Tensor:
+        x = _rows(x)
+        d = x.shape[1]
+        if packed.n != x.shape[0]:
+            raise ValueError("spmm_packed: the packed copy has another number of rows than x")
+        y = torch.empty((n_rows, d), dtype=x.dtype, device=x.device)
+        if n_rows == 0 or d == 0:
+            return y
+        with torch.cuda.device(x.device):
+            ws = (_workspace(x.device, "spmm_long", _lib.load().sgf_spmm_split_workspace_bytes(long_segments, d))
+                  if long_segments > 0 else None)
+            _lib.call("sgf_spmm_packed", _ptr(rowptr), _ptr(colind), _ptr(val), _ptr(x), x.stride(0), x.shape[0],
+                      _ptr(packed.slots), packed.slot_bytes, _ptr(packed.overflow), _ptr(y), y.stride(0), n_rows, d, _code(x),
+                      LONG_ROW, long_segments, _ptr(ws), 0 if ws is None else ws.numel(), _stream(x.device))
+        counters["spmm_packed"] += 1
+        return y
+
+    @staticmethod
     def reorder(ei: torch.Tensor, n: int, iters1: int, iters2: int):
         dev, nnz = ei.device, int(ei.shape[1])
         perm = torch.empty(n, dtype=torch.int32, device=dev)
@@ -724,6 +758,20 @@
                       _ptr(res), _ld(res), int(relu), n, d, _code(x), _ptr(y), y.stride(0),
                       _stream(dev))
         return y
+
+    @staticmethod
+    def bn_apply_packed(x, mean, rstd, gamma, beta, res, relu: bool, slot_bytes: int):
+        n, d = x.shape
+        dev = x.device
+        y = torch.empty((n, d), dtype=x.dtype, device=dev)
+        nbytes = _lib.load().sgf_spmm_packed_bytes(n, int(slot_bytes))
+        packed = PackedRows(torch.empty(nbytes, dtype=torch.uint8, device=dev), int(slot_bytes), n,
+                            torch.empty(1, dtype=torch.int32, device=dev))
+        with torch.cuda.device(dev):
+            _lib.call("sgf_bn_apply_packed", _ptr(x), _ld(x), _ptr(mean), _ptr(rstd), _ptr(gamma), _ptr(beta),
+                      _ptr(res), _ld(res), int(relu), n, d, _code(x), _ptr(y), y.stride(0), _ptr(packed.slots),
+                      packed.slot_bytes, _ptr(packed.overflow), _stream(dev))
+        return y, packed
 
     @staticmethod
     def bn_bwd_stats(gy, x, mean, rstd, gamma, beta, relu: bool) -> torch.Tensor:
diff --git a/sgformer_amd/linear.py b/sgformer_amd/linear.py
--- a/sgformer_amd/linear.py
+++ b/sgformer_amd/linear.py
@@ -170,7 +170,7 @@
 class _StemPairBN(torch.autograd.Function):
 
     @staticmethod
-    def forward(ctx, x, w0, b0, w1, b1, gamma, beta, bn_hook, shard, ln_gamma=None, ln_beta=None, ln_cfg=None):
+    def forward(ctx, x, w0, b0, w1, b1, gamma, beta, bn_hook, shard, ln_gamma=None, ln_beta=None, ln_cfg=None, pack=None):
         K.check(x)
         dt = x.dtype
         w0c, w1c = w0.to(dt), w1.to(dt)
@@ -205,7 +205,10 @@
         be32 = beta.detach().float().contiguous() if beta is not None else None
         mean = mean.detach().float().contiguous()
         rstd = rstd.detach().float().contiguous()
-        x0 = K.bn_apply(y0, mean, rstd, g32, be32, None, True)
+        if pack is not None:
+            x0, pack["out"] = K.bn_apply_packed(y0, mean, rstd, g32, be32, None, True, pack["slot_bytes"])
+        else:
+            x0 = K.bn_apply(y0, mean, rstd, g32, be32, None, True)
         out1, ln_saved = y1, (None, None, None, None, None)
         if ln_cfg is not None:
             eps, ln_relu, affine = ln_cfg
@@ -264,7 +267,7 @@
                                               "SGF_STEM_LN_FUSED=0")
             dx = K.gemm(dz, w0c)
             K.gemm(gl.contiguous(), w1c, out=dx, beta=1.0, addend=dx)
-        return dx, dw0, db0, dw1, db1, dgamma, dbeta, None, None, dlg, dlb, None
+        return dx, dw0, db0, dw1, db1, dgamma, dbeta, None, None, dlg, dlb, None, None
 
 
 def stem_pair_bn_supported(x, w0, w1) -> bool:
@@ -272,11 +275,11 @@
             and K.gram_bn_bwd_supported(w0.shape[0], x.shape[1], x.dtype))
 
 
-def stem_pair_bn(x, w0, b0, w1, b1, gamma, beta, bn_hook, shard=None, ln=None):
+def stem_pair_bn(x, w0, b0, w1, b1, gamma, beta, bn_hook, shard=None, ln=None, pack=None):
     if ln is None:
-        return _StemPairBN.apply(x, w0, b0, w1, b1, gamma, beta, bn_hook, shard)
+        return _StemPairBN.apply(x, w0, b0, w1, b1, gamma, beta, bn_hook, shard, None, None, None, pack)
     lg, lb, eps, relu = ln
-    return _StemPairBN.apply(x, w0, b0, w1, b1, gamma, beta, bn_hook, shard, lg, lb, (eps, relu, lg is not None))
+    return _StemPairBN.apply(x, w0, b0, w1, b1, gamma, beta, bn_hook, shard, lg, lb, (eps, relu, lg is not None), pack)
 
 
 def stem_ln_supported(x, w1) -> bool:
@@ -363,7 +366,7 @@
 class _LinearBNActRes(torch.autograd.Function):
 
     @staticmethod
-    def forward(ctx, y, x0, w, b, gamma, beta, bn_hook, relu: bool, use_res: bool, shard, chain, first: bool):
+    def forward(ctx, y, x0, w, b, gamma, beta, bn_hook, relu: bool, use_res: bool, shard, chain, first: bool, pack=None):
         K.check(y, x0)
         dt = x0.dtype
         wc = w.detach().to(dt).contiguous()
@@ -381,7 +384,10 @@
         be32 = beta.detach().float().contiguous() if beta is not None else None
         mean = mean.detach().float().contiguous()
         rstd = rstd.detach().float().contiguous()
-        out = K.bn_apply(z, mean, rstd, g32, be32, xr if use_res else None, relu)
+        if pack is not None:
+            out, pack["out"] = K.bn_apply_packed(z, mean, rstd, g32, be32, xr if use_res else None, relu, pack["slot_bytes"])
+        else:
+            out = K.bn_apply(z, mean, rstd, g32, be32, xr if use_res else None, relu)
         ctx.save_for_backward(yr, xr, z, wc, g32, be32, mean, rstd)
         ctx.meta = (bool(relu), bool(use_res), bool(training), float(n_tot), shard, chain, bool(first), w.dtype,
                     None if b is None else b.dtype, None if gamma is None else gamma.dtype)
@@ -437,11 +443,11 @@
         dbeta = stats[:d].to(gdt) if be32 is not None else None
         if shard is not None and g32 is not None:
             dgamma, dbeta = shard.unsum(dgamma), shard.unsum(dbeta)
-        return dy, dx0, dw, db, dgamma, dbeta, None, None, None, None, None, None
-
-
-def linear_bn_act_res(y, x0, w, b, gamma, beta, bn_hook, relu, use_res, shard, chain, first):
-    return _LinearBNActRes.apply(y, x0, w, b, gamma, beta, bn_hook, relu, use_res, shard, chain, first)
+        return dy, dx0, dw, db, dgamma, dbeta, None, None, None, None, None, None, None
+
+
+def linear_bn_act_res(y, x0, w, b, gamma, beta, bn_hook, relu, use_res, shard, chain, first, pack=None):
+    return _LinearBNActRes.apply(y, x0, w, b, gamma, beta, bn_hook, relu, use_res, shard, chain, first, pack)
 
 
 def linear(x, w, b):
diff --git a/sgformer_amd/ours.py b/sgformer_amd/ours.py
--- a/sgformer_amd/ours.py
+++ b/sgformer_amd/ours.py
@@ -16,6 +16,8 @@
 import os as _os
 OVERLAP_BRANCHES = _os.environ.get("SGF_OVERLAP", "1") == "1"
 OVERLAP_MIN_NODES = 65536
+
+PACKED_SLOT_BYTES = (384, 0, 0)
 _side_streams = {}
 
 
@@ -102,7 +104,7 @@
     def reset_parameters(self):
         self.W.reset_parameters()
 
-    def propagate(self, x, edge_index):
+    def propagate(self, x, edge_index, packed=None):
         shard = self._shard
         if isinstance(edge_index, ops.CSRGraph):
             graph = edge_index
@@ -110,7 +112,8 @@
             graph = shard.graph_for(edge_index)
         else:
             graph = ops.graph_cache.get(edge_index, x.shape[0])
-        return ops.spmm(graph, x, None if (shard is not None and shard.local_graph) else shard)
+        shard = None if (shard is not None and shard.local_graph) else shard
+        return ops.spmm(graph, x, shard, packed if shard is None else None)
 
     def forward(self, x, edge_index, x0, bn_stats=False):
         shard = self._shard
@@ -212,6 +215,22 @@
             return mean, torch.rsqrt(var + bn.eps), n_tot, use_batch
         return hook
 
+    def pack_request(self, layer: int, n: int, dtype, edge_index):
+        slot = PACKED_SLOT_BYTES[layer] if layer < len(PACKED_SLOT_BYTES) else 0
+        drop_on = self.training and self.dropout is not None and self.dropout > 0.0
+        if (not slot or drop_on or self._shard is not None or ops.K.name != "hip" or layer >= len(self.convs)
+                or self.convs[layer]._shard is not None or torch.cuda.is_current_stream_capturing()):
+            return None
+        if isinstance(edge_index, ops.CSRGraph):
+            graph = edge_index
+        elif torch.is_tensor(edge_index):
+            graph = ops.graph_cache.get(edge_index, n)
+        else:
+            return None
+        d = self.fcs[0].out_features
+        slot = ops.spmm_packed_slot(graph, (n, d), dtype, slot)
+        return {"slot_bytes": slot, "out": None} if slot else None
+
     def fused_stem_ok(self, x) -> bool:
         import os
         d = self.fcs[0].out_features
@@ -241,9 +260,10 @@
 
     def forward(self, x, edge_index, stem=None):
         ops._require_cuda(x, None if isinstance(edge_index, ops.CSRGraph) else edge_index)
-        x_first = None
-        if stem is not None and len(stem) == 3:
-            _, x, x_first = stem
+        x_first = packed = None
+        if stem is not None and len(stem) >= 3:
+            x, x_first = stem[1], stem[2]
+            packed = stem[3].pop("out", None) if len(stem) > 3 and stem[3] is not None else None
         else:
             if stem is not None:
                 x, stats0 = stem
@@ -256,9 +276,12 @@
                 x = x_first
             for i, conv in enumerate(self.convs):
                 bn = self.bns[i + 1]
-                y = conv.propagate(x, edge_index)
+                y = conv.propagate(x, edge_index, packed)
+                packed = None
+                req = self.pack_request(i + 1, x0.shape[0], x0.dtype, edge_index) if self.use_act else None
                 x = ops.linear_bn_act_res(y, x0, conv.W.weight, conv.W.bias, bn.weight, bn.bias, self._bn_hook(bn),
-                                          self.use_act, self.use_residual, self._shard, chain, i == 0)
+                                          self.use_act, self.use_residual, self._shard, chain, i == 0, req)
+                packed = req.pop("out", None) if req is not None else None
             return x
         uses_init = [c.use_init for c in self.convs]
         k = 1 + sum(uses_init) + (len(self.convs) if self.use_residual else 0)
@@ -518,9 +541,10 @@
             ln = None
             if getattr(tc, "use_bn", False) and hasattr(tc, "bns") and ops.stem_ln_supported(x, wt):
                 ln = (tc.bns[0].weight, tc.bns[0].bias, tc.bns[0].eps, True)
+            req = gc.pack_request(0, x.shape[0], x.dtype, edge_index)
             x0a, x0b, yt = ops.stem_pair_bn(x, wg, gc.fcs[0].bias, wt, tc.fcs[0].bias,
-                                            bn0.weight, bn0.bias, gc._bn_hook(bn0), gc._shard, ln)
-            stem_t, stem_g = (("ln", yt) if ln is not None else yt), ("bn", x0a, x0b)
+                                            bn0.weight, bn0.bias, gc._bn_hook(bn0), gc._shard, ln, req)
+            stem_t, stem_g = (("ln", yt) if ln is not None else yt), ("bn", x0a, x0b, req)
         elif both and ops.stem_pair_supported(x, wg, wt):
             want = gc.use_bn and _uses_batch_stats(gc, gc.bns[0])
             (yg, yt), st = ops.stem_pair(x, wg, gc.fcs[0].bias, wt, tc.fcs[0].bias,
```

Measured after the change: 29.57 million (median of 6 runs). 1.4% higher.
